# zhoubin-me/supertonic

Measured on AMD Instinct MI355X. Metric: audio-sec/sec (RTF^-1), 66M model, batch=128 per GPU, higher is better.
Workload: dtype bf16

## Files before the change

### include/stn.h

```cpp
#ifndef STN_H
#define STN_H
#include <stddef.h>
#include <stdint.h>

#include "stn_arch.h"

#ifdef __cplusplus
extern "C" {
#endif

#define STN_OK 0
#define STN_ERR_INVALID (-1)
#define STN_ERR_DEVICE (-2)
#define STN_ERR_STATE (-3)
#define STN_ERR_UNSUPPORTED (-4)
#define STN_ERR_IO (-5)

#define STN_DTYPE_F32 0
#define STN_DTYPE_BF16 1
#define STN_DTYPE_F16 2

typedef struct stn_handle stn_handle;

typedef struct stn_config {
// ... 240 lines not shown
int stn_op_expander(stn_handle* h, int hz, int rows, int W, const float* x, const stn_expander* c, float* y);
int stn_op_expander_ex(stn_handle* h, int hz, int rows, int W, const float* x, const stn_expander* c, int x_misalign, int in_place, float* y,
                       float* open_db, float* s1_end, float* s1_start, float* s2_end, float* s2_start, int* guard_ok, char* form,
                       size_t form_cap);
int stn_expander_coefs(const stn_expander* c, int rate_hz, double k[3], float k32[3], int64_t* hold_samples);
int stn_expander_curve(const stn_expander* c, int n, const double* in_db, double* out_db);
const char* stn_expander_error(const stn_expander* c, int rate_hz);

int stn_profile_enable(stn_handle* h, int on);
int stn_profile_reset(stn_handle* h);
int stn_profile_filter(stn_handle* h, const char* family_or_null);
int stn_profile_sample(stn_handle* h, int every);
int stn_launch_log_enable(stn_handle* h, int on);
int64_t stn_launch_log(stn_handle* h, char* out, size_t cap);
int stn_profile_count(stn_handle* h);
int stn_profile_get(stn_handle* h, int idx, char* name, size_t name_cap, double* total_ms, int64_t* launches,
                    double* flops, double* bytes);

int stn_dbg_xattn_hs_enable(stn_handle* h, int on);
int64_t stn_dbg_xattn_hs_stamps(stn_handle* h, unsigned long long* out, size_t cap);
int stn_dbg_fold_run_frames(const int32_t* latent_lengths, int B, int n_cu);

int stn_op_gemm(stn_handle* h, int dtype, int M, int N, int K, const float* A , const float* W ,
                const float* bias_or_null, int act , float* out );
int stn_op_gemm_ex(stn_handle* h, int dtype, int M, int N, int K, const float* A , const float* W , int mode, int act,
                   int out_dtype, int ldo, const float* bias_or_null, const float* gamma_or_null, const int32_t* len_or_null, int L,
                   const int32_t* row_b_or_null, const float* rowvec_or_null, int nseq, int nt, int tr, float* out, int64_t out_elems,
                   char* form, size_t form_cap);
int stn_dbg_gemm_form(int dtype, int M, int N, int K, int mode, int out_dtype, int ldo, int masked, int tr, char* out, size_t cap);
int stn_dbg_ffn_form(int dtype, int stage, int C, int I, int64_t M, int64_t gate_rows, int packed, int k, int max_dil, int mask,
                     int64_t min_rows, int64_t split_min_rows, int nt_hints, char* out, size_t cap);
int stn_op_gemm_bench(stn_handle* h, int dtype, int M, int N, int K, int mode, int iters, double* avg_ms);
int stn_op_gemm_phases(stn_handle* h, int dtype, int M, int N, int K, int mode, double* out6);
int stn_op_dwconv_ln(stn_handle* h, int dtype, int B, int L, int C, int k, int dil, const float* x,
                     const float* w , const float* bias, const float* ln_g, const float* ln_b, float* y);
int stn_op_dwconv_ln_ragged(stn_handle* h, int dtype, int B, int L, int C, int k, int dil, const float* x,
                            const float* w , const float* bias, const float* ln_g, const float* ln_b,
                            const int32_t* seqlen , float* y);
int stn_op_gemm_rows(stn_handle* h, int dtype, int M, int N, int K, const float* A, const float* W, const float* bias_or_null, int B,
                     const int32_t* rows, const int32_t* valid, int T, float* out, int64_t out_elems, char* form, size_t form_cap);
int stn_op_dwconv_ln_ex(stn_handle* h, int dtype, int B, int L, int C, int k, int dil, const float* x, int64_t x_rows,
                        const float* w_or_null , const float* bias_or_null, const float* ln_g, const float* ln_b,
                        const int32_t* seqlen_or_null, int packed, int ln_only, float* y, int64_t y_rows, char* form, size_t form_cap);
int stn_op_dwconv_ln_tail(stn_handle* h, int dtype, int B, int L, int C, int k, int dil, const float* x, int64_t x_rows,
                          const float* w , const float* bias, const float* ln_g, const float* ln_b, const int32_t* seqlen,
                          const float* tail , int T, int rf, float* y, int64_t y_rows, char* form, size_t form_cap);
int64_t stn_dbg_len_tables(int B, const int32_t* llen, int ve_rows, int with_pairs, int vo_form, int ccf, int T, int rf, int32_t* layout,
                           int32_t* out, int64_t out_n);
int stn_dbg_dwconv_ln_form(int dtype, int B, int L, int C, int k, int packed, char* out, size_t cap);
int stn_op_fold_ln(stn_handle* h, int dtype, int M, int C, int S, const float* part, const float* b2, const float* gamma,
                   const float* rowvec_or_null, const int32_t* row_b_or_null, int nseq, const float* ln_g, const float* ln_b, float* x,
                   float* y);
int stn_op_layout(stn_handle* h, int which, int dtype, const int32_t* p, int n_p, const float* a, int64_t a_n, const float* b, int64_t b_n,
                  const float* c, int64_t c_n, const int64_t* ids, int64_t ids_n, const int32_t* len, int packed, float* out, int64_t out_n,
                  float* out2, int64_t out2_n, int32_t* iout, int64_t iout_n);
int stn_op_attention(stn_handle* h, int dtype, int B, int Lq, int Lk, int H, int dh, const float* q, const float* k,
                     const float* v, const int32_t* qlen_or_null, const int32_t* klen_or_null, int rope_mode, float* o);
int stn_op_attention_ex(stn_handle* h, int dtype, int B, int Lq, int Lk, int H, int dh, const float* q, int64_t q_elems, int ldq,
                        int q_col, float* kv, int64_t kv_elems, int ldk, int k_col, int v_col, float* o, int64_t o_elems, int ldo,
                        const int32_t* qlen_or_null, const int32_t* klen_or_null, const int32_t* q_off_or_null,
                        const int32_t* k_off_or_null, int rope_mode, int k_rotated, int rot_groups, int rot_stride, int rot_col,
                        char* form, size_t form_cap);
int stn_op_xattn_hs(stn_handle* h, int dtype, int M, const float* xn, const float* Wq, const float* bq_or_null, const float* Wo,
                    const float* kv, int64_t kv_elems, int ldk, int k_col, int B, int L, int Lk, const int32_t* qlen,
                    const int32_t* klen_or_null, const int32_t* k_off_or_null, int rope_mode, int pairs_mode, int64_t part_stride,
                    float* part, int64_t part_elems, int32_t* pairs_out_or_null, char* form, size_t form_cap);
int stn_dbg_attn_form(int kind, int dtype, int B, int Lq, int Lk, int H, int dh, int ldq, int ldk, int misaligned, char* out, size_t cap);
int stn_op_ffn(stn_handle* h, int M, int C, int I, const float* xn , const float* W1, const float* b1, const float* W2,
               const float* b2_or_null, const float* gamma_or_null, const float* rowvec_or_null ,
               const int32_t* row_b_or_null , int nseq, float* x, int fused);
int stn_op_ffn_ex(stn_handle* h, int dtype, int M, int C, int I, const float* xn, int ldx, int64_t xn_elems, const float* W1, const float* b1,
                  const float* W2, const float* b2_or_null, const float* gamma_or_null, const int32_t* len_or_null, int L,
                  const int32_t* row_b_or_null, const float* rowvec_or_null, int rv_ld, int nseq, int mode, int split, float* x, int ldo,
                  int64_t x_elems, float* part_or_null, int64_t part_stride, int64_t part_elems, char* form, size_t form_cap);
int stn_op_ffn_bench(stn_handle* h, int M, int C, int I, int fused, int iters, double* out5);
int stn_op_fold_dwconv_ln(stn_handle* h, int B, int C, int k, int dil, int S, const int32_t* seqlen, const float* x, const float* part,
                          const float* b2_or_null, const float* gamma_or_null, const float* rowvec_or_null , const float* w ,
                          const float* bias, const float* ln_g, const float* ln_b, float* x_out, float* y);
int stn_op_fold_dwconv_ln_ex(stn_handle* h, int dtype, int B, int L, int C, int k, int dil, int S, int run_frames, const int32_t* seqlen,
                             const float* x_in, int64_t x_rows, const float* part, int64_t part_stride, int64_t part_elems,
                             const float* b2_or_null, const float* gamma_or_null, const float* rowvec_or_null, int rv_ld,
                             const float* w , const float* bias, const float* ln_g, const float* ln_b, float* x_out, int64_t x_out_rows,
                             float* y, int64_t y_rows, char* form, size_t form_cap);
int stn_dbg_fold_dwconv_ln_form(int dtype, int B, int L, int C, int k, int dil, int S, int has_rowvec, int run_frames, char* out, size_t cap);
int stn_op_block_bench(stn_handle* h, int B, int L, int C, int I, int k, int dil, int mode, int iters, double* out6);
int stn_op_randn(stn_handle* h, uint64_t seed, int B, int D, int L, const int64_t* utt_ids_or_null,
                 const int32_t* len_or_null, float* out);

const char* stn_version(void);
int stn_hip_versions(int* built, int* runtime);
int stn_device_count(void);
int stn_device_sync(int device);
int stn_ffn_fused_forms(int dtype, int C, int I);

#ifdef __cplusplus
}
#endif
#endif
```

### supertonic_amd/binding.py

```python
import ctypes
import os

import numpy as np

from .arch import StnArch

_HERE = os.path.dirname(os.path.abspath(__file__))
LIB_PATH = os.environ.get("STN_LIB") or os.path.join(_HERE, "libstn.so")
_LIB = None

F32, BF16, F16 = 0, 1, 2
_DTYPES = {"f32": F32, "fp32": F32, "float32": F32, "bf16": BF16, "f16": F16, "fp16": F16, "float16": F16, "half": F16,
           F32: F32, BF16: BF16, F16: F16}
ACT_NONE, ACT_GELU, ACT_SILU, ACT_GELU_TANH = 0, 1, 2, 3
EPI_STORE, EPI_RESID, EPI_STORE_T = 0, 1, 2
FFN_VOCODER, FFN_ESTIMATOR, FFN_TEXT = 1, 2, 4
LAYOUT_ROW_MAP, LAYOUT_NCL_TO_ROWS, LAYOUT_EULER_NCL, LAYOUT_UNPACK_ROWS, LAYOUT_EMBED, LAYOUT_MASKED_MEAN, LAYOUT_IM2COL, LAYOUT_VOCODER_IN = range(8)
LAYOUT_FILL_ROWS, LAYOUT_HS_PAIRS, LAYOUT_TRIM_LEN = 8, 9, 10
ENC_F32, ENC_PCM16, ENC_PCM24, ENC_MULAW, ENC_ALAW = 0, 1, 2, 3, 4
ENCODINGS = {"f32": ENC_F32, "pcm16": ENC_PCM16, "pcm24": ENC_PCM24, "mulaw": ENC_MULAW, "alaw": ENC_ALAW}
ENCODING_NAMES = {v: k for k, v in ENCODINGS.items()}
ENCODING_BYTES = {ENC_F32: 4, ENC_PCM16: 2, ENC_PCM24: 3, ENC_MULAW: 1, ENC_ALAW: 1}
ZERO_CODEWORD = {ENC_F32: 0, ENC_PCM16: 0, ENC_PCM24: 0, ENC_MULAW: 0xFF, ENC_ALAW: 0xD5}

# ... 462 lines not shown
    L.stn_batch_ve_rows.argtypes = [vp]
    L.stn_batch_ve_rows.restype = ctypes.c_int64
    L.stn_batch_vo_rows.argtypes = [vp]
    L.stn_batch_vo_rows.restype = ctypes.c_int64
    L.stn_graph_replays.restype = ctypes.c_int64
    L.stn_graph_replays.argtypes = [vp]
    L.stn_graphs_cached.restype = ctypes.c_int64
    L.stn_graphs_cached.argtypes = [vp]
    L.stn_batch_dims.argtypes = [vp, ctypes.POINTER(ci), ctypes.POINTER(ci), ctypes.POINTER(ctypes.c_int64)]
    L.stn_batch_fetch.argtypes = [vp, vp, ctypes.c_size_t, vp]
    L.stn_batch_fetch_latent.argtypes = [vp, _f32p]
    L.stn_batch_fetch_pcm16.argtypes = [vp, vp, ctypes.c_size_t, vp]
    L.stn_batch_fetch_pcm16_begin.argtypes = [vp, ci]
    L.stn_batch_fetch_slot_dims.argtypes = [vp, ci, ctypes.POINTER(ci), ctypes.POINTER(ctypes.c_int64)]
    L.stn_batch_fetch_pcm16_end.argtypes = [vp, ci, ctypes.POINTER(vp), ctypes.POINTER(ctypes.c_size_t), vp]
    L.stn_host_alloc_pinned.restype = vp
    L.stn_host_alloc_pinned.argtypes = [ctypes.c_size_t]
    L.stn_host_free_pinned.argtypes = [vp]
    L.stn_batch_wav_device_ptr.argtypes = [vp, ctypes.POINTER(vp)]
    L.stn_sync.argtypes = [vp]
    L.stn_set_stream.argtypes = [vp, vp]
    L.stn_batch_copy_wav_device.argtypes = [vp, vp, ctypes.c_int64]
    L.stn_batch_copy_pcm16_device.argtypes = [vp, vp, ctypes.c_int64]
    L.stn_profile_filter.argtypes = [vp, ctypes.c_char_p]
    L.stn_profile_sample.argtypes = [vp, ci]
    L.stn_launch_log_enable.argtypes = [vp, ci]
    L.stn_dbg_xattn_hs_enable.argtypes = [vp, ci]
    L.stn_dbg_xattn_hs_stamps.argtypes = [vp, vp, ctypes.c_size_t]
    L.stn_dbg_xattn_hs_stamps.restype = ctypes.c_int64
    L.stn_dbg_fold_run_frames.argtypes = [vp, ctypes.c_int, ctypes.c_int]
    L.stn_dbg_fold_run_frames.restype = ctypes.c_int
    L.stn_dbg_gemm_form.argtypes = [ci, ci, ci, ci, ci, ci, ci, ci, ci, ctypes.c_char_p, ctypes.c_size_t]
    L.stn_dbg_gemm_form.restype = ctypes.c_int
    L.stn_dbg_attn_form.argtypes = [ci, ci, ci, ci, ci, ci, ci, ci, ci, ci, ctypes.c_char_p, ctypes.c_size_t]
    L.stn_dbg_attn_form.restype = ctypes.c_int
    L.stn_dbg_ffn_form.argtypes = [ci, ci, ci, ci, ctypes.c_int64, ctypes.c_int64, ci, ci, ci, ci, ctypes.c_int64, ctypes.c_int64, ci,
                                   ctypes.c_char_p, ctypes.c_size_t]
    L.stn_dbg_ffn_form.restype = ctypes.c_int
    L.stn_launch_log.argtypes = [vp, ctypes.c_char_p, ctypes.c_size_t]
    L.stn_launch_log.restype = ctypes.c_int64
    L.stn_profile_enable.argtypes = [vp, ci]
    L.stn_profile_reset.argtypes = [vp]
    L.stn_profile_count.argtypes = [vp]
    L.stn_profile_get.argtypes = [vp, ci, ctypes.c_char_p, ctypes.c_size_t, ctypes.POINTER(ctypes.c_double),
                                  ctypes.POINTER(ctypes.c_int64), ctypes.POINTER(ctypes.c_double),
                                  ctypes.POINTER(ctypes.c_double)]
    L.stn_op_gemm.argtypes = [vp, ci, ci, ci, ci, _f32p, _f32p, vp, ci, _f32p]
    L.stn_op_gemm_ex.argtypes = [vp, ci, ci, ci, ci, _f32p, _f32p, ci, ci, ci, ci, vp, vp, vp, ci, vp, vp, ci, ci, ci, _f32p,
                                 ctypes.c_int64, ctypes.c_char_p, ctypes.c_size_t]
    L.stn_op_gemm_bench.argtypes = [vp, ci, ci, ci, ci, ci, ci, ctypes.POINTER(ctypes.c_double)]
    L.stn_op_gemm_phases.argtypes = [vp, ci, ci, ci, ci, ci, ctypes.POINTER(ctypes.c_double)]
    L.stn_op_dwconv_ln.argtypes = [vp, ci, ci, ci, ci, ci, ci, _f32p, _f32p, _f32p, _f32p, _f32p, _f32p]
    L.stn_op_dwconv_ln_ragged.argtypes = [vp, ci, ci, ci, ci, ci, ci, _f32p, _f32p, _f32p, _f32p, _f32p, _i32p, _f32p]
    L.stn_op_attention.argtypes = [vp, ci, ci, ci, ci, ci, ci, _f32p, _f32p, _f32p, vp, vp, ci, _f32p]
    L.stn_op_gemm_rows.argtypes = [vp, ci, ci, ci, ci, _f32p, _f32p, vp, ci, _i32p, _i32p, ci, _f32p, ctypes.c_int64, ctypes.c_char_p, ctypes.c_size_t]
    L.stn_op_dwconv_ln_ex.argtypes = [vp, ci, ci, ci, ci, ci, ci, _f32p, ctypes.c_int64, vp, vp, _f32p, _f32p, vp, ci, ci, _f32p, ctypes.c_int64,
                                      ctypes.c_char_p, ctypes.c_size_t]
    L.stn_op_dwconv_ln_tail.argtypes = [vp, ci, ci, ci, ci, ci, ci, _f32p, ctypes.c_int64, _f32p, _f32p, _f32p, _f32p, _i32p, _f32p, ci, ci, _f32p,
                                        ctypes.c_int64, ctypes.c_char_p, ctypes.c_size_t]
    L.stn_dbg_resample_form.argtypes = [ci, ci, ctypes.c_int64, ctypes.c_char_p, ctypes.c_size_t]
    L.stn_dbg_resample_form.restype = ctypes.c_int
    L.stn_dbg_dwconv_ln_form.argtypes = [ci, ci, ci, ci, ci, ci, ctypes.c_char_p, ctypes.c_size_t]
    L.stn_dbg_dwconv_ln_form.restype = ctypes.c_int
    L.stn_dbg_len_tables.argtypes = [ci, _i32p, ci, ci, ci, ci, ci, ci, _i32p, ctypes.c_void_p, ctypes.c_int64]
    L.stn_dbg_len_tables.restype = ctypes.c_int64
    L.stn_op_fold_ln.argtypes = [vp, ci, ci, ci, ci, _f32p, _f32p, _f32p, vp, vp, ci, _f32p, _f32p, _f32p, _f32p]
    L.stn_op_layout.argtypes = [vp, ci, ci, _i32p, ci, vp, ctypes.c_int64, vp, ctypes.c_int64, vp, ctypes.c_int64, vp, ctypes.c_int64, vp, ci,
                                vp, ctypes.c_int64, vp, ctypes.c_int64, vp, ctypes.c_int64]
    L.stn_op_attention_ex.argtypes = [vp, ci, ci, ci, ci, ci, ci, _f32p, ctypes.c_int64, ci, ci, _f32p, ctypes.c_int64, ci, ci, ci,
                                      _f32p, ctypes.c_int64, ci, vp, vp, vp, vp, ci, ci, ci, ci, ci, ctypes.c_char_p, ctypes.c_size_t]
    L.stn_op_xattn_hs.argtypes = [vp, ci, ci, _f32p, _f32p, vp, _f32p, _f32p, ctypes.c_int64, ci, ci, ci, ci, ci, _i32p, vp, vp, ci, ci,
                                  ctypes.c_int64, _f32p, ctypes.c_int64, vp, ctypes.c_char_p, ctypes.c_size_t]
    L.stn_op_randn.argtypes = [vp, cu64, ci, ci, ci, vp, vp, _f32p]
    L.stn_op_ffn.argtypes = [vp, ci, ci, ci, _f32p, _f32p, _f32p, _f32p, vp, vp, vp, vp, ci, _f32p, ci]
    L.stn_op_ffn_ex.argtypes = [vp, ci, ci, ci, ci, _f32p, ci, ctypes.c_int64, _f32p, _f32p, _f32p, vp, vp, vp, ci, vp, vp, ci, ci, ci, ci, _f32p, ci,
                                ctypes.c_int64, vp, ctypes.c_int64, ctypes.c_int64, ctypes.c_char_p, ctypes.c_size_t]
    L.stn_op_ffn_bench.argtypes = [vp, ci, ci, ci, ci, ci, ctypes.POINTER(ctypes.c_double)]
    L.stn_set_fused_ffn.argtypes = [vp, ci]
    L.stn_set_fused_ffn_min_rows.argtypes = [vp, ctypes.c_int64, ctypes.c_int64]
    L.stn_op_fold_dwconv_ln.argtypes = [vp, ci, ci, ci, ci, ci, _i32p, _f32p, _f32p, vp, vp, vp, _f32p, _f32p, _f32p, _f32p, _f32p, _f32p]
    L.stn_op_fold_dwconv_ln_ex.argtypes = [vp, ci, ci, ci, ci, ci, ci, ci, ci, _i32p, _f32p, ctypes.c_int64, _f32p, ctypes.c_int64, ctypes.c_int64, vp, vp,
                                           vp, ci, _f32p, _f32p, _f32p, _f32p, _f32p, ctypes.c_int64, _f32p, ctypes.c_int64, ctypes.c_char_p,
                                           ctypes.c_size_t]
    L.stn_dbg_fold_dwconv_ln_form.argtypes = [ci, ci, ci, ci, ci, ci, ci, ci, ci, ctypes.c_char_p, ctypes.c_size_t]
    L.stn_dbg_fold_dwconv_ln_form.restype = ctypes.c_int
    L.stn_op_block_bench.argtypes = [vp, ci, ci, ci, ci, ci, ci, ci, ci, ctypes.POINTER(ctypes.c_double)]
    L.stn_group_create.argtypes = [ci, vp, ci, ctypes.POINTER(vp)]
    L.stn_group_destroy.argtypes = [vp]
    L.stn_group_last_error.restype = ctypes.c_char_p
    L.stn_group_last_error.argtypes = [vp]
    L.stn_group_size.argtypes = [vp]
    L.stn_group_uses_rccl.argtypes = [vp]
    L.stn_group_handle.restype = vp
    L.stn_group_handle.argtypes = [vp, ci]
    L.stn_group_load_synthetic.argtypes = [vp, ctypes.POINTER(StnArch), cu64]
    L.stn_group_load_dir.argtypes = [vp, ctypes.c_char_p]
    L.stn_group_deal.argtypes = [ci, _i32p, ci, _i32p, _i32p]
    L.stn_group_synthesize.argtypes = [vp, ci, ci, _i64p, _f32p, _f32p, _f32p, ci, cf, vp, cu64, ctypes.POINTER(ctypes.c_int64)]
    L.stn_group_fetch_pcm16.argtypes = [vp, vp, ctypes.c_size_t, vp]
    L.stn_set_output_rate.argtypes = [vp, ci]
    L.stn_get_output_rate.argtypes = [vp]
    L.stn_resample_filter.argtypes = [ci, ci, vp, ctypes.c_size_t, ctypes.POINTER(ci), ctypes.POINTER(ci)]
    L.stn_resample_error.argtypes = [ci, ci]
    L.stn_resample_error.restype = ctypes.c_char_p
    L.stn_op_resample.argtypes = [vp, ci, ci, ci, ci, _f32p, vp, vp]
    L.stn_group_set_output_rate.argtypes = [vp, ci]
    _f64p = np.ctypeslib.ndpointer(np.float64, flags="C_CONTIGUOUS")
    L.stn_set_loudness.argtypes = [vp, ci, cf, cf]
    L.stn_get_loudness.argtypes = [vp, ctypes.POINTER(ci), ctypes.POINTER(cf), ctypes.POINTER(cf)]
    L.stn_batch_loudness.argtypes = [vp, vp, vp, vp]
    L.stn_op_loudness.argtypes = [vp, ci, ci, ci, _f32p, vp, vp, vp]
    L.stn_kweighting_filter.argtypes = [ci, _f64p, _f64p, _f64p, _f64p]
    L.stn_op_loudness_ex.argtypes = [vp, ci, ci, ci, _f32p, vp, ci, cf, cf, ci, vp, vp, vp, vp, vp, vp, vp, vp, ctypes.c_char_p, ctypes.c_size_t]
    L.stn_loudness_table.argtypes = [ci, vp, vp, ctypes.c_size_t, ctypes.POINTER(ci)]
    L.stn_group_set_loudness.argtypes = [vp, ci, cf, cf]
    L.stn_batch_loudness_range.argtypes = [vp, vp, vp, vp, vp]
    L.stn_op_loudness_range.argtypes = [vp, ci, ci, ci, _f32p, vp, vp, vp, vp, vp]
    L.stn_set_silence_trim.argtypes = [vp, ci, cf, cf, cf]
    L.stn_get_silence_trim.argtypes = [vp, ctypes.POINTER(ci), ctypes.POINTER(cf), ctypes.POINTER(cf), ctypes.POINTER(cf)]
    L.stn_batch_silence_edges.argtypes = [vp, vp, vp]
    L.stn_op_silence_edges.argtypes = [vp, ci, ci, ci, _f32p, vp, cf, cf, vp, vp]
    L.stn_op_silence_trim.argtypes = [vp, ci, ci, ci, _f32p, vp, cf, cf, cf, vp, ci, vp, vp, vp]
    L.stn_silence_fade_window.argtypes = [ci, cf, vp, ctypes.c_int64, ctypes.POINTER(ctypes.c_int64)]
    L.stn_set_pause_limit.argtypes = [vp, ci, cf]
    L.stn_get_pause_limit.argtypes = [vp, ctypes.POINTER(ci), ctypes.POINTER(cf)]
    L.stn_batch_pauses.argtypes = [vp, vp, vp, vp, ci]
    L.stn_op_pause_trim.argtypes = [vp, ci, ci, ci, _f32p, vp, cf, cf, cf, cf, vp, ci, vp, vp, vp, vp, vp, vp, ci]
    L.stn_op_silence_edges_ex.argtypes = [vp, ci, ci, ci, _f32p, vp, cf, cf, cf, cf, ci, vp, vp, vp, vp, vp, vp, vp, vp, ci, ctypes.c_char_p,
                                          ctypes.c_size_t]
    L.stn_group_set_pause_limit.argtypes = [vp, ci, cf]
    L.stn_set_limiter.argtypes = [vp, ci, cf]
    L.stn_get_limiter.argtypes = [vp, ctypes.POINTER(ci), ctypes.POINTER(cf)]
    L.stn_batch_limiter.argtypes = [vp, vp, vp]
    L.stn_op_limiter.argtypes = [vp, ci, ci, ci, _f32p, vp, vp, cf, cf, vp, vp, vp, vp]
    L.stn_limiter_window.argtypes = [ci, cf, vp, ctypes.c_int64, ctypes.POINTER(ctypes.c_int64)]
    L.stn_group_set_limiter.argtypes = [vp, ci, cf]
    L.stn_set_peak_mode.argtypes = [vp, ci]
    L.stn_get_peak_mode.argtypes = [vp]
    L.stn_group_set_peak_mode.argtypes = [vp, ci]
    L.stn_true_peak_filter.argtypes = [vp, ctypes.c_size_t, ctypes.POINTER(ci), ctypes.POINTER(ci)]
    L.stn_batch_true_peak.argtypes = [vp, vp, vp, vp]
    L.stn_op_true_peak.argtypes = [vp, ci, ci, ci, _f32p, vp, vp, ci, vp, vp, vp, ctypes.c_char_p, ctypes.c_size_t]
    L.stn_op_limiter_ex.argtypes = [vp, ci, ci, ci, _f32p, vp, vp, cf, cf, vp, vp, vp, vp, ci, vp, vp]
    fp = ctypes.POINTER(StnFilter)
    L.stn_set_filters.argtypes = [vp, ci, fp]
    L.stn_get_filters.argtypes = [vp, ctypes.POINTER(ci), fp]
    L.stn_group_set_filters.argtypes = [vp, ci, fp]
    L.stn_op_filter.argtypes = [vp, ci, ci, ci, _f32p, ci, fp, _f32p]
    L.stn_op_filter_ex.argtypes = [vp, ci, ci, ci, _f32p, ci, fp, ci, _f32p, vp, vp, ctypes.POINTER(ci), ctypes.c_char_p, ctypes.c_size_t]
    L.stn_filter_error.argtypes = [ci, fp, ci]
    L.stn_filter_error.restype = ctypes.c_char_p
    L.stn_filter_coefs.argtypes = [fp, ci, _f64p, _f32p]
    L.stn_filter_response.argtypes = [ci, fp, ci, ci, _f64p, _f64p]
    L.stn_dbg_filter_geometry.argtypes = [ctypes.POINTER(ci)] * 4
    cpp = ctypes.POINTER(StnCompressor)
    L.stn_set_compressor.argtypes = [vp, ci, cpp]
    L.stn_get_compressor.argtypes = [vp, ctypes.POINTER(ci), cpp]
    L.stn_group_set_compressor.argtypes = [vp, ci, cpp]
    L.stn_batch_compressor.argtypes = [vp, vp]
    L.stn_op_compressor.argtypes = [vp, ci, ci, ci, _f32p, cpp, _f32p]
    L.stn_op_compressor_ex.argtypes = [vp, ci, ci, ci, _f32p, cpp, ci, ci, _f32p, vp, vp, vp, vp, vp, ctypes.POINTER(ci), ctypes.c_char_p, ctypes.c_size_t]
    L.stn_compressor_error.argtypes = [cpp, ci]
    L.stn_compressor_error.restype = ctypes.c_char_p
    L.stn_compressor_coefs.argtypes = [cpp, ci, _f64p, _f32p]
    L.stn_compressor_curve.argtypes = [cpp, ci, _f64p, _f64p]
    xpp = ctypes.POINTER(StnExpander)
# ... 483 lines not shown
        raise StnError(-1, f"stn_limiter_window: {lookahead_ms} ms at {hz} Hz refused (lookahead_ms in [0.5, 10], hz in [8000, 192000])")
    w = np.empty(n.value, np.float32)
    if L.stn_limiter_window(int(hz), float(lookahead_ms), w.ctypes.data, w.size, ctypes.byref(n)) < 0:
        raise StnError(-1, "stn_limiter_window failed")
    return w


def _loudness_args(target_lufs):
    return (0, -23.0) if target_lufs is None else (1, float(target_lufs))


def resample_error(in_hz, out_hz):
    return load().stn_resample_error(int(in_hz), int(out_hz)).decode()


def resample_form(in_hz, out_hz, W):
    buf = ctypes.create_string_buffer(64)
    r = load().stn_dbg_resample_form(int(in_hz), int(out_hz), int(W), buf, len(buf))
    if r < 0:
        why = resample_error(in_hz, out_hz)
        raise StnError(r, f"stn_dbg_resample_form: {why}" if why else f"stn_dbg_resample_form: W = {W}, W >= 1 is required")
    return buf.value.decode()


def fold_run_frames(latent_lengths, n_cu=256):
    a = np.ascontiguousarray(latent_lengths, dtype=np.int32)
    r = load().stn_dbg_fold_run_frames(a.ctypes.data, len(a), int(n_cu))
    if r < 0:
        raise StnError(r, "stn_dbg_fold_run_frames: bad arguments")
    return int(r)


def gemm_form(dtype, M, N, K, mode=EPI_STORE, out_dtype="f32", ldo=None, masked=False, tr=-1):
    buf = ctypes.create_string_buffer(128)
    r = load().stn_dbg_gemm_form(_DTYPES[dtype], int(M), int(N), int(K), int(mode), _DTYPES[out_dtype], int(N if ldo is None else ldo),
                                 int(bool(masked)), int(tr), buf, len(buf))
    if r < 0:
        raise StnError(r, "stn_dbg_gemm_form: the launcher refuses this call")
    return buf.value.decode()


def attn_form(dtype, B, Lq, Lk, H, dh, ldq=None, ldk=None, misaligned=0, kind=0):
    buf = ctypes.create_string_buffer(64)
    C = H * dh
    r = load().stn_dbg_attn_form(int(kind), _DTYPES[dtype], int(B), int(Lq), int(Lk), int(H), int(dh), int(C if ldq is None else ldq),
                                 int(C if ldk is None else ldk), int(misaligned), buf, len(buf))
    if r < 0:
        raise StnError(r, "stn_dbg_attn_form: the launcher refuses this call")
    return buf.value.decode()


def dwconv_ln_form(dtype, B, L, C, k, packed=False):
    buf = ctypes.create_string_buffer(32)
    r = load().stn_dbg_dwconv_ln_form(_DTYPES[dtype], int(B), int(L), int(C), int(k), int(bool(packed)), buf, len(buf))
    if r < 0:
        raise StnError(r, "stn_dbg_dwconv_ln_form: the launcher refuses this call")
    return buf.value.decode()


LEN_VO_NONE, LEN_VO_2RF, LEN_VO_TAIL, LEN_VO_SCALED = range(4)


def len_tables(llen, ve_rows=0, with_pairs=False, vo_form=LEN_VO_NONE, ccf=6, T=0, rf=0):
    llen = _c(llen, np.int32)
    B = len(llen)
    lay = np.zeros(9, np.int32)
    args = (B, llen, int(ve_rows), int(bool(with_pairs)), int(vo_form), int(ccf), int(T), int(rf))
    tot = load().stn_dbg_len_tables(*args, lay, None, 0)
    if tot < 0:
        raise StnError(int(tot), "stn_dbg_len_tables: bad argument")
    out = np.full(tot, -12345, np.int32)
    out[:2] = 7
    assert load().stn_dbg_len_tables(*args, lay, out.ctypes.data, out.size) == tot
    assert out[0] == 7 and out[1] == 7
    names = ("seed", "llen", "ve_off", "ve_row_b", "pairs", "vo_n", "vo_valid", "vo_off")
    sizes = {"llen": B, "ve_off": B + 1, "ve_row_b": int(ve_rows), "pairs": B + 2, "vo_n": B, "vo_valid": B, "vo_off": B + 1}
    res = {"total": int(tot)}
    for i, n in enumerate(names):
        if n != "seed" and lay[i] >= 0:
            res[n] = out[lay[i]:lay[i] + sizes[n]].copy()
    return res


def fold_dwconv_ln_form(dtype, B, L, C, k, dil, S, rowvec=True, run_frames=0):
    buf = ctypes.create_string_buffer(96)
    r = load().stn_dbg_fold_dwconv_ln_form(_DTYPES[dtype], int(B), int(L), int(C), int(k), int(dil), int(S), int(bool(rowvec)), int(run_frames),
                                           buf, len(buf))
    if r < 0:
        raise StnError(r, "stn_dbg_fold_dwconv_ln_form: the launcher refuses this call")
    return buf.value.decode()


def ffn_form(dtype, stage, C, I, M, gate_rows=0, packed=True, k=5, max_dil=1, mask=9, min_rows=18432, split_min_rows=1, nt_hints=True):
    buf = ctypes.create_string_buffer(32)
    r = load().stn_dbg_ffn_form(_DTYPES[dtype], int(stage), int(C), int(I), int(M), int(gate_rows), int(bool(packed)), int(k), int(max_dil),
                                int(mask), int(min_rows), int(split_min_rows), int(bool(nt_hints)), buf, len(buf))
    if r < 0:
        raise StnError(r, "stn_dbg_ffn_form: invalid arguments")
    return buf.value.decode()


def _c(a, dt):
    return np.ascontiguousarray(a, dtype=dt)


def _opt(a, dt):
    if a is None:
        return None, None
    arr = _c(a, dt)
    return arr, arr.ctypes.data


class Engine:

    def __init__(self, device=0, dtype="bf16"):
        self._lib = load()
        self._h = ctypes.c_void_p()
        cfg = StnConfig(device, _DTYPES[dtype])
        rc = self._lib.stn_create(ctypes.byref(cfg), ctypes.byref(self._h))
        if rc != 0:
            msg = self._lib.stn_last_error(None).decode()
            self._h = None
            raise StnError(rc, msg)
        self.dtype = _DTYPES[dtype]
        self.device = device
        self.arch = None
        self._slot_enc = {}

    def close(self):
        if getattr(self, "_h", None):
            self._lib.stn_destroy(self._h)
            self._h = None

    def __del__(self):
        try:
            self.close()
        except Exception:
            pass

    def _need_model(self):
        if self.arch is None:
            raise StnError(-3, "no model loaded: call load_synthetic or load_dir first")

    def _ck(self, rc):
        if rc < 0:
            raise StnError(rc, self._lib.stn_last_error(self._h).decode())
        return rc

    def load_synthetic(self, arch: StnArch, seed: int = 7):
        self._ck(self._lib.stn_load_synthetic(self._h, ctypes.byref(arch), seed))
        self.arch = arch

    def last_error(self) -> str:
        return (self._lib.stn_last_error(self._h) or b"").decode()

    def load_dir(self, onnx_dir: str):
        self._ck(self._lib.stn_load_dir(self._h, onnx_dir.encode()))
        a = StnArch()
        self._ck(self._lib.stn_get_arch(self._h, ctypes.byref(a)))
        self.arch = a

    def tensor_names(self, arch: StnArch):
        n = self._ck(self._lib.stn_tensor_names(self._h, ctypes.byref(arch), None, 0))
        buf = ctypes.create_string_buffer(n + 1)
        self._ck(self._lib.stn_tensor_names(self._h, ctypes.byref(arch), buf, n + 1))
        return buf.value.decode().split("\n")[:-1]
# ... 781 lines not shown

    def op_gemm_bench(self, M, N, K, mode=0, iters=20, dtype=None):
        ms = ctypes.c_double()
        self._ck(self._lib.stn_op_gemm_bench(self._h, self.dtype if dtype is None else _DTYPES[dtype], M, N, K, mode,
                                             iters, ctypes.byref(ms)))
        return ms.value

    def op_ffn(self, xn, W1, b1, W2, b2, gamma, x, rowvec=None, row_b=None, fused=True):
        M, C = xn.shape
        I = W1.shape[0]
        out = np.array(x, dtype=np.float32, order="C", copy=True)
        _, b2p = _opt(b2, np.float32)
        b2a = _opt(b2, np.float32)[0]
        ga, gp = _opt(gamma, np.float32)
        rva, rvp = _opt(rowvec, np.float32)
        rba, rbp = _opt(row_b, np.int32)
        b2p = b2a.ctypes.data if b2a is not None else None
        self._ck(self._lib.stn_op_ffn(self._h, M, C, I, _c(xn, np.float32), _c(W1, np.float32), _c(b1, np.float32), _c(W2, np.float32),
                                      b2p, gp, rvp, rbp, 0 if rva is None else rva.shape[0], out, int(fused)))
        return out

    def op_ffn_ex(self, xn, W1, b1, W2, x, mode=1, b2=None, gamma=None, len=None, L=None, row_b=None, rowvec=None, split=0, part=None,
                  part_stride=0, M=None, dtype=None):
        xn = _c(xn, np.float32)
        I, C = W1.shape
        M = xn.shape[0] if M is None else int(M)
        x_r = np.array(x, dtype=np.float32, order="C", copy=True)
        p_r = None if part is None else np.array(part, dtype=np.float32, order="C", copy=True)
        nseq = 0
        for v in (len, rowvec):
            if v is not None:
                nseq = max(nseq, np.asarray(v).shape[0])
        if row_b is not None and rowvec is None:
            nseq = max(nseq, int(np.max(row_b)) + 1)
        _b, bp = _opt(b2, np.float32)
        _g, gp = _opt(gamma, np.float32)
        _l, lp = _opt(len, np.int32)
        _r, rp = _opt(row_b, np.int32)
        _v, vp_ = _opt(rowvec, np.float32)
        form = ctypes.create_string_buffer(32)
        self._ck(self._lib.stn_op_ffn_ex(self._h, self.dtype if dtype is None else _DTYPES[dtype], M, C, I, xn.reshape(-1), xn.shape[1], xn.size,
                                         _c(W1, np.float32), _c(b1, np.float32), _c(W2, np.float32), bp, gp, lp, int(M if L is None else L), rp, vp_,
                                         C if _v is None else _v.shape[1], nseq, int(mode), int(split), x_r.reshape(-1), x_r.shape[1], x_r.size,
                                         None if p_r is None else p_r.ctypes.data, int(part_stride), 0 if p_r is None else p_r.size, form,
                                         ctypes.sizeof(form)))
        return x_r, p_r, form.value.decode()

    def op_ffn_bench(self, M, C, I, fused=True, iters=20):
        out = (ctypes.c_double * 5)()
        self._ck(self._lib.stn_op_ffn_bench(self._h, M, C, I, int(fused), iters, out))
        return dict(ms=out[0], first_stage=out[1], tile_loop=out[2], epilogue=out[3], workgroups=int(out[4]))

    def op_fold_dwconv_ln(self, seqlen, x, part, b2, gamma, rowvec, w, bias, g, b, k, dil):
        seqlen = np.ascontiguousarray(seqlen, np.int32)
        S, M, C = part.shape
        xo = np.empty((M, C), np.float32)
        y = np.empty((M, C), np.float32)
        b2a, _ = _opt(b2, np.float32)
        ga, _ = _opt(gamma, np.float32)
        rva, _ = _opt(rowvec, np.float32)
        p = lambda a: None if a is None else a.ctypes.data
        self._ck(self._lib.stn_op_fold_dwconv_ln(self._h, len(seqlen), C, k, dil, S, seqlen, _c(x, np.float32), _c(part, np.float32), p(b2a), p(ga), p(rva),
                                                 _c(w, np.float32), _c(bias, np.float32), _c(g, np.float32), _c(b, np.float32), xo, y))
        return xo, y

    def op_fold_dwconv_ln_ex(self, seqlen, L, x_in, part, part_stride, S, b2, gamma, rowvec, w, bias, g, b, dil, x_out, y, run_frames=0, dtype=None):
        seqlen = _c(seqlen, np.int32)
        x_in = _c(x_in, np.float32)
        part = _c(part, np.float32).reshape(-1)
        xo = np.array(x_out, dtype=np.float32, order="C", copy=True)
        yo = np.array(y, dtype=np.float32, order="C", copy=True)
        C = x_in.shape[1]
        w = _c(w, np.float32)
        _b2, b2p = _opt(b2, np.float32)
        _g, gp = _opt(gamma, np.float32)
        _v, vp_ = _opt(rowvec, np.float32)
        form = ctypes.create_string_buffer(96)
        self._ck(self._lib.stn_op_fold_dwconv_ln_ex(self._h, self.dtype if dtype is None else _DTYPES[dtype], len(seqlen), int(L), C, w.shape[1], int(dil),
                                                    int(S), int(run_frames), seqlen, x_in.reshape(-1), x_in.shape[0], part, int(part_stride), part.size,
                                                    b2p, gp, vp_, C if _v is None else _v.shape[1], w, _c(bias, np.float32), _c(g, np.float32),
                                                    _c(b, np.float32), xo.reshape(-1), xo.shape[0], yo.reshape(-1), yo.shape[0], form, ctypes.sizeof(form)))
        return xo, yo, form.value.decode()

    def op_block_bench(self, B, L, C, I, k, dil, mode, iters=20):
        out = (ctypes.c_double * 6)()
        self._ck(self._lib.stn_op_block_bench(self._h, B, L, C, I, k, dil, mode, iters, out))
        return dict(ms=out[0], conv_ms=out[1], fold_phase1=out[2], fold_barrier=out[3], fold_phase2=out[4], fold_span=out[5])

    def set_fused_ffn_min_rows(self, k4_rows=-1, split_rows=-1):
        self._ck(self._lib.stn_set_fused_ffn_min_rows(self._h, int(k4_rows), int(split_rows)))

    def op_gemm_phases(self, M, N, K, mode=0, dtype=None):
        out = (ctypes.c_double * 6)()
        self._ck(self._lib.stn_op_gemm_phases(self._h, self.dtype if dtype is None else _DTYPES[dtype], M, N, K, mode, out))
        return dict(first_stage=out[0], k_loop=out[1], epilogue=out[2], grid_span=out[3], entry_spread=out[4], workgroups=int(out[5]))

    def op_dwconv_ln(self, x, w, bias, g, b, dil, dtype=None, seqlen=None):
        B, L, C = x.shape
        k = w.shape[1]
        y = np.empty((B, L, C), np.float32)
        if seqlen is not None:
            self._ck(self._lib.stn_op_dwconv_ln_ragged(self._h, self.dtype if dtype is None else _DTYPES[dtype], B, L, C, k,
                                                       dil, _c(x, np.float32), _c(w, np.float32), _c(bias, np.float32),
                                                       _c(g, np.float32), _c(b, np.float32), _c(seqlen, np.int32), y))
            return y
        self._ck(self._lib.stn_op_dwconv_ln(self._h, self.dtype if dtype is None else _DTYPES[dtype], B, L, C, k, dil,
                                            _c(x, np.float32), _c(w, np.float32), _c(bias, np.float32),
                                            _c(g, np.float32), _c(b, np.float32), y))
        return y

    def op_gemm_rows(self, A, W, out, rows, valid, T, bias=None, dtype=None):
        A = _c(A, np.float32)
        W = _c(W, np.float32)
        rows = _c(rows, np.int32)
        valid = _c(valid, np.int32)
        o_r = np.array(out, dtype=np.float32, order="C", copy=True)
        _b, bp = _opt(bias, np.float32)
        form = ctypes.create_string_buffer(96)
        self._ck(self._lib.stn_op_gemm_rows(self._h, self.dtype if dtype is None else _DTYPES[dtype], A.shape[0], W.shape[0], A.shape[1],
                                            A.reshape(-1), W.reshape(-1), bp, len(rows), rows, valid, int(T), o_r.reshape(-1), o_r.size, form,
                                            ctypes.sizeof(form)))
        return o_r, form.value.decode()

    def op_dwconv_ln_ex(self, x, w, bias, g, b, dil, out, B, L, seqlen=None, packed=False, ln_only=False, dtype=None):
        x = _c(x, np.float32)
        o_r = np.array(out, dtype=np.float32, order="C", copy=True)
        C = x.shape[1]
        _w, wp = _opt(w, np.float32)
        _b, bp = _opt(bias, np.float32)
        _l, lp = _opt(seqlen, np.int32)
        form = ctypes.create_string_buffer(32)
        self._ck(self._lib.stn_op_dwconv_ln_ex(self._h, self.dtype if dtype is None else _DTYPES[dtype], int(B), int(L), C,
                                               1 if _w is None else _w.shape[1], int(dil), x.reshape(-1), x.shape[0], wp, bp, _c(g, np.float32),
                                               _c(b, np.float32), lp, int(bool(packed)), int(bool(ln_only)), o_r.reshape(-1), o_r.shape[0], form,
                                               ctypes.sizeof(form)))
        return o_r, form.value.decode()

    def op_dwconv_ln_tail(self, x, w, bias, g, b, dil, out, L, seqlen, tail, T, dtype=None):
        x = _c(x, np.float32)
        tail = _c(tail, np.float32)
        o_r = np.array(out, dtype=np.float32, order="C", copy=True)
        C = x.shape[1]
        w = _c(w, np.float32)
        seqlen = _c(seqlen, np.int32)
        assert tail.ndim == 2 and tail.shape[1] == C and tail.shape[0] >= 1
        form = ctypes.create_string_buffer(32)
        self._ck(self._lib.stn_op_dwconv_ln_tail(self._h, self.dtype if dtype is None else _DTYPES[dtype], len(seqlen), int(L), C, w.shape[1],
                                                 int(dil), x.reshape(-1), x.shape[0], w, _c(bias, np.float32), _c(g, np.float32),
                                                 _c(b, np.float32), seqlen, tail.reshape(-1), int(T), tail.shape[0] - 1, o_r.reshape(-1),
                                                 o_r.shape[0], form, ctypes.sizeof(form)))
        return o_r, form.value.decode()

    def op_fold_ln(self, x, part, b2, gamma, g, b, rowvec=None, row_b=None, dtype=None):
        x_r = np.array(x, dtype=np.float32, order="C", copy=True)
        M, C = x_r.shape
        part = _c(part, np.float32)
        y = np.empty((M, C), np.float32)
        _v, vp_ = _opt(rowvec, np.float32)
        _r, rp = _opt(row_b, np.int32)
        self._ck(self._lib.stn_op_fold_ln(self._h, self.dtype if dtype is None else _DTYPES[dtype], M, C, part.shape[0], part.reshape(-1),
                                          _c(b2, np.float32), _c(gamma, np.float32), vp_, rp, 0 if _v is None else _v.shape[0],
                                          _c(g, np.float32), _c(b, np.float32), x_r, y))
        return x_r, y

    def op_layout(self, which, p, a=None, b=None, c=None, ids=None, length=None, packed=False, out=None, out2=None, iout=None, dtype="f32"):
        def f32(v):
# ... 81 lines not shown
```

### supertonic_amd/csrc/api.cpp

```cpp
#include "../../include/stn.h"

#include <algorithm>
#include <complex>
#include <cstdio>
#include <cstring>
#include <fstream>
#include <string>

#include "engine.hpp"
#include "host/json_min.hpp"
#include "host/graph_bind.hpp"
#include "host/onnx_reader.hpp"

#include <map>
#include <sstream>

struct stn_handle {
    stn::Engine* eng = nullptr;
    std::string err;
    std::vector<std::pair<std::string, stn::KernelStat>> prof;
};

static thread_local std::string g_create_err;

#define STN_TRY(h, body)                                             \
    if (!(h)) return STN_ERR_INVALID;                                \
    try {                                                            \
        body;                                                        \
        return STN_OK;                                               \
    } catch (const std::invalid_argument& e) {                       \
        (h)->err = e.what();                                         \
        return STN_ERR_INVALID;                                      \
    } catch (const std::exception& e) {                              \
        (h)->err = e.what();                                         \
        return (h)->err.rfind("HIP error", 0) == 0 ? STN_ERR_DEVICE : STN_ERR_STATE; \
    } catch (...) {                                                  \
        (h)->err = "unknown failure";                                \
        return STN_ERR_DEVICE;                                       \
    }

static void need(bool ok, const char* what) {
    if (!ok) throw std::invalid_argument(what);
}
static void need_model(stn_handle* h) {
    if (!h->eng->loaded()) throw std::runtime_error("no model loaded: call stn_load_synthetic or stn_load_dir first");
}

extern "C" {

const char* stn_version(void) { return "supertonic_amd 0.1 (gfx950)"; }

int stn_hip_versions(int* built, int* runtime) {
    int rt = 0;
    const hipError_t e = hipRuntimeGetVersion(&rt);
    if (built) *built = HIP_VERSION;
    if (runtime) *runtime = e == hipSuccess ? rt : -1;
    return e == hipSuccess ? STN_OK : STN_ERR_DEVICE;
}
int stn_device_count(void) {
    int n = 0;
    if (hipGetDeviceCount(&n) != hipSuccess) { (void)hipGetLastError(); return STN_ERR_DEVICE; }
    return n;
}
int stn_device_sync(int device) {
    if (hipSetDevice(device) != hipSuccess || hipDeviceSynchronize() != hipSuccess) { (void)hipGetLastError(); return STN_ERR_DEVICE; }
    return STN_OK;
}
int stn_ffn_fused_forms(int dtype, int C, int I) {
    if (C <= 0 || I <= 0 || !stn::ffn_fused_supported(dtype, C, I)) return 0;
    return stn::ffn_split_factor(dtype, C, I) > 1 ? 2 : 1;
}

int stn_create(const stn_config* cfg, stn_handle** out) {
    if (!cfg || !out) { g_create_err = "stn_create: null argument"; return STN_ERR_INVALID; }
    *out = nullptr;
    try {
        stn_handle* h = new stn_handle;
        h->eng = new stn::Engine(cfg->device, cfg->dtype);
        *out = h;
        return STN_OK;
    } catch (const std::exception& e) {
        g_create_err = e.what();
        return STN_ERR_DEVICE;
    }
}
int stn_destroy(stn_handle* h) {
    if (!h) return STN_OK;
    try { delete h->eng; } catch (...) {}
    delete h;
    return STN_OK;
}
const char* stn_last_error(const stn_handle* h) { return h ? h->err.c_str() : g_create_err.c_str(); }
// ... 1039 lines not shown
    if (form && form_cap) std::snprintf(form, form_cap, "%s", f.c_str());
}
int stn_op_xattn_hs(stn_handle* h, int dtype, int M, const float* xn, const float* Wq, const float* bq, const float* Wo, const float* kv,
                    int64_t kv_elems, int ldk, int k_col, int B, int L, int Lk, const int32_t* qlen, const int32_t* klen, const int32_t* k_off,
                    int rope_mode, int pairs_mode, int64_t part_stride, float* part, int64_t part_elems, int32_t* pairs_out, char* form,
                    size_t form_cap) {
    STN_TRY(h, xattn_hs_checked(h, dtype, M, xn, Wq, bq, Wo, kv, kv_elems, ldk, k_col, B, L, Lk, qlen, klen, k_off, rope_mode, pairs_mode,
                                part_stride, part, part_elems, pairs_out, form, form_cap))
}
int stn_dbg_attn_form(int kind, int dtype, int B, int Lq, int Lk, int H, int dh, int ldq, int ldk, int misaligned, char* out, size_t cap) {
    if (B < 1 || Lq < 1 || Lk < 1 || H < 1 || (dtype != STN_DTYPE_F32 && dtype != STN_DTYPE_BF16 && dtype != STN_DTYPE_F16) || (kind != 0 && kind != 1))
        return STN_ERR_INVALID;
    std::string f;
    try {
        if (kind == 0) {
            auto ptr = [&](int bit) { return reinterpret_cast<const void*>((uintptr_t)(misaligned & bit ? 4 : 0)); };
            f = stn::attn_form(dtype, B, Lq, Lk, H, dh, ldq, ldk, ptr(1), ptr(2), ptr(4)).str();
        } else {
            f = stn::xattn_hs_form(dtype, H * dh, H, B, Lq, Lk, ldk).str();
        }
    } catch (const std::exception&) { return STN_ERR_INVALID; }
    if (out && cap > f.size()) std::memcpy(out, f.c_str(), f.size() + 1);
    return (int)f.size();
}
int stn_op_ffn(stn_handle* h, int M, int C, int I, const float* xn, const float* W1, const float* b1, const float* W2, const float* b2,
               const float* gamma, const float* rowvec, const int32_t* row_b, int nseq, float* x, int fused) {
    STN_TRY(h, { need(M > 0 && C > 0 && I > 0 && C % 8 == 0 && I % 8 == 0 && xn && W1 && b1 && W2 && x, "stn_op_ffn: bad argument");
                 need(!rowvec || nseq > 0, "stn_op_ffn: rowvec needs nseq > 0");
                 if (rowvec && row_b) for (int m = 0; m < M; ++m) need(row_b[m] >= 0 && row_b[m] < nseq, "stn_op_ffn: row_b out of range");
                 need(fused >= 0 && fused <= 2, "stn_op_ffn: mode must be 0 (two launches), 1 (K4) or 2 (K4-split + fold)");
                 h->eng->op_ffn(M, C, I, xn, W1, b1, W2, b2, gamma, rowvec, row_b, nseq, x, fused); })
}
static void ffn_ex_checked(stn_handle* h, int dtype, int M, int C, int I, const float* xn, int ldx, int64_t xn_elems, const float* W1, const float* b1,
                           const float* W2, const float* b2, const float* gamma, const int32_t* len, int L, const int32_t* row_b, const float* rowvec,
                           int rv_ld, int nseq, int mode, int split, float* x, int ldo, int64_t x_elems, float* part, int64_t part_stride,
                           int64_t part_elems, char* form, size_t form_cap) {
    need(M > 0 && C > 0 && I > 0 && C % 8 == 0 && I % 8 == 0 && xn && W1 && b1 && W2 && x && L >= 1, "stn_op_ffn_ex: bad argument");
    need((dtype == STN_DTYPE_BF16 || dtype == STN_DTYPE_F16) && dtype == h->eng->dtype(), "stn_op_ffn_ex: dtype must be the 16-bit format of the engine");
    need(mode >= stn::FFN_GEMMS && mode <= stn::FFN_K4_SPLIT, "stn_op_ffn_ex: mode must be 0 (two launches), 1 (K4) or 2 (K4-split)");
    need(mode == stn::FFN_GEMMS || stn::ffn_fused_supported(dtype, C, I), "stn_op_ffn_ex: shape not supported by the fused kernel");
    need(ldx >= C && ldx % 8 == 0 && xn_elems >= (int64_t)M * ldx, "stn_op_ffn_ex: needs ldx >= C, ldx % 8 == 0 and xn_elems >= M*ldx");
    need(ldo >= C && ldo % 4 == 0 && x_elems >= (int64_t)M * ldo, "stn_op_ffn_ex: needs ldo >= C, ldo % 4 == 0 and x_elems >= M*ldo");
    need(!(len && row_b), "stn_op_ffn_ex: len and row_b exclude each other");
    const int64_t seqs = ((int64_t)M + L - 1) / L;
    if (len || (rowvec && !row_b)) need(nseq >= seqs, "stn_op_ffn_ex: len / rowvec by m / L need nseq >= ceil(M/L)");
    if (rowvec || len || row_b) need(nseq > 0, "stn_op_ffn_ex: nseq must be > 0");
    if (rowvec) need(rv_ld >= C && rv_ld % 4 == 0, "stn_op_ffn_ex: needs rv_ld >= C and rv_ld % 4 == 0");
    if (len) for (int b = 0; b < nseq; ++b) need(len[b] >= 0 && len[b] <= L, "stn_op_ffn_ex: len out of [0, L]");
    if (row_b) for (int m = 0; m < M; ++m) need(row_b[m] >= 0 && row_b[m] < nseq, "stn_op_ffn_ex: row_b out of [0, nseq)");
    if (mode == stn::FFN_K4_SPLIT) {
        const int S = split ? split : stn::ffn_split_choose(dtype, C, I, M);
        need(stn::ffn_split_valid(dtype, C, I, S), "stn_op_ffn_ex: not a split this shape runs with");
        need(part && part_stride >= stn::ffn_split_rows(M) * C && part_stride % 8 == 0 && part_elems >= (int64_t)S * part_stride,
             "stn_op_ffn_ex: mode 2 needs part, part_stride >= rows padded to 128 * C (a multiple of 8) and part_elems >= S * part_stride");
    } else {
        need(split == 0 && !part, "stn_op_ffn_ex: split and part belong to mode 2");
    }
    const std::string f = h->eng->op_ffn_ex(M, C, I, xn, ldx, xn_elems, W1, b1, W2, b2, gamma, len, L, row_b, rowvec, rv_ld, nseq, mode, split, x, ldo,
                                            x_elems, part, part_stride, part_elems);
    if (form && form_cap) std::snprintf(form, form_cap, "%s", f.c_str());
}
int stn_op_ffn_ex(stn_handle* h, int dtype, int M, int C, int I, const float* xn, int ldx, int64_t xn_elems, const float* W1, const float* b1,
                  const float* W2, const float* b2, const float* gamma, const int32_t* len, int L, const int32_t* row_b, const float* rowvec, int rv_ld,
                  int nseq, int mode, int split, float* x, int ldo, int64_t x_elems, float* part, int64_t part_stride, int64_t part_elems, char* form,
                  size_t form_cap) {
    STN_TRY(h, ffn_ex_checked(h, dtype, M, C, I, xn, ldx, xn_elems, W1, b1, W2, b2, gamma, len, L, row_b, rowvec, rv_ld, nseq, mode, split, x, ldo,
                              x_elems, part, part_stride, part_elems, form, form_cap))
}
int stn_op_ffn_bench(stn_handle* h, int M, int C, int I, int fused, int iters, double* out5) {
    STN_TRY(h, { need(M > 0 && C > 0 && I > 0 && C % 8 == 0 && I % 8 == 0 && iters > 0 && out5, "stn_op_ffn_bench: bad argument");
                 need(fused >= 0 && fused <= 2, "stn_op_ffn_bench: mode must be 0, 1 or 2");
                 h->eng->op_ffn_bench(M, C, I, fused, iters, out5); })
}
int stn_op_fold_dwconv_ln(stn_handle* h, int B, int C, int k, int dil, int S, const int32_t* seqlen, const float* x, const float* part,
                          const float* b2, const float* gamma, const float* rowvec, const float* w, const float* bias, const float* g,
                          const float* b, float* x_out, float* y) {
    STN_TRY(h, { need(B > 0 && C > 0 && C % 8 == 0 && (k == 5 || k == 7) && dil > 0 && (S == 4 || S == 8 || S == 12 || S == 24) && seqlen && x && part && w && bias && g && b && x_out && y,
                      "stn_op_fold_dwconv_ln: bad argument");
                 int64_t tot = 0;
                 for (int i = 0; i < B; ++i) { need(seqlen[i] >= 0 && seqlen[i] < (1 << 20), "stn_op_fold_dwconv_ln: seqlen out of range"); tot += seqlen[i]; }
                 need(tot > 0, "stn_op_fold_dwconv_ln: no rows");
                 h->eng->op_fold_dwconv_ln(B, C, k, dil, S, seqlen, x, part, b2, gamma, rowvec, w, bias, g, b, x_out, y); })
}
static void fold_dwconv_ln_ex_checked(stn_handle* h, int dtype, int B, int L, int C, int k, int dil, int S, int run_frames, const int32_t* seqlen,
                                      const float* x_in, int64_t x_rows, const float* part, int64_t part_stride, int64_t part_elems, const float* b2,
                                      const float* gamma, const float* rowvec, int rv_ld, const float* w, const float* bias, const float* g,
                                      const float* b, float* x_out, int64_t x_out_rows, float* y, int64_t y_rows, char* form, size_t form_cap) {
    const char* who = "stn_op_fold_dwconv_ln_ex";
    auto req = [&](bool ok, const char* what) { need(ok, (std::string(who) + ": " + what).c_str()); };
    req(B > 0 && L > 0 && C > 0 && seqlen && x_in && part && w && bias && g && b && x_out && y, "bad argument");
    req(dtype == STN_DTYPE_BF16 || dtype == STN_DTYPE_F16, "a 16-bit format needed");
    req(B <= 1024, "B <= 1024 needed");
    try { (void)stn::fold_dwconv_ln_form(dtype, B, L, C, k, dil, S, rowvec != nullptr, run_frames); }
    catch (const std::invalid_argument& e) { req(false, e.what()); }
    int64_t tot = 0;
    for (int i = 0; i < B; ++i) { req(seqlen[i] >= 0 && seqlen[i] <= L, "seqlen out of [0, L]"); tot += seqlen[i]; }
    req(tot > 0, "no rows");
    req(tot * C * 2 < 0x7FFFFFFFll, "too many rows");
    req(x_rows >= tot && x_out_rows >= tot && y_rows >= tot, "x_in / x_out / y hold fewer rows than the launch addresses");
    req(part_stride >= tot * C && part_stride % 8 == 0 && part_elems >= (int64_t)(S - 1) * part_stride + tot * C, "part smaller than the launch addresses, or a stride that is no multiple of 8");
    req(!rowvec || (rv_ld >= C && rv_ld % 4 == 0), "rv_ld >= C, a multiple of 4, needed");
    const std::string f = h->eng->op_fold_dwconv_ln_ex(dtype, B, L, C, k, dil, S, run_frames, seqlen, x_in, x_rows, part, part_stride, part_elems, b2, gamma,
                                                       rowvec, rv_ld, w, bias, g, b, x_out, x_out_rows, y, y_rows);
    if (form && form_cap) std::snprintf(form, form_cap, "%s", f.c_str());
}
int stn_op_fold_dwconv_ln_ex(stn_handle* h, int dtype, int B, int L, int C, int k, int dil, int S, int run_frames, const int32_t* seqlen,
                             const float* x_in, int64_t x_rows, const float* part, int64_t part_stride, int64_t part_elems, const float* b2,
                             const float* gamma, const float* rowvec, int rv_ld, const float* w, const float* bias, const float* g, const float* b,
                             float* x_out, int64_t x_out_rows, float* y, int64_t y_rows, char* form, size_t form_cap) {
    STN_TRY(h, fold_dwconv_ln_ex_checked(h, dtype, B, L, C, k, dil, S, run_frames, seqlen, x_in, x_rows, part, part_stride, part_elems, b2, gamma, rowvec,
                                         rv_ld, w, bias, g, b, x_out, x_out_rows, y, y_rows, form, form_cap))
}
int stn_dbg_fold_dwconv_ln_form(int dtype, int B, int L, int C, int k, int dil, int S, int has_rowvec, int run_frames, char* out, size_t cap) {
    std::string f;
    try { f = stn::fold_dwconv_ln_form(dtype, B, L, C, k, dil, S, has_rowvec != 0, run_frames).str(); } catch (const std::exception&) { return STN_ERR_INVALID; }
    if (out && cap > f.size()) std::memcpy(out, f.c_str(), f.size() + 1);
    return (int)f.size();
}
int stn_op_block_bench(stn_handle* h, int B, int L, int C, int I, int k, int dil, int mode, int iters, double* out2) {
    STN_TRY(h, { need(B > 0 && L > 0 && C > 0 && I > 0 && C % 8 == 0 && I % 8 == 0 && (k == 5 || k == 7) && dil > 0 && iters > 0 && out2 && (mode == 0 || mode == 2),
                      "stn_op_block_bench: bad argument");
                 h->eng->op_block_bench(B, L, C, I, k, dil, mode, iters, out2); })
}
int stn_op_randn(stn_handle* h, uint64_t seed, int B, int D, int L, const int64_t* utt_ids, const int32_t* len, float* out) {
    STN_TRY(h, { need(B > 0 && D > 0 && L > 0 && out, "stn_op_randn: bad argument"); h->eng->op_randn(seed, B, D, L, utt_ids, len, out); })
}

}
```

### supertonic_amd/csrc/engine.cpp

```cpp
#include "engine.hpp"
#include "dev_env.hpp"
#include "engine_internal.hpp"

#include <algorithm>
#include <cmath>
#include <cstdio>
#include <cstring>

namespace stn {
using detail::up;

Arena::~Arena() {
    for (auto& c : chunks_) (void)hipFree(c.p);
}
size_t Arena::capacity() const {
    size_t t = 0;
    for (auto& c : chunks_) t += c.cap;
    return t;
}
void* Arena::alloc(size_t bytes) {
    bytes = (bytes + 255) & ~size_t(255);
    if (bytes == 0) bytes = 256;
    for (;;) {
        if (cur_ < chunks_.size()) {
// ... 416 lines not shown
    if (g_launch_ev.start) {
        g_launch_ev = LaunchEvents{};
        ev_pool_.push_back(spans_.back().a);
        ev_pool_.push_back(spans_.back().b);
        spans_.pop_back();
    }
    prof_active_ = false;
}
void Engine::profile_reset() {
    sync();
    for (auto& sp : spans_) { ev_pool_.push_back(sp.a); ev_pool_.push_back(sp.b); }
    spans_.clear();
    g_launch_log.entries.clear();
}
void Engine::launch_log_enable(bool on) { g_launch_log.on = on; g_launch_log.family = "-"; g_launch_log.entries.clear(); }
std::string Engine::launch_log() const {
    std::string out;
    for (const auto& e : g_launch_log.entries) {
        std::string k = e.second;
        size_t b = 0;
        while (b < k.size() && (k[b] == '(' || k[b] == ' ' || k[b] == '&')) ++b;
        size_t en = b;
        while (en < k.size() && (isalnum((unsigned char)k[en]) || k[en] == '_' || k[en] == ':')) ++en;
        out += e.first + "\t" + k.substr(b, en - b) + "\n";
    }
    return out;
}
std::vector<std::pair<std::string, KernelStat>> Engine::profile_collect() {
    sync();
    std::unordered_map<std::string, KernelStat> acc;
    std::vector<std::string> order;
    for (auto& sp : spans_) {
        float ms = 0.f;
        if (hipEventElapsedTime(&ms, sp.a, sp.b) != hipSuccess) { (void)hipGetLastError(); continue; }
        auto it = acc.find(sp.tag);
        if (it == acc.end()) { order.push_back(sp.tag); it = acc.emplace(sp.tag, KernelStat{}).first; }
        it->second.ms += ms;
        it->second.launches += 1;
        it->second.flops += sp.flops;
        it->second.bytes += sp.bytes;
    }
    std::vector<std::pair<std::string, KernelStat>> out;
    for (auto& t : order) out.emplace_back(t, acc[t]);
    return out;
}

void Engine::gemm(const char* tag, int dt, const void* A, int lda, const Linear& w, int M, Epilogue e) {
    if (!e.bias) e.bias = w.b;
    const double esz = is_half(dt) ? 2.0 : 4.0;
    if (prof_on_) {
        double out_b = (double)M * w.N * (e.mode == EPI_STORE ? (is_half(e.out_dtype) ? 2.0 : 4.0) : (e.mode == EPI_RESID ? 8.0 : 4.0));
        prof_begin(tag, 2.0 * M * (double)w.N * w.K, ((double)M * w.K + (double)w.N * w.K) * esz + out_b);
    }
    const GemmForm f = gemm_form(dt, M, w.N, w.K, lda, w.K, e, A, w.w.as(dt));
    if (f.split > 1) {
        const Arena::Mark mk = ar_.mark();
        float* ws = f32_alloc((int64_t)f.split * M * w.N);
        launch_gemm_form(s_, f, A, lda, w.w.as(dt), w.K, M, w.N, w.K, e, ws);
        ar_.release(mk);
    } else {
        launch_gemm_form(s_, f, A, lda, w.w.as(dt), w.K, M, w.N, w.K, e, nullptr);
    }
    if (prof_on_) prof_end();
}

void* Engine::to_act(const float* src, int64_t n) {
    if (dt_ == F32) return const_cast<float*>(src);
    void* d = act_alloc(n);
    launch_cast(s_, dt_, src, n, d);
    return d;
}

void Engine::convnext(const ConvNeXt& p, const FfnForm& f, float* x, int B, int L, int C, int hid, int k, int dil, const int* len,
                      const int* conv_len, const float* rowvec, int rv_ld, const Ragged* rg, FoldState* fs, const DwconvTail& tl) {
    const int64_t M = rg ? (int64_t)rg->rows : (int64_t)B * L;
    if (f.kind == FFN_K4_SPLIT && !(fs && rg)) throw std::logic_error("convnext: K4-split needs the stage's fold state and packed rows");
    const Arena::Mark mk = ar_.mark();
    void* xn = act_alloc(M * C);
    if (fs) x = fs->x;
    if (tl.tail && (fs || !rg)) throw std::logic_error("convnext: a tail table needs packed rows and no fold state");
    if (fs && fs->pending) {
        if (prof_on_) prof_begin("fold_dwconv_ln", (double)M * C * (2.0 * k + 8 + 2.0 * fs->fold.S), (double)M * C * (8.0 + 2.0 + 2.0 * fs->fold.S));
        fs->fold.run_frames = rg->fold_run;
        launch_fold_dwconv_ln(s_, dt_, fs->x, fs->x_alt, B, L, C, fs->fold, p.dw_t, p.dw_b, k, dil, p.ln.g, p.ln.b, a_.ln_eps, xn, len, rg->off);
        if (prof_on_) prof_end();
        std::swap(fs->x, fs->x_alt);
        fs->pending = false;
        x = fs->x;
    } else {
        if (prof_on_) prof_begin("dwconv_ln", (double)M * C * (2.0 * k + 8), (double)M * C * (4.0 + (is_half(dt_) ? 2.0 : 4.0)));
        launch_dwconv_ln(s_, dt_, x, B, L, C, p.dw_t, p.dw_b, k, dil, p.ln.g, p.ln.b, a_.ln_eps, xn, rg ? len : conv_len, rg ? rg->off : nullptr, tl);
        if (prof_on_) prof_end();
    }
    FfnArgs fa;
    fa.xn = xn; fa.ldx = C; fa.b1 = p.pw1.b; fa.b2 = p.pw2.b; fa.gamma = p.gamma; fa.x = x; fa.ldo = C; fa.M = (int)M; fa.I = hid;
    fa.rowvec = rowvec; fa.rv_ld = rv_ld; fa.row_b = (rg && rowvec) ? rg->row_b : nullptr;
    fa.len = rg ? nullptr : len; fa.L = L;
    if (f.kind != FFN_GEMMS) {
        const auto fw = ffn_w_.find(p.pw1.w.as(dt_));
        const int* s = std::find(std::begin(FFN_SPLITS), std::end(FFN_SPLITS), f.split);
        fa.wseq = fw == ffn_w_.end() ? nullptr : f.kind == FFN_K4 ? fw->second.wseq : s != std::end(FFN_SPLITS) ? fw->second.wsplit[s - FFN_SPLITS] : nullptr;
        if (!fa.wseq) throw std::logic_error("convnext: no packed weight stream for " + f.str());
    }
    if (f.kind == FFN_K4_SPLIT) { fa.part = fs->part; fa.part_stride = fs->part_stride; }
    const FoldArgs pending = ffn_launch(f, C, fa, p.pw1, p.pw2);
    if (f.kind == FFN_K4_SPLIT) { fs->fold = pending; fs->pending = true; }
    ar_.release(mk);
}

FoldArgs Engine::ffn_launch(const FfnForm& f, int C, const FfnArgs& a, const Linear& w1, const Linear& w2) {
    const int64_t M = a.M;
    const int hid = a.I;
    FoldArgs pending;
    if (f.kind == FFN_K4_SPLIT) {
        FfnArgs sa;
        sa.xn = a.xn; sa.ldx = a.ldx; sa.wseq = a.wseq; sa.b1 = a.b1; sa.M = a.M; sa.I = hid; sa.ts = a.ts;
        sa.split = f.split; sa.part = a.part; sa.part_stride = a.part_stride;
        if (prof_on_) prof_begin("ffn_split", 4.0 * M * (double)C * hid, (double)M * C * (2.0 + 2.0 * sa.split) + 4.0 * C * hid);
        launch_ffn_fused(s_, dt_, C, sa);
        if (prof_on_) prof_end();
        pending = ffn_pending(f, a);
    } else if (f.kind == FFN_K4) {
        if (prof_on_) prof_begin("ffn_fused", 4.0 * M * (double)C * hid, (double)M * C * (2.0 + 8.0) + 4.0 * C * hid);
        launch_ffn_fused(s_, dt_, C, a);
        if (prof_on_) prof_end();
    } else {
        const Arena::Mark mk = ar_.mark();
        void* u = act_alloc(M * hid);
        Epilogue e1;
        e1.mode = EPI_STORE; e1.act = gelu_act_; e1.out_dtype = dt_; e1.out = u; e1.ldo = hid; e1.bias = a.b1; e1.nt = f.nt ? 1 : 0;
        gemm("gemm_pw1_gelu", dt_, a.xn, a.ldx, w1, (int)M, e1);
        Epilogue e2;
        e2.mode = EPI_RESID; e2.resid = a.x; e2.ldo = a.ldo; e2.bias = a.b2; e2.gamma = a.gamma; e2.len = a.len; e2.L = a.L;
        e2.rowvec = a.rowvec; e2.rv_ld = a.rv_ld; e2.row_b = a.row_b;
        gemm("gemm_pw2_resid", dt_, u, hid, w2, (int)M, e2);
        ar_.release(mk);
    }
    return pending;
}

void Engine::fold_layernorm(FoldState& fs, int64_t M, int C, const LNorm& ln, void* xn, const char* tag) {
    const size_t esz = is_half(dt_) ? 2 : 4;
    if (fs.pending) {
        if (prof_on_) prof_begin("fold_ln", (double)M * C * (8 + 2.0 * fs.fold.S), (double)M * C * (8.0 + esz + 2.0 * fs.fold.S));
        launch_fold_ln(s_, dt_, fs.x, M, C, fs.fold, ln.g, ln.b, a_.ln_eps, xn);
        if (prof_on_) prof_end();
        fs.pending = false;
        return;
    }
    if (tag && prof_on_) prof_begin(tag, (double)M * C * 8, (double)M * C * (4.0 + esz));
    launch_layernorm(s_, dt_, fs.x, M, C, ln.g, ln.b, a_.ln_eps, xn);
    if (tag && prof_on_) prof_end();
}

void Engine::attn_block(const Attn& p, float* x, int B, int Lq, int C, int H, const void* ctx, int Lk, const int* qlen,
                        const int* klen, int rope_mode, bool self, const Ragged* qrg) {
    const int64_t Mq = qrg ? (int64_t)qrg->rows : (int64_t)B * Lq, Mk = (int64_t)B * Lk;
    const Arena::Mark mk = ar_.mark();
    const size_t esz = is_half(dt_) ? 2 : 4;
    void* xn = act_alloc(Mq * C);
    if (prof_on_) prof_begin("layernorm", (double)Mq * C * 8, (double)Mq * C * (4.0 + esz));
    launch_layernorm(s_, dt_, x, Mq, C, p.ln.g, p.ln.b, a_.ln_eps, xn);
    if (prof_on_) prof_end();
    const char *q = nullptr, *k = nullptr, *v = nullptr;
    int ldq = C, ldk = 2 * C;
    if (self) {
// ... 597 lines not shown
```

### supertonic_amd/csrc/engine.hpp

```cpp
#pragma once
#include <cmath>
#include <hip/hip_runtime.h>

#include <algorithm>
#include <cstdint>
#include <functional>
#include <initializer_list>
#include <iterator>
#include <stdexcept>
#include <string>
#include <unordered_map>
#include <vector>

#include "../../include/stn_arch.h"
#include "host/len_tables.hpp"
#include "host/join_plan.hpp"
#include "host/pause_plan.hpp"
#include "host/formant.hpp"
#include "host/pitch.hpp"
#include "kernels.hpp"

namespace stn {

#define STN_HIP(expr)                                                                                          \
// ... 77 lines not shown

   private:
    char* p_ = nullptr;
    size_t cap_ = 0;
};

class DeviceTable {
   public:
    DeviceTable() = default;
    DeviceTable(const DeviceTable&) = delete;
    DeviceTable& operator=(const DeviceTable&) = delete;
    ~DeviceTable() { if (p_) (void)hipFree(p_); }
    void* put(Engine& e, const void* host, size_t bytes);
    template <typename T> T* put(Engine& e, const std::vector<T>& host) { return static_cast<T*>(put(e, host.data(), host.size() * sizeof(T))); }
    explicit operator bool() const { return p_ != nullptr; }

   private:
    void* p_ = nullptr;
};
template <typename Table, size_t N = 1>
struct OnDevice { Table t; DeviceTable dev[N]; };

struct RowSpans { const int64_t* n = nullptr; const int64_t* full = nullptr; };

struct Carve {
    char* base = nullptr;
    size_t off = 0;
    template <typename T> T* take(size_t count) {
        const size_t o = off;
        off += (count * sizeof(T) + 255) / 256 * 256;
        return base ? reinterpret_cast<T*>(base + o) : nullptr;
    }
};

enum Stage : int { ST_PITCH, ST_RATE, ST_FILTER, ST_EXPANDER, ST_DEESSER, ST_COMPRESSOR, N_STAGES };
struct RowsId {
    uint64_t seq = 0; int hz = 0; int64_t Wo = 0; uint64_t gen[N_STAGES] = {};
    bool operator==(const RowsId& o) const { return seq == o.seq && hz == o.hz && Wo == o.Wo && std::equal(gen, gen + N_STAGES, o.gen); }
};
template <typename Set, typename Table>
struct DynStage {
    bool on = false;
    Set set;
    uint64_t gen = 0;
    struct Made { Table t; Set from{}; DeviceTable dev[2]; };
    Made tab, op_tab;
    DevBuf buf;
    RowsId key; const void* key_buf = nullptr; bool valid = false;
};

struct KernelStat { double ms = 0; long launches = 0; double flops = 0; double bytes = 0; };

class Engine {
   public:
    Engine(int device, int dtype);
    ~Engine();
    Engine(const Engine&) = delete;

    void load_synthetic(const stn_arch& a, uint64_t seed);
    using TensorSource = std::function<std::vector<float>(const std::string& name, int rows, int cols)>;
    void load_tensors(const stn_arch& a, const TensorSource& src);
    std::vector<std::string> tensor_names(const stn_arch& a);
    bool loaded() const { return loaded_; }
    const stn_arch& arch() const { return a_; }
    int64_t param_count() const { return params_; }
    int dtype() const { return dt_; }
    hipStream_t stream() const { return s_; }
    void sync() { STN_HIP(hipStreamSynchronize(s_)); if (dp_s_) STN_HIP(hipStreamSynchronize(dp_s_)); if (te_s_) STN_HIP(hipStreamSynchronize(te_s_)); ++drains_; }
    void set_stream(hipStream_t s);

    struct Ragged;
    void duration_dev(int B, int Lt, const int64_t* ids, const float* style_dp, const int* tlen, float* dur, const Ragged* trg = nullptr);
    void text_enc_dev(int B, int Lt, const int64_t* ids, const float* style_ttl, const int* tlen, float* ncl, void* rows,
                      const Ragged* trg = nullptr);
    struct VeCtx { void* text_kv = nullptr; void* style_kv = nullptr; int Lt = 0; const int* text_off = nullptr; };
    VeCtx ve_prepare_dev(int B, int Lt, const void* text_rows, const float* style_ttl, const int* tlen, const Ragged* trg = nullptr, bool defer_text = false);
    void ve_text_kv_dev(const VeCtx& c, int B, int Lt, const void* text_rows, const int* tlen, const Ragged* trg);
    float* ve_time_cond_dev(int rows, const float* total_step, const float* current_step, float* tb_out = nullptr );
    struct TimeCond { int steps = 0, B = 0; uint64_t wgen = ~0ull; float* buf = nullptr; size_t cap = 0; float *tot = nullptr, *cur = nullptr, *dt = nullptr, *tb = nullptr; };
    TimeCond tcond_;
    void ensure_time_cond(int total_step, int B);
    struct Ragged { const int* off = nullptr; const int* row_b = nullptr; int rows = 0;
                    const int* hs_pairs = nullptr;
                    int fold_run = 0; };
    void ve_step_dev(int B, int L, const VeCtx& c, const float* noisy, const int* tlen, const int* llen,
                     const float* total_step, const float* current_step, float* denoised, const float* tb = nullptr,
                     const Ragged* rg = nullptr, const float* dt = nullptr ,
                     void* z_rows = nullptr ,
                     bool z_ready = false ,
                     bool z_next = false );
    void vocoder_dev(int B, int L, const float* latent, float* wav, const int* vlen = nullptr, int vrows = 0,
                     const int* valid = nullptr, bool tails = false, const int* voff = nullptr);
    int vocoder_receptive_field() const;
    void prepare_xattn_weights();
    std::unordered_map<const void*, const void*> frag_w_;
    void hs_stamps_enable(bool on);
    int64_t hs_stamps_fetch(unsigned long long* out, size_t cap);
    unsigned long long* hs_ts_ = nullptr;
    int hs_ts_wgs_ = 0;
    static constexpr int HS_TS_WG = 8192;
    const float* unit_vec_ = nullptr;
    std::unordered_map<const void*, const void*> frag_acc_w_;
    void prepare_vocoder_constants();
    void prepare_ffn_weights();
    struct FfnW { const void *wseq = nullptr, *wsplit[std::size(FFN_SPLITS)] = {}; };
    std::unordered_map<const void*, FfnW> ffn_w_;

    void duration(int B, int Lt, const int64_t* ids, const float* style_dp, const float* text_mask, float* dur);
    void text_enc(int B, int Lt, const int64_t* ids, const float* style_ttl, const float* text_mask, float* text_emb);
    void vector_est(int B, int L, int Lt, const float* noisy, const float* text_emb, const float* style_ttl,
                    const float* text_mask, const float* latent_mask, const float* total_step,
                    const float* current_step, float* denoised);
    void vocoder(int B, int L, const float* latent, float* wav);

    struct Batch {
        int B = 0, Lt = 0, L = 0, noise_L = 0, total_step = 0;
        float speed = 1.f;
        bool have_override = false, have_noise = false;
        uint64_t noise_seed = 0;
        int64_t* ids = nullptr; size_t ids_cap = 0;
        int* tlen = nullptr; size_t tlen_cap = 0;
        float* style_ttl = nullptr; size_t ttl_cap = 0;
        float* style_dp = nullptr; size_t dp_cap = 0;
        float* dur = nullptr; size_t dur_cap = 0;
        int* llen = nullptr;
        int* tab = nullptr; size_t tab_cap = 0;
        LenTables tl;
        int64_t* utt_ids = nullptr; size_t utt_cap = 0;
        float* noise = nullptr; size_t noise_cap = 0;
        float* xt[2] = {nullptr, nullptr}; size_t xt_cap[2] = {0, 0};
        float* wav = nullptr; size_t wav_cap = 0;
        unsigned char* text_side = nullptr; size_t text_side_cap = 0;
        unsigned char* text_rows = nullptr; size_t text_cap = 0;
        int* toff = nullptr; size_t toff_cap = 0;
        int trows = 0;
        uint64_t gen = 0;
        std::vector<float> h_dur; std::vector<int> h_llen;
    };
    void batch_upload(int B, int Lt, const int64_t* ids, const float* text_mask, const float* style_ttl,
                      const float* style_dp, const float* duration_override, const int64_t* utt_ids);
    void batch_set_noise(const float* noise, int L);
    void batch_run(int total_step, float speed, uint64_t noise_seed);
    void set_graph_mode(bool on) { graph_on_ = on; }
    void set_vocoder_mode(bool length_aware) { vo_ragged_ = length_aware; }
    void set_packed_rows(bool on) { packed_ve_ = on; }
    void set_gelu_form(int tanh_form) { if ((tanh_form != 0) != (gelu_act_ == ACT_GELU_TANH)) { sync(); drop_graphs(); } gelu_act_ = tanh_form ? ACT_GELU_TANH : ACT_GELU; }
    int gelu_form() const { return gelu_act_ == ACT_GELU_TANH ? 1 : 0; }
    void set_shape_buckets(bool on) { shape_buckets_ = on; }
    static int64_t bucket_up(int64_t x, int64_t min_gran) {
        if (x <= 0) return x;
        int64_t g = min_gran;
        while (g * 8 <= x) g *= 2;
        return (x + g - 1) / g * g;
    }
    void set_duration_read(bool always) { dur_read_always_ = always; }
    void set_fused_xattn(int mode) { fused_xattn_ = mode ? 1 : 0; }
    void set_fused_ffn(int mask) { fused_ffn_ = mask; }
    void set_fused_ffn_min_rows(int64_t k4_rows, int64_t split_rows) {
        sync(); drop_graphs();
        if (k4_rows >= 0) ffn_min_rows_ = k4_rows;
        if (split_rows >= 0) ffn_split_min_rows_ = split_rows;
    }
    int fused_ffn() const { return fused_ffn_; }
    int64_t last_ve_rows() const { return last_ve_rows_; }
    int64_t last_vo_rows() const { return last_vo_rows_; }
    bool packed_text_ok(int B) const {
        return packed_ve_ && B <= 1024 && dwconv_ln_supports_packed(a_.te_dim, a_.te_kernel) && dwconv_ln_supports_packed(a_.dp_dim, a_.dp_kernel);
    }
    bool packed_rows_ok(int B) const { return packed_ve_ && B <= 1024 && a_.ve_dilated > 0 && dwconv_ln_supports_packed(a_.ve_dim, a_.ve_kernel); }
    long graph_replays() const { return graph_replays_; }
    size_t graphs_cached() const { return graphs_.size(); }
    const Batch& batch() const { return bt_; }
    void batch_fetch(float* wav, size_t wav_capacity, float* duration);
    void batch_fetch_pcm16(int16_t* pcm, size_t capacity, float* duration);
    bool fetch_slot_dims(int slot, int* B, int64_t* W) const {
        const FetchSlot& f = fetch_[slot];
        if (!f.busy || f.dur.empty()) return false;
        *B = (int)f.dur.size(); *W = (int64_t)(f.n / f.dur.size());
        return true;
    }
    void batch_fetch_pcm16_begin(int slot);
    void batch_fetch_pcm16_end(int slot, const int16_t** pcm, size_t* n, float* duration);
    void batch_fetch_latent(float* latent);
    void batch_copy_wav_device(float* dst, int64_t dst_stride);
    void batch_copy_pcm16_device(int16_t* dst, int64_t dst_stride);
    void batch_fetch_encoded(int enc, void* dst, size_t capacity_bytes, float* duration);
    void batch_fetch_encoded_begin(int slot, int enc);
    void batch_fetch_encoded_end(int slot, const void** data, size_t* n_bytes, float* duration);
    void batch_copy_encoded_device(int enc, void* dst, int64_t dst_stride);
    void op_encode(int enc, int rows, int W, const float* x, void* y);
    void set_dither(int mode, uint64_t seed);
    int dither_mode() const { return dither_.mode; }
    uint64_t dither_seed() const { return dither_.seed; }
    void set_pitch(float semitones);
    float pitch() const { return ps_semi_; }
    int pitch_a() const { return ps_a_; }
    int pitch_b() const { return ps_b_; }
    bool pitch_on() const { return ps_a_ != ps_b_; }
    void op_time_stretch(int hz, int rows, int W, const float* x, const int64_t* n, int a, int b, float* y, int* delta, float* score);
    void op_pitch(int hz, int rows, int W, const float* x, const int64_t* n, float semitones, float* y);
    void set_pitch_mode(int mode);
    int pitch_mode() const { return ps_mode_; }
    struct FormantProbe {
        float *ax = nullptr, *cy = nullptr;
        double *g = nullptr, *ex = nullptr, *ey = nullptr;
        bool guard_ok = false;
    };
    void op_formant(int hz, int rows, int W, const float* x, const float* y, const int64_t* n, float* out, FormantProbe* probe = nullptr);
// ... 81 lines not shown
    void op_filter(int hz, int rows, int W, const float* x, int n, const stn_filter* f, float* y, FlProbe* probe);

    void set_compressor(bool on, const stn_compressor* c);
    bool compressor_on() const { return cp_.on; }
    const stn_compressor& compressor() const { return cp_.set; }
    void batch_compressor(float* max_reduction_db);
    struct CpProbe {
        int x_misalign = 0, in_place = 0;
        float *gr = nullptr, *s1_end = nullptr, *s1_start = nullptr, *s2_end = nullptr, *s2_start = nullptr;
        bool guard_ok = false;
        const char* form = "";
    };
    void op_compressor(int hz, int rows, int W, const float* x, const stn_compressor& c, float* y, CpProbe* probe);

    void set_deesser(bool on, const stn_deesser* c);
    bool deesser_on() const { return ds_.on; }
    const stn_deesser& deesser() const { return ds_.set; }
    void batch_deesser(float* max_reduction_db);
    struct DsProbe {
        int x_misalign = 0, in_place = 0;
        float *band = nullptr, *gr = nullptr, *st_end = nullptr, *st_start = nullptr;
        float *s1_end = nullptr, *s1_start = nullptr, *s2_end = nullptr, *s2_start = nullptr;
        bool guard_ok = false;
        const char* form = "";
    };
    void op_deesser(int hz, int rows, int W, const float* x, const stn_deesser& c, float* y, DsProbe* probe);

    void set_expander(bool on, const stn_expander* c);
    bool expander_on() const { return xp_.on; }
    const stn_expander& expander() const { return xp_.set; }
    void batch_expander(float* min_attenuation_db, int64_t* closed_samples);
    struct XpProbe {
        int x_misalign = 0, in_place = 0;
        float *open = nullptr, *s1_end = nullptr, *s1_start = nullptr, *s2_end = nullptr, *s2_start = nullptr;
        bool guard_ok = false;
        const char* form = "";
    };
    void op_expander(int hz, int rows, int W, const float* x, const stn_expander& c, float* y, XpProbe* probe);

    void profile_enable(bool on) { if (on != prof_on_) profile_reset(); prof_on_ = on; }
    void launch_log_enable(bool on);
    std::string launch_log() const;
    void profile_sample(int every) { prof_every_ = every < 1 ? 1 : every; prof_seen_ = 0; }
    void profile_filter(const std::string& family) { if (family != prof_filter_) profile_reset(); prof_filter_ = family; }
    void profile_reset();
    std::vector<std::pair<std::string, KernelStat>> profile_collect();

    void op_gemm(int dtype, int M, int N, int K, const float* A, const float* W, const float* bias, int act, float* out);
    std::string op_gemm_ex(int dtype, int M, int N, int K, const float* A, const float* W, int mode, int act, int out_dtype, int ldo,
                           const float* bias, const float* gamma, const int* len, int L, const int* row_b, const float* rowvec, int nseq,
                           int nt, int tr, float* out, int64_t out_elems);
    std::string op_attention_ex(int dtype, int B, int Lq, int Lk, int H, int dh, const float* q, int64_t q_elems, int ldq, int q_col,
                                float* kv, int64_t kv_elems, int ldk, int k_col, int v_col, float* o, int64_t o_elems, int ldo,
                                const int* qlen, const int* klen, const int* q_off, const int* k_off, int rope_mode, int k_rotated,
                                int rot_groups, int rot_stride, int rot_col);
    std::string op_xattn_hs(int dtype, int M, const float* xn, const float* Wq, const float* bq, const float* Wo, const float* kv,
                            int64_t kv_elems, int ldk, int k_col, int B, int L, int Lk, const int* qlen, const int* klen, const int* k_off,
                            int rope_mode, int pairs_mode, int64_t part_stride, float* part, int64_t part_elems, int* pairs_out);
    void op_attention(int dtype, int B, int Lq, int Lk, int H, int dh, const float* q, const float* k, const float* v,
                      const int* qlen, const int* klen, int rope_mode, float* o);
    std::string op_gemm_rows(int dtype, int M, int N, int K, const float* A, const float* W, const float* bias, int B, const int* rows,
                             const int* valid, int T, float* out, int64_t out_elems);
    void op_dwconv_ln(int dtype, int B, int L, int C, int k, int dil, const float* x, const float* w, const float* bias,
                      const float* g, const float* b, float* y, const int* seqlen = nullptr );
    std::string op_dwconv_ln_ex(int dtype, int B, int L, int C, int k, int dil, const float* x, int64_t x_rows, const float* w, const float* bias,
                                const float* g, const float* b, const int* seqlen, int packed, int ln_only, float* y, int64_t y_rows,
                                const float* tail = nullptr, int T = 0, int rf = 0);
    void op_fold_ln(int dtype, int M, int C, int S, const float* part, const float* b2, const float* gamma, const float* rowvec, const int* row_b,
                    int nseq, const float* g, const float* b, float* x, float* y);
    void op_layout(int which, int dtype, const int* p, const float* a, int64_t a_n, const float* b, int64_t b_n, const float* c, int64_t c_n,
                   const int64_t* ids, int64_t ids_n, const int* len, int packed, float* out, int64_t out_n, float* out2, int64_t out2_n, int* iout,
                   int64_t iout_n);
    double op_gemm_bench(int dtype, int M, int N, int K, int mode, int iters);
    void op_gemm_phases(int dtype, int M, int N, int K, int mode, double* out6);
    void op_randn(uint64_t seed, int B, int D, int L, const int64_t* utt_ids, const int* len, float* out);
    void op_ffn(int M, int C, int I, const float* xn, const float* W1, const float* b1, const float* W2, const float* b2, const float* gamma,
                const float* rowvec , const int* row_b , int nseq, float* x, int mode);
    std::string op_ffn_ex(int M, int C, int I, const float* xn, int ldx, int64_t xn_elems, const float* W1, const float* b1, const float* W2,
                          const float* b2, const float* gamma, const int* len, int L, const int* row_b, const float* rowvec, int rv_ld, int nseq,
                          int mode, int split, float* x, int ldo, int64_t x_elems, float* part, int64_t part_stride, int64_t part_elems);
    void op_fold_dwconv_ln(int B, int C, int k, int dil, int S, const int* seqlen, const float* x, const float* part, const float* b2,
                           const float* gamma, const float* rowvec , const float* w , const float* bias,
                           const float* g, const float* b, float* x_out, float* y);
    std::string op_fold_dwconv_ln_ex(int dtype, int B, int L, int C, int k, int dil, int S, int run_frames, const int* seqlen, const float* x_in,
                                     int64_t x_rows, const float* part, int64_t part_stride, int64_t part_elems, const float* b2, const float* gamma,
                                     const float* rowvec, int rv_ld, const float* w, const float* bias, const float* g, const float* b, float* x_out,
                                     int64_t x_out_rows, float* y, int64_t y_rows);
    void op_ffn_bench(int M, int C, int I, int mode, int iters, double* out5);
    void op_block_bench(int B, int L, int C, int I, int k, int dil, int mode, int iters, double* out6);

    Arena& arena() { return ar_; }

   private:
    DevTensor& tensor(const std::string& name);
    const float* vecf(const std::string& name) { return tensor(name).f32; }
    Linear linear(const std::string& prefix);
    LNorm lnorm(const std::string& prefix);
    ConvNeXt convnext_w(const std::string& prefix);
    Attn attn_w(const std::string& prefix, bool self);
    void free_weights();
    using RawSource = std::function<std::vector<float>(const std::string& name, int kind, int rows, int cols, float gain)>;
    void load_weights(const stn_arch& a, const RawSource& src, std::vector<std::string>* names_only);

    size_t act_bytes(int64_t n) const { return (size_t)n * (is_half(dt_) ? 2 : 4); }
    void* act_alloc(int64_t n) { return ar_.alloc(act_bytes(n)); }
    float* f32_alloc(int64_t n) { return static_cast<float*>(ar_.alloc((size_t)n * 4)); }
    void gemm(const char* tag, int dt, const void* A, int lda, const Linear& w, int M, Epilogue e);
    struct FoldState {
        float* x = nullptr;
        float* x_alt = nullptr;
        void* part = nullptr;
        int64_t part_stride = 0;
        bool pending = false;
        FoldArgs fold;
    };
    FfnForm ffn_plan(int stage, int C, int I, int64_t M, int64_t gate_rows, bool packed, int k, int max_dil) const {
        return ffn_form(dt_, stage, C, I, M, gate_rows, packed, k, max_dil, fused_ffn_, ffn_min_rows_, ffn_split_min_rows_, nt_hints_);
    }
    FoldArgs ffn_launch(const FfnForm& f, int C, const FfnArgs& a, const Linear& w1, const Linear& w2);
    static FoldArgs ffn_pending(const FfnForm& f, const FfnArgs& a) {
        return FoldArgs{a.part, f.split, a.part_stride, a.b2, a.gamma, a.rowvec, a.rv_ld, a.row_b};
    }
    struct FfnOp { FfnForm f; Linear w1, w2; FfnArgs a; };
    FfnOp op_ffn_setup(const char* op, int mode, int M, int C, int I, const float* W1, const float* W2, int split = 0);
    void convnext(const ConvNeXt& p, const FfnForm& f, float* x, int B, int L, int C, int hid, int k, int dil, const int* len,
                  const int* conv_len = nullptr, const float* rowvec = nullptr, int rv_ld = 0, const Ragged* rg = nullptr, FoldState* fs = nullptr,
                  const DwconvTail& tl = DwconvTail() );
    void fold_layernorm(FoldState& fs, int64_t M, int C, const LNorm& ln, void* xn, const char* tag);
    void attn_block(const Attn& p, float* x, int B, int Lq, int C, int H, const void* ctx, int Lk, const int* qlen,
                    const int* klen, int rope_mode, bool self, const Ragged* qrg = nullptr);
    void* to_act(const float* src, int64_t n);

    struct ProfSpan { std::string tag; hipEvent_t a, b; double flops, bytes; };
    void prof_begin(const char* tag, double flops, double bytes);
    void prof_end();
    class StageSpan {
       public:
        StageSpan(Engine& e, const char* stage, const char* tag, double flops, double bytes) : e_(e), prev_(e.stage_) {
            e_.stage_ = stage;
            begin(tag, flops, bytes);
        }
        ~StageSpan() { end(); e_.stage_ = prev_; }
        StageSpan(const StageSpan&) = delete;
        StageSpan& operator=(const StageSpan&) = delete;
        void next(const char* tag, double flops, double bytes) { end(); begin(tag, flops, bytes); }

       private:
        void begin(const char* tag, double flops, double bytes) { if ((begun_ = e_.prof_on_)) e_.prof_begin(tag, flops, bytes); }
        void end() { if (begun_) e_.prof_end(); begun_ = false; }
        Engine& e_;
        const char* prev_;
        bool begun_ = false;
    };

    int device_, dt_;
    int n_cu_ = 256;
    hipStream_t s_ = nullptr, own_s_ = nullptr;
    const char* stage_ = "";
    std::string prof_filter_;
    std::string log_family_;
    int prof_every_ = 1;
    uint64_t prof_seen_ = 0;
    bool prof_active_ = false;
    stn_arch a_{};
    bool loaded_ = false;
    int64_t params_ = 0;
    std::unordered_map<std::string, DevTensor> w_;
// ... 243 lines not shown
```

### supertonic_amd/csrc/engine_batch.cpp

```cpp
#include "engine.hpp"
#include "engine_internal.hpp"

#include <algorithm>
#include <cmath>
#include <cstdio>
#include <cstring>

namespace stn {
using detail::up;


template <typename T>
void Engine::ensure(T*& p, size_t& cap, size_t need) {
    if (p && need <= cap) return;
    const size_t n = std::max<size_t>(need + need / 4, 64);
    T* q = nullptr;
    STN_HIP(hipMalloc(reinterpret_cast<void**>(&q), n * sizeof(T)));
    if (p) {
        batch_owned_.erase(std::find(batch_owned_.begin(), batch_owned_.end(), static_cast<void*>(p)));
        batch_retired_.push_back(p);
    }
    batch_owned_.push_back(q);
    p = q;
    cap = n;
// ... 64 lines not shown
}

static void latent_geometry(const stn_arch& a, const std::vector<float>& dur, int& L, std::vector<int>& llen) {
    const int cs = a.base_chunk_size * a.chunk_compress_factor;
    float mx = dur[0];
    for (float d : dur) mx = std::max(mx, d);
    const float wav_len_max = mx * (float)a.sample_rate;
    L = (int)((wav_len_max + (float)cs - 1.0f) / (float)cs);
    llen.resize(dur.size());
    for (size_t i = 0; i < dur.size(); ++i) {
        const int64_t wl = (int64_t)(dur[i] * (float)a.sample_rate);
        llen[i] = (int)((wl + cs - 1) / cs);
    }
}

void Engine::batch_run(int total_step, float speed, uint64_t noise_seed) {
    STN_HIP(hipSetDevice(device_));
    Batch& b = bt_;
    if (b.B == 0) throw std::runtime_error("batch_run: no batch uploaded");
    if (total_step < 1) throw std::runtime_error("total_step must be >= 1");
    if (!(speed > 0.f)) throw std::runtime_error("speed must be > 0");
    const stn_arch& a = a_;
    const int B = b.B, Lt = b.Lt, D = a.latent_dim * a.chunk_compress_factor;
    b.total_step = total_step; b.speed = speed; b.noise_seed = noise_seed;
    ar_.reset();
    Ragged trg;
    const bool tpk = packed_text_ok(B) && b.trows > 0;
    if (tpk) { trg.off = b.toff; trg.rows = b.trows; }
    std::vector<float> dur(B);
    const size_t text_bytes = (size_t)(tpk ? (int64_t)b.trows : (int64_t)B * Lt) * a.te_out_dim * (is_half(dt_) ? 2 : 4);
    ensure(b.text_side, b.text_side_cap, text_bytes);
    ensure(b.text_rows, b.text_cap, text_bytes);
    {
        struct Side {
            Engine& e; hipStream_t& s; Arena& ar; bool on;
            Side(Engine& e_, hipStream_t& s_, Arena& ar_) : e(e_), s(s_), ar(ar_), on(s_ != nullptr) { if (on) { std::swap(e.s_, s); e.ar_.swap(ar); e.ar_.reset(); } }
            ~Side() { if (on) { std::swap(e.s_, s); e.ar_.swap(ar); } }
        };
        {
            Side side(*this, te_s_, te_ar_);
            if (side.on && copied_valid_) STN_HIP(hipStreamWaitEvent(s_, ev_copied_, 0));
            text_enc_dev(B, Lt, b.ids, b.style_ttl, b.tlen, nullptr, b.text_side, tpk ? &trg : nullptr);
            STN_HIP(hipEventRecord(ev_te_, s_));
        }
        {
            Side side(*this, dp_s_, dp_ar_);
            duration_dev(B, Lt, b.ids, b.style_dp, b.tlen, b.dur, tpk ? &trg : nullptr);
            if (!b.have_override || dur_read_always_) {
                STN_HIP(hipMemcpyAsync(dur.data(), b.dur, sizeof(float) * B, hipMemcpyDeviceToHost, s_));
                STN_HIP(hipEventRecord(ev_dp_, s_));
            }
        }
        if (!b.have_override || dur_read_always_) STN_HIP(hipEventSynchronize(ev_dp_));
        if (b.have_override) dur = b.h_dur;
    }
    auto take_text_rows = [this, &b, text_bytes]() {
        if (te_s_) STN_HIP(hipStreamWaitEvent(s_, ev_te_, 0));
        STN_HIP(hipMemcpyAsync(b.text_rows, b.text_side, text_bytes, hipMemcpyDeviceToDevice, s_));
        STN_HIP(hipEventRecord(ev_copied_, s_));
        copied_valid_ = true;
    };
    for (float& d : dur) d /= speed;
    int L = 0;
    latent_geometry(a, dur, L, b.h_llen);
    if (L < 1) throw std::runtime_error("predicted duration too short: zero latent frames");
    if (shape_buckets_ && !b.have_noise) L = (int)bucket_up(L, 16);
    if (b.have_noise && b.noise_L != L)
        throw std::runtime_error("injected noise has L=" + std::to_string(b.noise_L) + " but the durations imply L=" + std::to_string(L));
    b.L = L;
    reported_dur_ = dur;
    ++ed_seq_;
    const size_t nx = (size_t)B * D * L, nw = (size_t)B * L * a.base_chunk_size * a.chunk_compress_factor;
    ensure(b.xt[0], b.xt_cap[0], nx);
    ensure(b.xt[1], b.xt_cap[1], nx);
    ensure(b.wav, b.wav_cap, nw);
    int ve_rows = 0;
    if (packed_rows_ok(B)) for (int v : b.h_llen) ve_rows += v;
    if (shape_buckets_) ve_rows = (int)bucket_up(ve_rows, 64);
    int vform = VO_DENSE;
    const int tr_rows = vocoder_rows(B, L, &vform);
    const int tab_vo = vo_ragged_ ? LEN_VO_SCALED : !tr_rows ? LEN_VO_NONE : vform == VO_TRIM_TAIL ? LEN_VO_TAIL : LEN_VO_2RF;
    const bool tab_pairs = ve_rows > 0 && fused_xattn_ && is_half(dt_) && B >= 2;
    b.tl = len_tables_layout(B, ve_rows, tab_pairs, tab_vo);
    h_tab_.assign((size_t)b.tl.total, 0);
    len_tables_build(b.tl, b.h_llen.data(), B, ve_rows, tab_pairs, tab_vo, a.chunk_compress_factor, L * a.chunk_compress_factor, vo_rf_, h_tab_.data());
    const unsigned long long seed64 = (unsigned long long)noise_seed;
    std::memcpy(h_tab_.data() + b.tl.seed, &seed64, sizeof seed64);
    ensure(b.tab, b.tab_cap, (size_t)b.tl.total);
    b.llen = b.tab + b.tl.llen;
    seed_dev_ = reinterpret_cast<unsigned long long*>(b.tab + b.tl.seed);
    if ((size_t)b.tl.total > pin_tab_cap_) {
        if (pin_tab_) { sync(); drop_graphs(); (void)hipHostFree(pin_tab_); pin_tab_ = nullptr; }
        const size_t cap = std::max<size_t>((size_t)b.tl.total + (size_t)b.tl.total / 4, (size_t)1024 * (64 + 8));
        STN_HIP(hipHostMalloc(reinterpret_cast<void**>(&pin_tab_), sizeof(int) * cap, hipHostMallocDefault));
        pin_tab_cap_ = cap;
        pin_valid_ = false;
    }
    if (!pin_valid_ || pin_tab_n_ != h_tab_.size() || !std::equal(h_tab_.begin(), h_tab_.end(), pin_tab_)) {
        sync();
        std::copy(h_tab_.begin(), h_tab_.end(), pin_tab_);
        pin_tab_n_ = h_tab_.size();
        pin_valid_ = true;
    }

    ensure_time_cond(total_step, B);
    GraphKey key;
    key.B = B; key.Lt = Lt; key.L = L; key.steps = total_step; key.noise = b.have_noise; key.ragged = vo_ragged_; key.xattn = fused_xattn_;
    key.ffn = fused_ffn_; key.gen = b.gen; key.wgen = wgen_; key.pin = pin_tab_;
    key.rows = ve_rows;
    last_ve_rows_ = key.rows ? key.rows : (int64_t)B * L;
    key.vrows = tr_rows; key.vform = vform;
    if (shape_buckets_) key.vrows = (int)bucket_up(key.vrows, 64 * a.chunk_compress_factor);
    key.trows = tpk ? b.trows : 0;
    last_vo_rows_ = (int64_t)B * L * a.chunk_compress_factor;
    if (vo_ragged_ && packed_ve_ && is_half(dt_)) {
        last_vo_rows_ = 0;
        for (int v : b.h_llen) last_vo_rows_ += (int64_t)v * a.chunk_compress_factor;
        if (shape_buckets_) last_vo_rows_ = bucket_up(last_vo_rows_, 64 * a.chunk_compress_factor);
        key.vrows = (int)last_vo_rows_;
    }
    else if (key.vrows) last_vo_rows_ = key.vrows;
    key.p0 = b.xt[0]; key.p1 = b.wav; key.s = s_;
    const bool graphable = graph_on_ && !prof_on_;
    if (graphable) {
        for (auto& g : graphs_)
            if (g.key == key) {
                g.last_use = ++graph_clock_;
                STN_HIP(hipGraphLaunch(g.exec, s_));
                take_text_rows();
                STN_HIP(hipGraphLaunch(g.exec2, s_));
                ++graph_replays_;
                return;
            }
    }
    const auto warm = std::find(warm_keys_.begin(), warm_keys_.end(), key);
    if (graphable && warm != warm_keys_.end()) {
        const Arena::Mark cap0 = ar_.mark();
        const size_t cap_before = ar_.capacity();
        STN_HIP(hipStreamBeginCapture(s_, hipStreamCaptureModeThreadLocal));
        bool ok = true;
        std::string why;
        hipGraph_t g = nullptr, g2 = nullptr;
        hipError_t ec1 = hipErrorUnknown;
        bool split = false;
        auto split_capture = [&]() {
            ec1 = hipStreamEndCapture(s_, &g);
            split = true;
            STN_HIP(hipStreamBeginCapture(s_, hipStreamCaptureModeThreadLocal));
        };
        try { enqueue_after_duration(total_step, split_capture); } catch (const std::exception& e) { ok = false; why = e.what(); }
        const hipError_t ec = hipStreamEndCapture(s_, &g2);
        text_gate_ = nullptr;
        ar_.release(cap0);
        hipGraphExec_t ex = nullptr, ex2 = nullptr;
        if (ok && split && ec1 == hipSuccess && ec == hipSuccess && g && g2 && ar_.capacity() == cap_before &&
            hipGraphInstantiate(&ex, g, nullptr, nullptr, 0) == hipSuccess && hipGraphInstantiate(&ex2, g2, nullptr, nullptr, 0) == hipSuccess) {
            if (graphs_.size() >= kGraphCache) {
                auto lru = std::min_element(graphs_.begin(), graphs_.end(), [](const GraphEntry& x, const GraphEntry& y) { return x.last_use < y.last_use; });
                sync();
                (void)hipGraphExecDestroy(lru->exec);
                (void)hipGraphDestroy(lru->graph);
                if (lru->exec2) (void)hipGraphExecDestroy(lru->exec2);
                if (lru->graph2) (void)hipGraphDestroy(lru->graph2);
                graphs_.erase(lru);
            }
            GraphEntry e;
            e.key = key; e.graph = g; e.exec = ex; e.graph2 = g2; e.exec2 = ex2; e.last_use = ++graph_clock_;
            graphs_.push_back(e);
            warm_keys_.erase(warm);
            STN_HIP(hipGraphLaunch(ex, s_));
            take_text_rows();
            STN_HIP(hipGraphLaunch(ex2, s_));
            ++graph_replays_;
            return;
        }
        if (ex) (void)hipGraphExecDestroy(ex);
        if (ex2) (void)hipGraphExecDestroy(ex2);
        if (g2) (void)hipGraphDestroy(g2);
        if (g) (void)hipGraphDestroy(g);
        (void)hipGetLastError();
        if (!ok) throw std::runtime_error("graph capture failed: " + why);
    }
    if (warm == warm_keys_.end()) {
        if (warm_keys_.size() >= kWarmKeys) warm_keys_.erase(warm_keys_.begin());
        warm_keys_.push_back(key);
    }
    enqueue_after_duration(total_step, take_text_rows);
}

void Engine::ensure_time_cond(int total_step, int B) {
    TimeCond& t = tcond_;
    if (t.steps == total_step && t.B == B && t.wgen == wgen_ && t.buf) return;
    const stn_arch& a = a_;
    const size_t n_cnt = (size_t)2 * total_step * B + (size_t)B, n_tb = (size_t)total_step * B * a.ve_main_blocks * a.ve_dim;
    const size_t need = (n_cnt + 3) / 4 * 4 + n_tb;
    if (need > t.cap) {
        sync();
        drop_graphs();
        if (t.buf) (void)hipFree(t.buf);
        t.buf = nullptr; t.cap = 0;
        STN_HIP(hipMalloc(reinterpret_cast<void**>(&t.buf), need * sizeof(float)));
        t.cap = need;
    }
    t.tot = t.buf; t.cur = t.tot + (size_t)total_step * B; t.dt = t.cur + (size_t)total_step * B; t.tb = t.buf + (n_cnt + 3) / 4 * 4;
    t.steps = 0;
    const Arena::Mark mk = ar_.mark();
    launch_step_counters(s_, t.tot, t.cur, t.dt, B, total_step);
    (void)ve_time_cond_dev(total_step * B, t.tot, t.cur, t.tb);
    ar_.release(mk);
    t.steps = total_step; t.B = B; t.wgen = wgen_;
}

void Engine::enqueue_after_duration(int total_step, const std::function<void()>& take_text_rows) {
    Batch& b = bt_;
    const stn_arch& a = a_;
    const int B = b.B, Lt = b.Lt, L = b.L, D = a.latent_dim * a.chunk_compress_factor;
    const size_t nx = (size_t)B * D * L;
    STN_HIP(hipMemcpyAsync(b.tab, pin_tab_, sizeof(int) * (size_t)b.tl.total, hipMemcpyHostToDevice, s_));
    Ragged trg;
    const bool tpk = packed_text_ok(B) && b.trows > 0;
    if (tpk) { trg.off = b.toff; trg.rows = b.trows; }
    const Ragged* trgp = tpk ? &trg : nullptr;
    void* text_rows = b.text_rows;
    if (b.have_noise) {
        STN_HIP(hipMemcpyAsync(b.xt[0], b.noise, nx * 4, hipMemcpyDeviceToDevice, s_));
        launch_mask_ncl(s_, b.xt[0], B, D, L, b.llen);
    } else {
        stage_ = "ve";
        if (prof_on_) prof_begin("noise", 0.0, (double)nx * 4.0);
        launch_randn_masked(s_, 0, b.utt_ids, B, D, L, b.llen, b.xt[0], seed_dev_);
        if (prof_on_) prof_end();
    }
    VeCtx c = ve_prepare_dev(B, Lt, text_rows, b.style_ttl, b.tlen, trgp, true);
    text_gate_ = [this, &c, &b, &take_text_rows, B, Lt, text_rows, trgp]() {
        take_text_rows();
        ve_text_kv_dev(c, B, Lt, text_rows, b.tlen, trgp);
    };
    struct Disarm { std::function<void()>& g; ~Disarm() { g = nullptr; } } disarm{text_gate_};
    if (a.ve_main_blocks == 0) { auto fire = std::move(text_gate_); text_gate_ = nullptr; fire(); }
    if (tcond_.steps != total_step || tcond_.B != B || tcond_.wgen != wgen_) throw std::runtime_error("time conditioning not prepared for this run");
    const float* tot_all = tcond_.tot;
    const float* cur_all = tcond_.cur;
    const float* dt_all = tcond_.dt;
    const float* tb_all = tcond_.tb;
    const size_t tb_stride = (size_t)B * a.ve_main_blocks * a.ve_dim;
    Ragged rg;
    const Ragged* rgp = nullptr;
    if (packed_rows_ok(B)) {
        rg.rows = 0;
        for (int v : b.h_llen) rg.rows += v;
        if (shape_buckets_) rg.rows = (int)bucket_up(rg.rows, 64);
        if (b.tl.ve_off < 0 || b.tl.ve_row_b + rg.rows > b.tl.total) throw std::logic_error("batch_run: no row map in the length tables");
        const int* off = b.tab + b.tl.ve_off;
        const int* row_b = b.tab + b.tl.ve_row_b;
        rg.off = off; rg.row_b = row_b;
        rg.fold_run = fold_run_frames(b.h_llen.data(), B, n_cu_);
        if (fused_xattn_ && is_half(dt_) && B >= 2) {
            if (b.tl.pairs < 0) throw std::logic_error("batch_run: no pairing in the length tables");
            const int* pairs = b.tab + b.tl.pairs;
            rg.hs_pairs = pairs;
        }
        rgp = &rg;
    }
    int cur = 0;
    const int Dz = (a.latent_dim * a.chunk_compress_factor + 63) / 64 * 64;
    const int64_t Mz = rgp ? (int64_t)rg.rows : (int64_t)B * L;
    void* z_rows = act_alloc(Mz * Dz);
    for (int st = 0; st < total_step; ++st) {
        ve_step_dev(B, L, c, b.xt[cur], b.tlen, b.llen, tot_all + (size_t)st * B, cur_all + (size_t)st * B, b.xt[cur ^ 1],
                    tb_all + (size_t)st * tb_stride, rgp, dt_all, z_rows, st > 0, st + 1 < total_step);
        cur ^= 1;
    }
    final_xt_ = cur;
    const int* vlen = nullptr;
    if (vo_ragged_) vlen = b.tab + b.tl.vo_n;
    int vrows = 0;
    const int* valid = nullptr;
    bool tails = false;
    if (vo_ragged_ && packed_ve_) {
        for (int v : b.h_llen) vrows += v * a.chunk_compress_factor;
        if (shape_buckets_) vrows = (int)bucket_up(vrows, 64 * a.chunk_compress_factor);
    } else if (int vform = VO_DENSE; int tr = vocoder_rows(B, L, &vform)) {
        if (shape_buckets_) tr = (int)bucket_up(tr, 64 * a.chunk_compress_factor);
        vlen = b.tab + b.tl.vo_n; valid = b.tab + b.tl.vo_valid; vrows = tr; tails = vform == VO_TRIM_TAIL;
    }
    if (vlen && b.tl.vo_n < 0) throw std::logic_error("batch_run: no vocoder extents in the length tables");
    vocoder_dev(B, L, b.xt[cur], b.wav, vlen, vrows, valid, tails, vlen ? b.tab + b.tl.vo_off : nullptr);
    STN_HIP(hipGetLastError());
}


char* DevBuf::reserve(Engine& e, size_t bytes, bool* moved) {
    const bool grow = !p_ || bytes > cap_;
    if (moved) *moved = grow;
    if (!grow) return p_;
    e.sync();
    if (p_) (void)hipFree(p_);
    p_ = nullptr; cap_ = 0;
    STN_HIP(hipMalloc(reinterpret_cast<void**>(&p_), bytes + bytes / 4));
    cap_ = bytes + bytes / 4;
    return p_;
}

void* DeviceTable::put(Engine& e, const void* host, size_t bytes) {
    void* p = nullptr;
    STN_HIP(hipMalloc(&p, bytes));
    STN_HIP(hipMemcpyAsync(p, host, bytes, hipMemcpyHostToDevice, e.stream()));
    e.sync();
    if (p_) (void)hipFree(p_);
    return p_ = p;
}

int64_t Engine::out_row_len() {
    STN_HIP(hipSetDevice(device_));
    const Batch& b = bt_;
    if (!b.wav || b.L == 0) throw std::runtime_error("no finished batch");
    return out_len(native_row_len());
}

bool Engine::out_native() const { return !pitch_on() && !loudness_on() && !out_in_scratch(); }

const float* Engine::out_source(int64_t Wo) {
    const Batch& b = bt_;
    const float* wav = wav_rows();
    if (!out_in_scratch()) return wav;
    float* d = out_f32_buf((size_t)b.B * Wo);
    const float* cur = wav;
    if (resample_on()) { resample_enqueue(rs_table(), cur, b.B, native_row_len(), ENC_F32, d, Wo); cur = d; }
    if (filter_on()) { fl_batch(cur, Wo, d); cur = d; }
    if (expander_on()) { xp_batch(cur, Wo, d); cur = d; }
    if (deesser_on()) { ds_batch(cur, Wo, d); cur = d; }
    if (compressor_on()) { cp_batch(cur, Wo, d); cur = d; }
    return d;
}

RowsId Engine::rows_id(Stage stage, int64_t Wo) const {
    const uint64_t gen[] = {ps_gen_, 0, fl_gen_, xp_.gen, ds_.gen, cp_.gen};
    static_assert(sizeof(gen) / sizeof(gen[0]) == N_STAGES, "one generation per stage of the chain");
    RowsId id{ed_seq_, output_rate(), Wo, {}};
// ... 450 lines not shown
```

### supertonic_amd/csrc/engine_ops.cpp

```cpp
#include "engine.hpp"
#include "engine_internal.hpp"

#include <algorithm>
#include <cmath>
#include <cstdio>
#include <cstring>

namespace stn {
using detail::up;

void Engine::op_gemm(int dtype, int M, int N, int K, const float* A, const float* W, const float* bias, int act, float* out) {
    STN_HIP(hipSetDevice(device_));
    ar_.reset();
    float* dA = up(ar_, s_, A, (size_t)M * K);
    float* dW = up(ar_, s_, W, (size_t)N * K);
    float* dB = bias ? up(ar_, s_, bias, (size_t)N) : nullptr;
    float* dO = f32_alloc((size_t)M * N);
    const void* pa = dA;
    const void* pw = dW;
    if (is_half(dtype)) {
        void* a16 = ar_.alloc((size_t)M * K * 2);
        void* w16 = ar_.alloc((size_t)N * K * 2);
        launch_cast(s_, dtype, dA, (int64_t)M * K, a16);
        launch_cast(s_, dtype, dW, (int64_t)N * K, w16);
// ... 336 lines not shown
    float* d_x = up(ar_, s_, x, (size_t)M * C);
    fa.xn = xn16; fa.x = d_x; fa.b1 = up(ar_, s_, b1, (size_t)I); fa.b2 = b2 ? up(ar_, s_, b2, (size_t)C) : nullptr;
    fa.gamma = gamma ? up(ar_, s_, gamma, (size_t)C) : nullptr;
    fa.rowvec = rowvec ? up(ar_, s_, rowvec, (size_t)nseq * C) : nullptr; fa.rv_ld = C;
    fa.row_b = (rowvec && row_b) ? up(ar_, s_, row_b, (size_t)M) : nullptr;
    FoldArgs fo = ffn_launch(op.f, C, fa, op.w1, op.w2);
    if (op.f.kind == FFN_K4_SPLIT) {
        float *ones = f32_alloc(C), *zeros = f32_alloc(C);
        launch_fill(s_, ones, C, 1.f); launch_fill(s_, zeros, C, 0.f);
        if (!fo.b2) fo.b2 = zeros;
        if (!fo.gamma) fo.gamma = ones;
        void* y = act_alloc((int64_t)M * C);
        launch_fold_ln(s_, dt_, d_x, M, C, fo, ones, ones, a_.ln_eps, y);
    }
    STN_HIP(hipGetLastError());
    STN_HIP(hipMemcpyAsync(x, d_x, sizeof(float) * (size_t)M * C, hipMemcpyDeviceToHost, s_));
    sync();
}

void Engine::op_ffn_bench(int M, int C, int I, int mode, int iters, double* out5) {
    STN_HIP(hipSetDevice(device_));
    ar_.reset();
    for (int i = 0; i < 5; ++i) out5[i] = 0.0;
    float* rnd = f32_alloc((int64_t)M * C);
    launch_randn_masked(s_, 11, nullptr, 1, M, C, nullptr, rnd);
    float* wr = f32_alloc((int64_t)I * C);
    launch_randn_masked(s_, 12, nullptr, 1, I, C, nullptr, wr);
    launch_scale(s_, wr, I * C, 0.05f);
    FfnOp op = op_ffn_setup("op_ffn_bench", mode, M, C, I, wr, wr);
    void* xn16 = act_alloc((int64_t)M * C);
    launch_cast(s_, dt_, rnd, (int64_t)M * C, xn16);
    float* d_b1 = f32_alloc(I);
    float* d_b2 = f32_alloc(C);
    float* d_g = f32_alloc(C);
    launch_fill(s_, d_b1, I, 0.01f); launch_fill(s_, d_b2, C, 0.01f); launch_fill(s_, d_g, C, 0.1f);
    float* d_x = f32_alloc((int64_t)M * C);
    STN_HIP(hipMemsetAsync(d_x, 0, sizeof(float) * (size_t)M * C, s_));
    op.a.xn = xn16; op.a.b1 = d_b1; op.a.b2 = d_b2; op.a.gamma = d_g; op.a.x = d_x;
    const int S = op.f.split;
    const int nslab = (M + 127) / 128;
    const int nwg = S > 1 ? (nslab + 7) / 8 * 8 * S : nslab;
    unsigned long long* ts = static_cast<unsigned long long*>(ar_.alloc(sizeof(unsigned long long) * 4 * (size_t)nwg));
    auto run = [&](unsigned long long* stamps) { op.a.ts = stamps; ffn_launch(op.f, C, op.a, op.w1, op.w2); };
    for (int i = 0; i < 3; ++i) run(nullptr);
    hipEvent_t a, b;
    STN_HIP(hipEventCreate(&a)); STN_HIP(hipEventCreate(&b));
    STN_HIP(hipEventRecord(a, s_));
    for (int i = 0; i < iters; ++i) run(nullptr);
    STN_HIP(hipEventRecord(b, s_));
    STN_HIP(hipEventSynchronize(b));
    float ms = 0.f;
    STN_HIP(hipEventElapsedTime(&ms, a, b));
    (void)hipEventDestroy(a); (void)hipEventDestroy(b);
    out5[0] = ms / iters;
    if (op.f.kind != FFN_GEMMS) {
        STN_HIP(hipMemsetAsync(ts, 0, sizeof(unsigned long long) * 4 * (size_t)nwg, s_));
        run(ts);
        std::vector<unsigned long long> h((size_t)4 * nwg);
        STN_HIP(hipMemcpyAsync(h.data(), ts, sizeof(unsigned long long) * h.size(), hipMemcpyDeviceToHost, s_));
        sync();
        double s1 = 0, s2 = 0, s3 = 0;
        int live = 0;
        for (int w = 0; w < nwg; ++w) {
            if (!h[4 * w + 3]) continue;
            ++live;
            s1 += (double)(h[4 * w + 1] - h[4 * w]); s2 += (double)(h[4 * w + 2] - h[4 * w + 1]); s3 += (double)(h[4 * w + 3] - h[4 * w + 2]);
        }
        if (live) { out5[1] = s1 / live; out5[2] = s2 / live; out5[3] = s3 / live; }
        out5[4] = live;
    }
    STN_HIP(hipGetLastError());
    sync();
}

void Engine::op_fold_dwconv_ln(int B, int C, int k, int dil, int S, const int* seqlen, const float* x, const float* part, const float* b2,
                               const float* gamma, const float* rowvec, const float* w, const float* bias, const float* g, const float* b,
                               float* x_out, float* y) {
    if (!is_half(dt_)) throw std::invalid_argument("op_fold_dwconv_ln: 16-bit engines only");
    int L = 0;
    int64_t M = 0;
    for (int i = 0; i < B; ++i) { M += seqlen[i]; L = std::max(L, seqlen[i]); }
    std::fill(x_out, x_out + M * C, 0.f);
    std::fill(y, y + M * C, 0.f);
    op_fold_dwconv_ln_ex(dt_, B, L, C, k, dil, S, 0, seqlen, x, M, part, M * C, M * C * S, b2, gamma, rowvec, C, w, bias, g, b, x_out, M, y, M);
}

void Engine::op_block_bench(int B, int L, int C, int I, int k, int dil, int mode, int iters, double* out2) {
    STN_HIP(hipSetDevice(device_));
    ar_.reset();
    for (int i = 0; i < 6; ++i) out2[i] = 0.0;
    const int64_t M = (int64_t)B * L;
    float* wr = f32_alloc((int64_t)I * C);
    launch_randn_masked(s_, 12, nullptr, 1, I, C, nullptr, wr);
    launch_scale(s_, wr, I * C, 0.05f);
    FfnOp op = op_ffn_setup("op_block_bench", mode, (int)M, C, I, wr, wr);
    std::vector<int> len(B, L), off(B + 1);
    for (int i = 0; i <= B; ++i) off[i] = i * L;
    const int* dlen = up(ar_, s_, len.data(), (size_t)B);
    const int* doff = up(ar_, s_, off.data(), (size_t)B + 1);
    float* xa = f32_alloc(M * C);
    float* xb = f32_alloc(M * C);
    launch_randn_masked(s_, 11, nullptr, 1, (int)M, C, nullptr, xa);
    float* d_b1 = f32_alloc(I);
    float* d_b2 = f32_alloc(C);
    float* d_g = f32_alloc(C);
    float* d_one = f32_alloc(C);
    float* dwt = f32_alloc((int64_t)k * C);
    launch_fill(s_, d_b1, I, 0.01f); launch_fill(s_, d_b2, C, 0.01f); launch_fill(s_, d_g, C, 0.01f); launch_fill(s_, d_one, C, 1.f);
    launch_fill(s_, dwt, k * C, 1.f / k);
    void* xn = act_alloc(M * C);
    op.a.xn = xn; op.a.b1 = d_b1; op.a.b2 = d_b2; op.a.gamma = d_g;
    const bool split = op.f.kind == FFN_K4_SPLIT;
    if (split) STN_HIP(hipMemsetAsync(op.a.part, 0, (size_t)op.a.part_stride * op.f.split * 2, s_));
    FoldArgs fo = ffn_pending(op.f, op.a);
    auto conv = [&]() {
        if (split) { launch_fold_dwconv_ln(s_, dt_, xa, xb, B, L, C, fo, dwt, d_b2, k, dil, d_one, d_b2, 1e-6f, xn, dlen, doff); std::swap(xa, xb); }
        else launch_dwconv_ln(s_, dt_, xa, B, L, C, dwt, d_b2, k, dil, d_one, d_b2, 1e-6f, xn, dlen, doff);
    };
    auto block = [&]() { conv(); op.a.x = xa; ffn_launch(op.f, C, op.a, op.w1, op.w2); };
    hipEvent_t a, b;
    STN_HIP(hipEventCreate(&a)); STN_HIP(hipEventCreate(&b));
    for (int which = 0; which < 2; ++which) {
        for (int i = 0; i < 3; ++i) { if (which) conv(); else block(); }
        STN_HIP(hipEventRecord(a, s_));
        for (int i = 0; i < iters; ++i) { if (which) conv(); else block(); }
        STN_HIP(hipEventRecord(b, s_));
        STN_HIP(hipEventSynchronize(b));
        float ms = 0.f;
        STN_HIP(hipEventElapsedTime(&ms, a, b));
        out2[which] = ms / iters;
    }
    (void)hipEventDestroy(a); (void)hipEventDestroy(b);
    if (split) {
        const int nwg = B * ((L + 7) / 8);
        unsigned long long* ts = static_cast<unsigned long long*>(ar_.alloc(sizeof(unsigned long long) * 4 * (size_t)nwg));
        STN_HIP(hipMemsetAsync(ts, 0, sizeof(unsigned long long) * 4 * (size_t)nwg, s_));
        fo.ts = ts;
        conv();
        fo.ts = nullptr;
        std::vector<unsigned long long> h((size_t)4 * nwg);
        STN_HIP(hipMemcpyAsync(h.data(), ts, sizeof(unsigned long long) * h.size(), hipMemcpyDeviceToHost, s_));
        sync();
        double p1 = 0, p2 = 0, p3 = 0; int live = 0;
        unsigned long long tmin = ~0ull, tmax = 0;
        for (int w = 0; w < nwg; ++w) {
            if (!h[4 * w + 3]) continue;
            ++live;
            p1 += (double)(h[4 * w + 1] - h[4 * w]); p2 += (double)(h[4 * w + 2] - h[4 * w + 1]); p3 += (double)(h[4 * w + 3] - h[4 * w + 2]);
            tmin = std::min(tmin, h[4 * w]); tmax = std::max(tmax, h[4 * w + 3]);
        }
        if (live) { out2[2] = p1 / live; out2[3] = p2 / live; out2[4] = p3 / live; out2[5] = (double)(tmax - tmin); }
    }
    STN_HIP(hipGetLastError());
    sync();
}

static void down_as(Arena& ar, hipStream_t s, int dtype, const void* d, float* h, size_t n) {
    const float* src = static_cast<const float*>(d);
    if (is_half(dtype)) {
        float* w = static_cast<float*>(ar.alloc(n * 4));
        launch_half_to_f32(s, dtype, d, (int64_t)n, w);
        src = w;
    }
    STN_HIP(hipMemcpyAsync(h, src, n * 4, hipMemcpyDeviceToHost, s));
}

std::string Engine::op_ffn_ex(int M, int C, int I, const float* xn, int ldx, int64_t xn_elems, const float* W1, const float* b1, const float* W2,
// ... 2 lines not shown
    STN_HIP(hipSetDevice(device_));
    ar_.reset();
    float* d_w1 = up(ar_, s_, W1, (size_t)I * C);
    float* d_w2 = up(ar_, s_, W2, (size_t)C * I);
    FfnOp op = op_ffn_setup("op_ffn_ex", mode, M, C, I, d_w1, d_w2, split);
    FfnArgs& fa = op.a;
    fa.xn = up_as(ar_, s_, dt_, xn, (size_t)xn_elems); fa.ldx = ldx;
    float* d_x = up(ar_, s_, x, (size_t)x_elems);
    fa.x = d_x; fa.ldo = ldo;
    fa.b1 = up(ar_, s_, b1, (size_t)I);
    fa.b2 = b2 ? up(ar_, s_, b2, (size_t)C) : nullptr;
    fa.gamma = gamma ? up(ar_, s_, gamma, (size_t)C) : nullptr;
    fa.rowvec = rowvec ? up(ar_, s_, rowvec, (size_t)nseq * rv_ld) : nullptr; fa.rv_ld = rv_ld;
    fa.row_b = row_b ? up(ar_, s_, row_b, (size_t)M) : nullptr;
    fa.len = len ? up(ar_, s_, len, (size_t)nseq) : nullptr; fa.L = L;
    void* d_part = nullptr;
    if (op.f.kind == FFN_K4_SPLIT) {
        d_part = up_as(ar_, s_, dt_, part, (size_t)part_elems);
        fa.part = d_part; fa.part_stride = part_stride;
    }
    ffn_launch(op.f, C, fa, op.w1, op.w2);
    STN_HIP(hipGetLastError());
    STN_HIP(hipMemcpyAsync(x, d_x, sizeof(float) * (size_t)x_elems, hipMemcpyDeviceToHost, s_));
    if (d_part) down_as(ar_, s_, dt_, d_part, part, (size_t)part_elems);
    sync();
    return op.f.str();
}

std::string Engine::op_dwconv_ln_ex(int dtype, int B, int L, int C, int k, int dil, const float* x, int64_t x_rows, const float* w,
                                    const float* bias, const float* g, const float* b, const int* seqlen, int packed, int ln_only, float* y,
                                    int64_t y_rows, const float* tail, int T, int rf) {
    STN_HIP(hipSetDevice(device_));
    ar_.reset();
    const int* dlen = seqlen ? up(ar_, s_, seqlen, (size_t)B) : nullptr;
    float* dx = up(ar_, s_, x, (size_t)x_rows * C);
    float* dg = up(ar_, s_, g, (size_t)C);
    float* dbt = up(ar_, s_, b, (size_t)C);
    void* dy = up_as(ar_, s_, dtype, y, (size_t)y_rows * C);
    std::string form = "layernorm";
    if (ln_only) {
        launch_layernorm(s_, dtype, dx, (int64_t)B * L, C, dg, dbt, 1e-6f, dy);
    } else {
        std::vector<float> wt((size_t)C * k);
        for (int c = 0; c < C; ++c) for (int j = 0; j < k; ++j) wt[(size_t)j * C + c] = w[(size_t)c * k + j];
        float* dw = up(ar_, s_, wt.data(), wt.size());
        float* db = up(ar_, s_, bias, (size_t)C);
        int* off = nullptr;
        if (packed) {
            off = static_cast<int*>(ar_.alloc(sizeof(int) * (size_t)(B + 1)));
            launch_row_map(s_, dlen, B, off, nullptr);
        }
        DwconvTail tl;
        if (tail) { tl.tail = up(ar_, s_, tail, (size_t)(rf + 1) * C); tl.T = T; tl.rf = rf; }
        form = dwconv_ln_form(dtype, B, L, C, k, packed != 0).str();
        launch_dwconv_ln(s_, dtype, dx, B, L, C, dw, db, k, dil, dg, dbt, 1e-6f, dy, dlen, off, tl);
    }
    STN_HIP(hipGetLastError());
    down_as(ar_, s_, dtype, dy, y, (size_t)y_rows * C);
    sync();
    return form;
}

void Engine::op_fold_ln(int dtype, int M, int C, int S, const float* part, const float* b2, const float* gamma, const float* rowvec,
                        const int* row_b, int nseq, const float* g, const float* b, float* x, float* y) {
    STN_HIP(hipSetDevice(device_));
    ar_.reset();
    const size_t n = (size_t)M * C;
    FoldArgs fo;
    fo.part = up_as(ar_, s_, dtype, part, n * S); fo.S = S; fo.part_stride = (int64_t)n;
    fo.b2 = up(ar_, s_, b2, (size_t)C); fo.gamma = up(ar_, s_, gamma, (size_t)C);
    fo.rowvec = rowvec ? up(ar_, s_, rowvec, (size_t)nseq * C) : nullptr; fo.rv_ld = C;
    fo.row_b = (rowvec && row_b) ? up(ar_, s_, row_b, (size_t)M) : nullptr;
    float* dx = up(ar_, s_, x, n);
    float* dg = up(ar_, s_, g, (size_t)C);
    float* dbt = up(ar_, s_, b, (size_t)C);
    void* dy = ar_.alloc(n * 2);
    launch_fold_ln(s_, dtype, dx, M, C, fo, dg, dbt, 1e-6f, dy);
    STN_HIP(hipGetLastError());
    STN_HIP(hipMemcpyAsync(x, dx, n * 4, hipMemcpyDeviceToHost, s_));
    down_as(ar_, s_, dtype, dy, y, n);
    sync();
}

std::string Engine::op_fold_dwconv_ln_ex(int dtype, int B, int L, int C, int k, int dil, int S, int run_frames, const int* seqlen, const float* x_in,
                                         int64_t x_rows, const float* part, int64_t part_stride, int64_t part_elems, const float* b2, const float* gamma,
                                         const float* rowvec, int rv_ld, const float* w, const float* bias, const float* g, const float* b, float* x_out,
                                         int64_t x_out_rows, float* y, int64_t y_rows) {
    STN_HIP(hipSetDevice(device_));
    ar_.reset();
    std::vector<float> wt((size_t)C * k);
    for (int c = 0; c < C; ++c) for (int j = 0; j < k; ++j) wt[(size_t)j * C + c] = w[(size_t)c * k + j];
    const int* dlen = up(ar_, s_, seqlen, (size_t)B);
    int* doff = static_cast<int*>(ar_.alloc(sizeof(int) * (size_t)(B + 1)));
    launch_row_map(s_, dlen, B, doff, nullptr);
    float* dx = up(ar_, s_, x_in, (size_t)x_rows * C);
    float* dxo = up(ar_, s_, x_out, (size_t)x_out_rows * C);
    void* dy = up_as(ar_, s_, dtype, y, (size_t)y_rows * C);
    float* dw = up(ar_, s_, wt.data(), wt.size());
    float* db = up(ar_, s_, bias, (size_t)C);
    float* dg = up(ar_, s_, g, (size_t)C);
    float* dbt = up(ar_, s_, b, (size_t)C);
    FoldArgs fo;
    fo.part = up_as(ar_, s_, dtype, part, (size_t)part_elems); fo.S = S; fo.part_stride = part_stride;
    if (b2) fo.b2 = up(ar_, s_, b2, (size_t)C);
    else { float* z = f32_alloc(C); launch_fill(s_, z, C, 0.f); fo.b2 = z; }
    if (gamma) fo.gamma = up(ar_, s_, gamma, (size_t)C);
    else { float* o = f32_alloc(C); launch_fill(s_, o, C, 1.f); fo.gamma = o; }
    fo.rowvec = rowvec ? up(ar_, s_, rowvec, (size_t)B * rv_ld) : nullptr; fo.rv_ld = rowvec ? rv_ld : C;
    fo.run_frames = run_frames;
    const std::string form = fold_dwconv_ln_form(dtype, B, L, C, k, dil, S, rowvec != nullptr, run_frames).str();
    launch_fold_dwconv_ln(s_, dtype, dx, dxo, B, L, C, fo, dw, db, k, dil, dg, dbt, 1e-6f, dy, dlen, doff);
    STN_HIP(hipGetLastError());
    STN_HIP(hipMemcpyAsync(x_out, dxo, sizeof(float) * (size_t)x_out_rows * C, hipMemcpyDeviceToHost, s_));
    down_as(ar_, s_, dtype, dy, y, (size_t)y_rows * C);
    sync();
    return form;
}

void Engine::op_layout(int which, int dtype, const int* p, const float* a, int64_t a_n, const float* b, int64_t b_n, const float* c, int64_t c_n,
                       const int64_t* ids, int64_t ids_n, const int* len, int packed, float* out, int64_t out_n, float* out2, int64_t out2_n,
                       int* iout, int64_t iout_n) {
    STN_HIP(hipSetDevice(device_));
    ar_.reset();
    auto need = [](bool ok, const char* what) { if (!ok) throw std::invalid_argument(std::string("stn_op_layout: ") + what); };
    auto rows_needed = [&](int B, int rows_per_seq) -> int64_t {
        if (!packed) return (int64_t)B * rows_per_seq;
        int64_t t = 0;
        for (int i = 0; i < B; ++i) t += len[i];
        return t;
    };
    auto check_len = [&](int B, int hi, bool required) {
        need(B > 0 && B <= 1024, "1 <= B <= 1024");
        need(len || !(required || packed), "lengths needed");
        if (len) for (int i = 0; i < B; ++i) need(len[i] >= 0 && len[i] <= hi, "a length outside [0, rows per sequence]");
    };
    auto row_off = [&](const int* dlen, int B) -> int* {
        if (!packed) return nullptr;
        int* off = static_cast<int*>(ar_.alloc(sizeof(int) * (size_t)(B + 1)));
        launch_row_map(s_, dlen, B, off, nullptr);
        return off;
    };
    switch (which) {
    case 0: {
        const int B = p[0], rows_padded = p[1], with_b = p[2];
        need(B > 0 && len && iout && rows_padded >= 0, "row_map: B > 0, lengths and iout needed");
        if (B > 1024) { launch_row_map(s_, nullptr, B, nullptr, nullptr); return; }
        int64_t tot = 0;
        for (int i = 0; i < B; ++i) { need(len[i] >= 0 && len[i] < (1 << 20), "row_map: length out of range"); tot += len[i]; }
        need(iout_n >= B + 1 + (with_b ? std::max<int64_t>(tot, rows_padded) : 0), "row_map: iout too small");
        const int* dlen = up(ar_, s_, len, (size_t)B);
        int* d = up(ar_, s_, iout, (size_t)iout_n);
        launch_row_map(s_, dlen, B, d, with_b ? d + B + 1 : nullptr, rows_padded);
        STN_HIP(hipMemcpyAsync(iout, d, (size_t)iout_n * 4, hipMemcpyDeviceToHost, s_));
        break;
    }
    case 1: {
        const int B = p[0], C = p[1], L = p[2], ldo = p[3];
        need(C > 0 && L > 0 && ldo >= C && a && out, "ncl_to_rows: bad shape");
        check_len(B, L, false);
        need(a_n >= (int64_t)B * C * L && out_n >= rows_needed(B, L) * ldo, "ncl_to_rows: buffer too small");
        const int* dlen = len ? up(ar_, s_, len, (size_t)B) : nullptr;
        float* da = up(ar_, s_, a, (size_t)a_n);
        void* d = up_as(ar_, s_, dtype, out, (size_t)out_n);
        launch_ncl_to_rows(s_, dtype, da, B, C, L, d, ldo, dlen, row_off(dlen, B));
        down_as(ar_, s_, dtype, d, out, (size_t)out_n);
        break;
    }
    case 2: {
        const int B = p[0], D = p[1], L = p[2], with_z = p[3], ldz = p[4];
        need(D > 0 && L > 0 && a && b && c && out && (!with_z || (out2 && ldz >= D)), "euler_ncl: bad shape");
        check_len(B, L, false);
        const int64_t vr = rows_needed(B, L);
        need(a_n >= (int64_t)B * D * L && out_n >= (int64_t)B * D * L && c_n >= B && b_n >= vr * D && (!with_z || out2_n >= vr * ldz), "euler_ncl: buffer too small");
        const int* dlen = len ? up(ar_, s_, len, (size_t)B) : nullptr;
        float* dp = up(ar_, s_, a, (size_t)a_n);
        float* dv = up(ar_, s_, b, (size_t)b_n);
        float* ddt = up(ar_, s_, c, (size_t)c_n);
        float* d = up(ar_, s_, out, (size_t)out_n);
        void* dz = with_z ? up_as(ar_, s_, dtype, out2, (size_t)out2_n) : nullptr;
        launch_euler_ncl(s_, dp, dv, ddt, dlen, B, D, L, d, row_off(dlen, B), dz, dtype, ldz);
        STN_HIP(hipMemcpyAsync(out, d, (size_t)out_n * 4, hipMemcpyDeviceToHost, s_));
        if (dz) down_as(ar_, s_, dtype, dz, out2, (size_t)out2_n);
        break;
    }
    case 3: {
        const int B = p[0], T = p[1], W = p[2];
        need(T > 0 && W > 0 && W % 4 == 0 && a && out, "unpack_rows: bad shape");
        packed = 1;
        check_len(B, T, true);
        need(a_n >= rows_needed(B, T) * W && a_n > 0 && out_n >= (int64_t)B * T * W, "unpack_rows: buffer too small");
        const int* dlen = up(ar_, s_, len, (size_t)B);
        float* da = up(ar_, s_, a, (size_t)a_n);
        float* d = up(ar_, s_, out, (size_t)out_n);
// ... 110 lines not shown
```

### supertonic_amd/csrc/kernels.hpp

```cpp
#pragma once
#include <hip/hip_runtime.h>
#include <hip/hip_ext.h>
#include <stdint.h>
#include <stdio.h>
#include <stdlib.h>

#include <stdexcept>
#include <type_traits>
#include <utility>
#include <vector>
#include <string>

#include "dither.hpp"

namespace stn {

struct LaunchEvents { hipEvent_t start = nullptr, stop = nullptr; };
inline thread_local LaunchEvents g_launch_ev;
struct LaunchLog {
    bool on = false;
    const char* family = "-";
    std::vector<std::pair<std::string, const char*>> entries;
    void add(const char* kexpr) { if (entries.size() < 200000) entries.emplace_back(family, kexpr); }
};
// ... 43 lines not shown
};

struct Epilogue {
    int mode = EPI_STORE;
    int act = ACT_NONE;
    int out_dtype = F32;
    const float* bias = nullptr;
    void* out = nullptr;
    int ldo = 0;
    const float* gamma = nullptr;
    float* resid = nullptr;
    const int* len = nullptr;
    int L = 1;
    const int* row_b = nullptr;
    const float* rowvec = nullptr;
    int rv_ld = 0;
    const int* map_off = nullptr;
    const int* map_valid = nullptr;
    int map_B = 0, map_T = 0;
    int ksplit = 1;
    int nt = 0;
    int tr_epilogue = 0;
    int tr_force = -1;
    unsigned long long* ts = nullptr;
};

enum GemmKernel : int { GK_TILED = 0, GK_RING_VEC = 1, GK_RING = 2, GK_REG = 3 };
enum GemmEpiForm : int { GE_LANE = 0, GE_SLAB = 1, GE_TR = 2 };
constexpr int GEMM_CFG_F32_64 = 19, GEMM_CFG_F32_128 = 20;
struct GemmForm {
    int dtype = F32, mode = EPI_STORE;
    int kernel = GK_REG;
    int cfg = 0;
    int bm = 128, bn = 128, wm = 2, wn = 2, nstage = 2, ks = 64, esz = 2;
    int epi = GE_LANE;
    int tr_epilogue = 0;
    int split = 1;
    std::string str() const;
};
GemmForm gemm_form(int dtype, int M, int N, int K, int lda, int ldw, const Epilogue& e, const void* A, const void* W, bool allow_split = true);
void launch_gemm_form(hipStream_t s, const GemmForm& f, const void* A, int lda, const void* W, int ldw, int M, int N, int K,
                      const Epilogue& e, float* workspace);
bool gemm_form_maps_rows(const GemmForm& f);
void launch_gemm(hipStream_t s, int dtype, const void* A, int lda, const void* W, int ldw, int M, int N, int K,
                 const Epilogue& e);
int gemm_splitk_factor(int dtype, int M, int N, int K, const Epilogue& e);
void launch_gemm_splitk(hipStream_t s, int dtype, const void* A, int lda, const void* W, int ldw, int M, int N, int K, const Epilogue& e,
                        int S, float* workspace);

struct FfnArgs {
    const void* xn = nullptr; int ldx = 0;
    const void* wseq = nullptr;
    const float* b1 = nullptr;
    const float* b2 = nullptr;
    const float* gamma = nullptr;
    float* x = nullptr; int ldo = 0;
    int M = 0, I = 0;
    const int* row_b = nullptr;
    const float* rowvec = nullptr; int rv_ld = 0;
    const int* len = nullptr; int L = 1;
    unsigned long long* ts = nullptr;
    int split = 1;
    void* part = nullptr;
    int64_t part_stride = 0;
};
bool ffn_fused_supported(int dtype, int C, int I);
int ffn_split_factor(int dtype, int C, int I);
constexpr int FFN_SPLITS[] = {4, 8, 12};
bool ffn_split_valid(int dtype, int C, int I, int S);
int ffn_split_choose(int dtype, int C, int I, int64_t M);
inline int64_t ffn_split_rows(int64_t M) { return (M + 127) / 128 * 128; }
enum FfnKind : int { FFN_GEMMS = 0, FFN_K4 = 1, FFN_K4_SPLIT = 2 };
enum FfnStage : int { FFN_VOCODER = 1, FFN_ESTIMATOR = 2, FFN_TEXT = 4 };
struct FfnForm {
    int kind = FFN_GEMMS, split = 1;
    bool nt = false;
    std::string str() const;
};
FfnForm ffn_form(int dtype, int stage, int C, int I, int64_t M, int64_t gate_rows, bool packed, int k, int max_dil, int mask, int64_t min_rows,
                 int64_t split_min_rows, bool nt_hints);
__host__ __device__ constexpr inline int ffn_lds_side_offset(int C, int I) { return (4 * C * 64 + (I + 2 * C) * 4 + 1023) & ~1023; }
__host__ __device__ constexpr inline bool ffn_lds_has_side(int C) { return C == 384; }
void launch_ffn_fused(hipStream_t s, int dtype, int C, const FfnArgs& a);
struct FoldArgs {
    const void* part = nullptr; int S = 0; int64_t part_stride = 0;
    const float* b2 = nullptr;
    const float* gamma = nullptr;
    const float* rowvec = nullptr; int rv_ld = 0;
    const int* row_b = nullptr;
    unsigned long long* ts = nullptr;
    int run_frames = 0;
};
int fold_run_frames(const int* lengths, int B, int n_cu);
void launch_fold_ln(hipStream_t s, int act_dtype, float* x, int64_t M, int C, const FoldArgs& f, const float* g, const float* b, float eps, void* y);
bool fold_dwconv_ln_supported(int C, int k, int dil);
struct FoldDwconvLnForm {
    int act_dtype = BF16, K = 5, nslot = 3, S = 4, U = 1, run = 32, cps = 1;
    bool rv = false;
    unsigned grid = 0;
    size_t lds = 0;
    std::string str() const;
};
FoldDwconvLnForm fold_dwconv_ln_form(int act_dtype, int B, int L, int C, int k, int dil, int S, bool has_rowvec, int run_frames);
void launch_fold_dwconv_ln(hipStream_t s, int act_dtype, const float* x_in, float* x_out, int B, int L, int C, const FoldArgs& f, const float* w_t,
                           const float* bias, int k, int dil, const float* ln_g, const float* ln_b, float eps, void* y, const int* seqlen,
                           const int* row_off);
void launch_repack_frag_acc(hipStream_t s, const void* W, int N, int K, void* Wf);
void launch_ffn_pack(hipStream_t s, const void* W1, const void* W2, int C, int I, void* tmp, void* wseq, int S = 1);

struct DwconvTail {
    const float* tail = nullptr;
    int T = 0, rf = 0;
};
void launch_dwconv_ln(hipStream_t s, int out_dtype, const float* x, int B, int L, int C, const float* w_t,
                      const float* bias, int k, int dil, const float* ln_g, const float* ln_b, float eps, void* y,
                      const int* seqlen = nullptr, const int* row_off = nullptr, const DwconvTail& tl = DwconvTail());
enum DwconvLnKernel : int { DW_V3 = 0, DW_V2 = 1, DW_GENERIC = 2 };
struct DwconvLnForm {
    int out_dtype = F32;
    int kernel = DW_GENERIC;
    int K = 0, R = 1;
    bool occ4 = false;
    std::string str() const;
};
DwconvLnForm dwconv_ln_form(int out_dtype, int B, int L, int C, int k, bool packed);
bool dwconv_ln_supports_packed(int C, int k);
void launch_row_map(hipStream_t s, const int* len, int B, int* row_off , int* row_b ,
                    int rows_padded = 0 );
constexpr int LN_NI = 4;
void check_ln_shape(int C);
void launch_layernorm(hipStream_t s, int out_dtype, const float* x, int64_t M, int C, const float* g, const float* b,
                      float eps, void* y);

enum AttnVec : int { ATTN_VEC_Q = 1, ATTN_VEC_K = 2, ATTN_VEC_V = 4 };
struct AttnForm {
    int dtype = F32;
    bool mfma = false;
    int dh = 0;
    int kc = 0, nch = 0;
    int tpr = 8, vec = 0;
    size_t lds = 0;
    std::string str() const;
};
AttnForm attn_form(int dtype, int B, int Lq, int Lk, int H, int dh, int ldq, int ldk, const void* q, const void* k, const void* v);
void launch_attention(hipStream_t s, int dtype, const void* q, int ldq, const void* k, const void* v, int ldk, void* o,
                      int ldo, int B, int Lq, int Lk, int H, int dh, const int* qlen, const int* klen, int rope_mode,
                      float rope_base, float rope_gamma, bool k_rotated = false,
                      const int* q_off = nullptr ,
                      const int* k_off = nullptr );
void launch_repack_frag(hipStream_t s, const void* W, int N, int K, void* Wf);
bool xattn_hs_supported(int dtype, int C, int H, int L, int Lk, int ldk);
void launch_xattn_hs(hipStream_t s, int dtype, const void* xn, int64_t M, const void* WqF, const float* bq, const void* kp, const void* vp, int ldk,
                     const void* WoA, void* part, int64_t part_stride, int B, int L, int Lk, const int* qlen, const int* klen,
                     const int* q_off, const int* k_off, int rope_mode, float rope_base, float rope_gamma, unsigned long long* ts = nullptr,
                     const int* pairs = nullptr );
struct XattnHsForm {
    bool f16 = false;
    int U = 1, kc = 32;
    size_t lds = 0;
    std::string str() const;
};
XattnHsForm xattn_hs_form(int dtype, int C, int H, int B, int L, int Lk, int ldk);
void launch_xattn_hs_pairs(hipStream_t s, const int* qlen, int B, int* pairs);
void launch_rope_rows(hipStream_t s, int dtype, void* x, int ld, int B, int L, const int* len, int groups, int group_stride,
                      int H, int dh, int rope_mode, float rope_base, float rope_gamma, const int* row_off = nullptr );

void launch_embed(hipStream_t s, const int64_t* ids, const float* emb, int vocab, int B, int L, int C, const int* len,
                  float* x, const int* row_off = nullptr );
void launch_mask_to_len(hipStream_t s, const float* mask, int B, int L, int* len);
void launch_ncl_to_rows(hipStream_t s, int out_dtype, const float* in, int B, int C, int L, void* out, int ld_out = 0,
                        const int* len = nullptr, const int* row_off = nullptr );
void launch_euler_ncl(hipStream_t s, const float* prev, const float* v, const float* dt, const int* len, int B, int D, int L, float* out,
                      const int* row_off = nullptr , void* z_rows = nullptr, int z_dtype = 0, int ldz = 0);
void launch_cast(hipStream_t s, int out_dtype, const float* in, int64_t n, void* out);
void launch_add_rowvec(hipStream_t s, float* x, const float* v, int ldv, int B, int L, int C, const int* len);
void launch_time_embed(hipStream_t s, const float* cur, const float* tot, int B, int dim, float scale, float* te);
void launch_scale_len(hipStream_t s, const int* len, int B, int factor, int* out);
void launch_vocoder_in(hipStream_t s, const float* latent, int B, int L, int ld, int ccf, const float* w ,
                       const float* bias, int C, int k, float* x, const int* seqlen = nullptr);
void launch_vocoder_im2col(hipStream_t s, int out_dtype, const float* latent, int B, int L, int ld, int ccf, int k, int kp, void* cols,
                           const int* seqlen = nullptr ,
                           const int* row_off = nullptr );
void launch_fill_rows(hipStream_t s, const int* valid, int B, int T, int W, int rf, const float* quiet, const float* edge, float* dst);
void launch_unpack_rows(hipStream_t s, const float* src, const int* len, const int* row_off, int B, int T, int W, float* dst);
void launch_trim_len(hipStream_t s, const int* len, int B, int ccf, int T, int rf, int* n_out, int* valid_out, bool tail_form = false);
void launch_unpack_rows_quiet(hipStream_t s, const float* src, const int* valid, const int* row_off, int B, int T, int W, int rf,
                              const float* quiet, const float* edge, float* dst);
void launch_masked_mean(hipStream_t s, int in_dtype, const void* x, int B, int L, int C, const int* len, float* pooled,
                        const int* row_off = nullptr );
// ... 172 lines not shown
```

### supertonic_amd/csrc/kernels_fold.hip

```cpp
#include "kernels.hpp"
#include "kernels_dev.hpp"
#include "dev_env.hpp"
#include "kernels_fold.hpp"

#include <type_traits>
#include <stdio.h>
#include <stdlib.h>

namespace stn {

template <typename OutT, bool F16, bool RV, int S>
__global__ __launch_bounds__(256) void fold_ln_kernel(float* __restrict__ x, int64_t M, int C, const uint16_t* __restrict__ part,
                                                      int64_t pstride, const float* __restrict__ b2, const float* __restrict__ gamma,
                                                      const float* __restrict__ rowvec, int rv_ld, const int* __restrict__ row_b,
                                                      const float* __restrict__ g, const float* __restrict__ bt, float eps, OutT* __restrict__ y) {
    const int lane = threadIdx.x & 63;
    const int64_t row = (int64_t)blockIdx.x * 4 + (threadIdx.x >> 6);
    if (row >= M) return;
    const int C4 = C >> 2;
    float4* x4 = reinterpret_cast<float4*>(x) + row * C4;
    const float4* rv4 = nullptr;
    if constexpr (RV) rv4 = reinterpret_cast<const float4*>(rowvec + (size_t)(row_b ? row_b[row] : 0) * rv_ld);
    const float4* b24 = reinterpret_cast<const float4*>(b2);
    const float4* gm4 = reinterpret_cast<const float4*>(gamma);
// ... 162 lines not shown
            }
#pragma unroll
            for (int u = 0; u < U; ++u) {
                const int r = r0 + u * rpp;
                if (r < nw) {
                    float4* sp4 = reinterpret_cast<float4*>(fold_sm + (size_t)r * C + c8 * 8);
                    sp4[0] = fold_four(xa[u][0], acc[u], bb0, gm0, tv0);
                    sp4[1] = fold_four(xa[u][1], acc[u] + 4, bb1, gm1, tv1);
                }
            }
        }
    }
#pragma unroll
    for (int i = 0; i < NPV; ++i) {
        const int q = tid + i * FOLD_NT;
        if (q < (K + 3) * C4) reinterpret_cast<float4*>(wsm)[q] = pv[i];
    }
    if (tid < C4) reinterpret_cast<float4*>(zrow)[tid] = make_float4(0.f, 0.f, 0.f, 0.f);
    if (ts) st1 = __builtin_readcyclecounter();
    __syncthreads();
    if (ts) st2 = __builtin_readcyclecounter();
    const int lane = tid & 63, l32 = lane & 31;
    const float4* ws4 = reinterpret_cast<const float4*>(wsm);
    for (int tp = t0; tp < t1; tp += FOLD_TCH) {
    asm volatile("" ::: "memory");
    const int t = tp + 2 * (tid >> 6) + (lane >> 5);
    const bool live = t < t1;
    const int tl = live ? t : t0;
    float4 h[FOLD_NSLOT];
#pragma unroll
    for (int i = 0; i < FOLD_NSLOT; ++i) {
        const int c4 = l32 + 32 * i, cq = c4 < C4 ? c4 : 0;
        float4 a = ws4[K * C4 + cq];
#pragma unroll
        for (int j = 0; j < K; ++j) {
            const int tt = tl + (j - HALF) * dil;
            const bool in = tt >= 0 && tt < Lv;
            const float4 xv = *reinterpret_cast<const float4*>((in ? fold_sm + (size_t)(tt - w0) * C : zrow) + cq * 4);
            const float4 wv = ws4[j * C4 + cq];
            a.x = fmaf(wv.x, xv.x, a.x); a.y = fmaf(wv.y, xv.y, a.y);
            a.z = fmaf(wv.z, xv.z, a.z); a.w = fmaf(wv.w, xv.w, a.w);
        }
        h[i] = c4 < C4 ? a : make_float4(0.f, 0.f, 0.f, 0.f);
    }
    float s = 0.f;
#pragma unroll
    for (int i = 0; i < FOLD_NSLOT; ++i) s += (h[i].x + h[i].y) + (h[i].z + h[i].w);
    const float mean = half_wave_sum(s) * inv_c;
    float v = 0.f;
#pragma unroll
    for (int i = 0; i < FOLD_NSLOT; ++i)
        if (l32 + 32 * i < C4) {
            const float dx = h[i].x - mean, dy = h[i].y - mean, dz = h[i].z - mean, dw = h[i].w - mean;
            v += (dx * dx + dy * dy) + (dz * dz + dw * dw);
        }
    const float rstd = rsqrtf(half_wave_sum(v) * inv_c + eps);
    if (live) {
#pragma unroll
        for (int i = 0; i < FOLD_NSLOT; ++i) {
            const int c4 = l32 + 32 * i;
            if (c4 < C4) {
                const float4 gg = ws4[(K + 1) * C4 + c4], bb = ws4[(K + 2) * C4 + c4];
                store4(y + (row0 + t) * C + c4 * 4, (h[i].x - mean) * rstd * gg.x + bb.x, (h[i].y - mean) * rstd * gg.y + bb.y,
                       (h[i].z - mean) * rstd * gg.z + bb.z, (h[i].w - mean) * rstd * gg.w + bb.w);
            }
        }
    }
    }
    if (rq < rpp)
        for (int r = rq; r < nw; r += rpp) {
            const int tt = w0 + r;
            if (tt >= t0 && tt < t1) {
                const float4* sp4 = reinterpret_cast<const float4*>(fold_sm + (size_t)r * C + c8 * 8);
                float4* op = reinterpret_cast<float4*>(xout + (row0 + tt) * C + c8 * 8);
                op[0] = sp4[0]; op[1] = sp4[1];
            }
        }
    if (ts && tid == 0) {
        unsigned long long* tp = ts + (size_t)blockIdx.x * 4;
        tp[0] = st0; tp[1] = st1; tp[2] = st2; tp[3] = __builtin_readcyclecounter();
    }
}

int fold_run_frames(const int* lengths, int B, int n_cu) {
    if (!lengths || B <= 0 || n_cu <= 0) return 0;
    int Lmax = 0;
    for (int i = 0; i < B; ++i) Lmax = std::max(Lmax, lengths[i]);
    if ((long)B * ((Lmax + FOLD_TCH - 1) / FOLD_TCH) <= n_cu) return 0;
    for (int tch = FOLD_TCH + 8; tch <= FOLD_TCH_MAX; tch += 8)
        if ((long)B * ((Lmax + tch - 1) / tch) <= n_cu) return tch;
    return 0;
}

static size_t fold_dwconv_lds(int C, int k, int dil, int tch = FOLD_TCH) { return ((size_t)(tch + (k - 1) * dil) + 1 + (size_t)(k + 3)) * C * 4; }
bool fold_dwconv_ln_supported(int C, int k, int dil) {
    return C % 8 == 0 && C <= 512 && (k == 5 || k == 7) && dil >= 1 && fold_dwconv_lds(C, k, dil) <= 160 * 1024;
}

std::string FoldDwconvLnForm::str() const {
    char m_[96];
    snprintf(m_, sizeof m_, "fold_dwconv_ln<%s,K%d,%s,ns%d,S%d,U%d> run %d cps %d", act_dtype == F16 ? "f16" : "bf16", K, rv ? "rv" : "norv", nslot, S, U, run, cps);
    return m_;
}

static FoldDwconvLnForm fold_dwconv_ln_form_forced(int act_dtype, int B, int L, int C, int k, int dil, int S, bool has_rowvec, int run_frames, int force) {
    if (!is_half(act_dtype) || B < 1 || L < 1 || !fold_dwconv_ln_supported(C, k, dil) || (S != 4 && S != 8 && S != 12 && S != 24) ||
        (int64_t)B * ((L + FOLD_TCH_FEW - 1) / FOLD_TCH_FEW) > 0x7FFFFFFFll)
        throw std::invalid_argument("fold_dwconv_ln: 16-bit format, k in {5,7}, C % 8 == 0, C <= 512, 4, 8, 12 or 24 splits and an image within 160 KiB of LDS needed");
    FoldDwconvLnForm f;
    f.act_dtype = act_dtype; f.K = k; f.rv = has_rowvec; f.S = S;
    f.nslot = C <= 384 ? 3 : 4;
    f.U = fold_phase1_rows(S, k, f.nslot);
    int tch = force == FOLD_TCH || force == FOLD_TCH_FEW ? force : (int64_t)B * ((L + FOLD_TCH - 1) / FOLD_TCH) < 64 ? FOLD_TCH_FEW : FOLD_TCH;
    if ((force == 40 || force == 48) && fold_dwconv_lds(C, k, dil, force) <= 160 * 1024) tch = force;
    if (!force && tch == FOLD_TCH && run_frames > FOLD_TCH && run_frames <= FOLD_TCH_MAX && run_frames % 8 == 0 && fold_dwconv_lds(C, k, dil, run_frames) <= 160 * 1024)
        tch = run_frames;
    f.run = tch;
    f.cps = (L + tch - 1) / tch;
    f.grid = (unsigned)((int64_t)B * f.cps);
    f.lds = fold_dwconv_lds(C, k, dil, tch);
    return f;
}
FoldDwconvLnForm fold_dwconv_ln_form(int act_dtype, int B, int L, int C, int k, int dil, int S, bool has_rowvec, int run_frames) {
    return fold_dwconv_ln_form_forced(act_dtype, B, L, C, k, dil, S, has_rowvec, run_frames, 0);
}

template <typename OutT, int K, bool RV, int NSLOT, int S>
static void launch_fold_dwconv_ln_one(hipStream_t s, const FoldDwconvLnForm& fm, const float* x_in, float* x_out, int C, const FoldArgs& f, const float* w_t,
                                      const float* bias, int dil, const float* g, const float* b, float eps, OutT* y, const int* seqlen, const int* row_off) {
    constexpr bool F16 = std::is_same<OutT, f16_t>::value;
    static PerDeviceOnce attr_once;
    if (attr_once.need())
        stn_check_hip(hipFuncSetAttribute(reinterpret_cast<const void*>(&fold_dwconv_ln_kernel<OutT, F16, K, RV, NSLOT, S>), hipFuncAttributeMaxDynamicSharedMemorySize,
                                          160 * 1024), "hipFuncSetAttribute(fold_dwconv_ln)");
    if (fm.K != K || fm.rv != RV || fm.nslot != NSLOT || fm.S != S || fm.U != fold_phase1_rows(S, K, NSLOT)) throw std::logic_error("fold_dwconv_ln: no kernel for form " + fm.str());
    STN_KLAUNCH((fold_dwconv_ln_kernel<OutT, F16, K, RV, NSLOT, S>), dim3(fm.grid), dim3(FOLD_NT), fm.lds, s, x_in, x_out, fm.cps, C,
                static_cast<const uint16_t*>(f.part), f.part_stride, f.b2, f.gamma, f.rowvec, f.rv_ld, w_t, bias, dil, g, b, eps, 1.0f / (float)C, y, seqlen, row_off, f.ts, fm.run);
}

void launch_fold_dwconv_ln(hipStream_t s, int act_dtype, const float* x_in, float* x_out, int B, int L, int C, const FoldArgs& f, const float* w_t,
                           const float* bias, int k, int dil, const float* ln_g, const float* ln_b, float eps, void* y, const int* seqlen,
                           const int* row_off) {
    if (B == 0 || L == 0) return;
    if (!is_half(act_dtype) || !seqlen || !row_off || x_in == x_out || !fold_dwconv_ln_supported(C, k, dil) ||
        (int64_t)B * ((L + FOLD_TCH_FEW - 1) / FOLD_TCH_FEW) > 0x7FFFFFFFll)
        throw std::invalid_argument("launch_fold_dwconv_ln: packed 16-bit rows, separate output, k in {5,7}, C % 8 == 0, C <= 512 needed");
    check_fold_args(f, 0, C, "launch_fold_dwconv_ln");
    static const int force = [] { const char* e = stn::dev_env("STN_FOLD_TCH"); return e ? atoi(e) : 0; }();
    const FoldDwconvLnForm fm = fold_dwconv_ln_form_forced(act_dtype, B, L, C, k, dil, f.S, f.rowvec != nullptr, f.run_frames, force);
    bool found = false;
    with_half_type(act_dtype, [&](auto* tag) {
    with_const<5, 7>(fm.K, [&](auto K) {
    with_const<0, 1>(fm.rv, [&](auto rv) {
    with_const<3, 4>(fm.nslot, [&](auto ns) {
    found = with_const<4, 8, 12, 24>(fm.S, [&](auto S) {
        using T = std::remove_pointer_t<decltype(tag)>;
        launch_fold_dwconv_ln_one<T, K(), rv() != 0, ns(), S()>(s, fm, x_in, x_out, C, f, w_t, bias, dil, ln_g, ln_b, eps, static_cast<T*>(y), seqlen, row_off);
    }); }); }); }); });
    if (!found) throw std::logic_error("fold_dwconv_ln: no kernel for form " + fm.str());
}

}
```

### supertonic_amd/csrc/kernels_fold.hpp

```cpp
#pragma once
#include <hip/hip_runtime.h>
#include <stdint.h>

namespace stn {

template <bool F16>
__device__ __forceinline__ float p16_to_f(unsigned h) {
    if constexpr (F16) { const _Float16 v = __builtin_bit_cast(_Float16, (uint16_t)h); return (float)v; }
    else return __uint_as_float(h << 16);
}
template <bool F16, int N, int CH, bool FIRST>
__device__ __forceinline__ void fold_chunk(const uint16_t* __restrict__ p16, int64_t pstride, int s0, float (&acc)[N]) {
    unsigned w[CH][N / 2];
#pragma unroll
    for (int c = 0; c < CH; ++c) {
        const uint16_t* q = p16 + (size_t)(s0 + c) * pstride;
        if constexpr (N == 8) { const uint4 u = *reinterpret_cast<const uint4*>(q); w[c][0] = u.x; w[c][1] = u.y; w[c][2] = u.z; w[c][3] = u.w; }
        else { const uint2 u = *reinterpret_cast<const uint2*>(q); w[c][0] = u.x; w[c][1] = u.y; }
    }
#pragma unroll
    for (int c = 0; c < CH; ++c)
#pragma unroll
        for (int j = 0; j < N / 2; ++j) {
            const float lo = p16_to_f<F16>(w[c][j] & 0xFFFFu), hi = p16_to_f<F16>(w[c][j] >> 16);
            if (FIRST && c == 0) { acc[2 * j] = lo; acc[2 * j + 1] = hi; }
            else { acc[2 * j] += lo; acc[2 * j + 1] += hi; }
        }
}
template <bool F16, int N, int S>
__device__ __forceinline__ void fold_sum(const uint16_t* __restrict__ p16, int64_t pstride, float (&acc)[N]) {
    constexpr int CH = S <= 12 ? S : 12;
    static_assert(S % CH == 0, "split count");
    fold_chunk<F16, N, CH, true>(p16, pstride, 0, acc);
#pragma unroll
    for (int s0 = CH; s0 < S; s0 += CH) fold_chunk<F16, N, CH, false>(p16, pstride, s0, acc);
}
__device__ __forceinline__ float fold_one(float x, float y, float b2, float gm, float rv) { return x + gm * (y + b2) + rv; }
__device__ __forceinline__ float4 fold_four(float4 x, const float* acc, float4 b2, float4 gm, float4 rv) {
    return make_float4(fold_one(x.x, acc[0], b2.x, gm.x, rv.x), fold_one(x.y, acc[1], b2.y, gm.y, rv.y), fold_one(x.z, acc[2], b2.z, gm.z, rv.z),
                       fold_one(x.w, acc[3], b2.w, gm.w, rv.w));
}


__device__ __forceinline__ float dpp_add(float v, int ctrl_sel) {
    const int iv = __float_as_int(v);
    int o;
    switch (ctrl_sel) {
        case 0: o = __builtin_amdgcn_update_dpp(0, iv, 0xB1, 0xF, 0xF, true); break;
        case 1: o = __builtin_amdgcn_update_dpp(0, iv, 0x4E, 0xF, 0xF, true); break;
        case 2: o = __builtin_amdgcn_update_dpp(0, iv, 0x141, 0xF, 0xF, true); break;
        default: o = __builtin_amdgcn_update_dpp(0, iv, 0x140, 0xF, 0xF, true); break;
    }
    return v + __int_as_float(o);
}
__device__ __forceinline__ float half_wave_sum(float v) {
    v = dpp_add(v, 0); v = dpp_add(v, 1); v = dpp_add(v, 2); v = dpp_add(v, 3);
    return v + __int_as_float(__builtin_amdgcn_ds_swizzle(__float_as_int(v), 0x401F));
}


}
```

Before: 48240.

## Add packed-run fold_dwconv_ln kernel that tiles ragged rows evenly across CUs

```diff
diff --git a/include/stn.h b/include/stn.h
--- a/include/stn.h
+++ b/include/stn.h
@@ -346,6 +346,13 @@
                              const float* b2_or_null, const float* gamma_or_null, const float* rowvec_or_null, int rv_ld,
                              const float* w , const float* bias, const float* ln_g, const float* ln_b, float* x_out, int64_t x_out_rows,
                              float* y, int64_t y_rows, char* form, size_t form_cap);
+int stn_op_fold_dwconv_ln_runs(stn_handle* h, int dtype, int B, int L, int C, int k, int dil, int S, int n_cu, const int32_t* seqlen,
+                               const float* x_in, int64_t x_rows, const float* part, int64_t part_stride, int64_t part_elems,
+                               const float* b2_or_null, const float* gamma_or_null, const float* rowvec_or_null, int rv_ld,
+                               const float* w , const float* bias, const float* ln_g, const float* ln_b, float* x_out, int64_t x_out_rows,
+                               float* y, int64_t y_rows, char* form, size_t form_cap);
+int64_t stn_dbg_fold_runs(const int32_t* lengths, int B, int rows, int n_cu, int k, int dil, int32_t* shape3, int32_t* table, int32_t* windows,
+                          int32_t* taps);
 int stn_dbg_fold_dwconv_ln_form(int dtype, int B, int L, int C, int k, int dil, int S, int has_rowvec, int run_frames, char* out, size_t cap);
 int stn_op_block_bench(stn_handle* h, int B, int L, int C, int I, int k, int dil, int mode, int iters, double* out6);
 int stn_op_randn(stn_handle* h, uint64_t seed, int B, int D, int L, const int64_t* utt_ids_or_null,
diff --git a/supertonic_amd/binding.py b/supertonic_amd/binding.py
--- a/supertonic_amd/binding.py
+++ b/supertonic_amd/binding.py
@@ -568,6 +568,9 @@
     L.stn_op_fold_dwconv_ln_ex.argtypes = [vp, ci, ci, ci, ci, ci, ci, ci, ci, _i32p, _f32p, ctypes.c_int64, _f32p, ctypes.c_int64, ctypes.c_int64, vp, vp,
                                            vp, ci, _f32p, _f32p, _f32p, _f32p, _f32p, ctypes.c_int64, _f32p, ctypes.c_int64, ctypes.c_char_p,
                                            ctypes.c_size_t]
+    L.stn_op_fold_dwconv_ln_runs.argtypes = L.stn_op_fold_dwconv_ln_ex.argtypes
+    L.stn_dbg_fold_runs.argtypes = [_i32p, ci, ci, ci, ci, ci, ctypes.c_void_p, ctypes.c_void_p, ctypes.c_void_p, ctypes.c_void_p]
+    L.stn_dbg_fold_runs.restype = ctypes.c_int64
     L.stn_dbg_fold_dwconv_ln_form.argtypes = [ci, ci, ci, ci, ci, ci, ci, ci, ci, ctypes.c_char_p, ctypes.c_size_t]
     L.stn_dbg_fold_dwconv_ln_form.restype = ctypes.c_int
     L.stn_op_block_bench.argtypes = [vp, ci, ci, ci, ci, ci, ci, ci, ci, ctypes.POINTER(ctypes.c_double)]
@@ -1217,6 +1220,21 @@
     return res
 
 
+def fold_runs(lengths, rows=None, n_cu=256, k=5, dil=1):
+    lengths = _c(lengths, np.int32)
+    rows = int(lengths.sum()) if rows is None else int(rows)
+    sh = np.zeros(3, np.int32)
+    n = load().stn_dbg_fold_runs(lengths, len(lengths), rows, int(n_cu), int(k), int(dil), sh.ctypes.data, None, None, None)
+    if n < 0:
+        raise StnError(int(n), "stn_dbg_fold_runs: bad argument")
+    table = np.full(n, -12345, np.int32)
+    windows = np.full(2 * int(sh[1]), -12345, np.int32)
+    taps = np.full(int(lengths.sum()) * int(k), -12345, np.int32)
+    assert load().stn_dbg_fold_runs(lengths, len(lengths), rows, int(n_cu), int(k), int(dil), sh.ctypes.data, table.ctypes.data, windows.ctypes.data,
+                                    taps.ctypes.data) == n
+    return dict(R=int(sh[0]), grid=int(sh[1]), rounds=int(sh[2]), table=table.reshape(-1, 4), windows=windows.reshape(-1, 2), taps=taps.reshape(-1, int(k)))
+
+
 def fold_dwconv_ln_form(dtype, B, L, C, k, dil, S, rowvec=True, run_frames=0):
     buf = ctypes.create_string_buffer(96)
     r = load().stn_dbg_fold_dwconv_ln_form(_DTYPES[dtype], int(B), int(L), int(C), int(k), int(dil), int(S), int(bool(rowvec)), int(run_frames),
@@ -2164,6 +2182,24 @@
                                                     _c(b, np.float32), xo.reshape(-1), xo.shape[0], yo.reshape(-1), yo.shape[0], form, ctypes.sizeof(form)))
         return xo, yo, form.value.decode()
 
+    def op_fold_dwconv_ln_runs(self, seqlen, L, x_in, part, part_stride, S, b2, gamma, rowvec, w, bias, g, b, dil, x_out, y, n_cu=256, dtype=None):
+        seqlen = _c(seqlen, np.int32)
+        x_in = _c(x_in, np.float32)
+        part = _c(part, np.float32).reshape(-1)
+        xo = np.array(x_out, dtype=np.float32, order="C", copy=True)
+        yo = np.array(y, dtype=np.float32, order="C", copy=True)
+        C = x_in.shape[1]
+        w = _c(w, np.float32)
+        _b2, b2p = _opt(b2, np.float32)
+        _g, gp = _opt(gamma, np.float32)
+        _v, vp_ = _opt(rowvec, np.float32)
+        form = ctypes.create_string_buffer(112)
+        self._ck(self._lib.stn_op_fold_dwconv_ln_runs(self._h, self.dtype if dtype is None else _DTYPES[dtype], len(seqlen), int(L), C, w.shape[1], int(dil),
+                                                      int(S), int(n_cu), seqlen, x_in.reshape(-1), x_in.shape[0], part, int(part_stride), part.size,
+                                                      b2p, gp, vp_, C if _v is None else _v.shape[1], w, _c(bias, np.float32), _c(g, np.float32),
+                                                      _c(b, np.float32), xo.reshape(-1), xo.shape[0], yo.reshape(-1), yo.shape[0], form, ctypes.sizeof(form)))
+        return xo, yo, form.value.decode()
+
     def op_block_bench(self, B, L, C, I, k, dil, mode, iters=20):
         out = (ctypes.c_double * 6)()
         self._ck(self._lib.stn_op_block_bench(self._h, B, L, C, I, k, dil, mode, iters, out))
diff --git a/supertonic_amd/csrc/api.cpp b/supertonic_amd/csrc/api.cpp
--- a/supertonic_amd/csrc/api.cpp
+++ b/supertonic_amd/csrc/api.cpp
@@ -8,6 +8,7 @@
 #include <string>
 
 #include "engine.hpp"
+#include "kernels_fold.hpp"
 #include "host/json_min.hpp"
 #include "host/graph_bind.hpp"
 #include "host/onnx_reader.hpp"
@@ -1213,11 +1214,11 @@
                  need(tot > 0, "stn_op_fold_dwconv_ln: no rows");
                  h->eng->op_fold_dwconv_ln(B, C, k, dil, S, seqlen, x, part, b2, gamma, rowvec, w, bias, g, b, x_out, y); })
 }
-static void fold_dwconv_ln_ex_checked(stn_handle* h, int dtype, int B, int L, int C, int k, int dil, int S, int run_frames, const int32_t* seqlen,
+static void fold_dwconv_ln_ex_checked(stn_handle* h, int dtype, int B, int L, int C, int k, int dil, int S, int run_frames, int n_cu, const int32_t* seqlen,
                                       const float* x_in, int64_t x_rows, const float* part, int64_t part_stride, int64_t part_elems, const float* b2,
                                       const float* gamma, const float* rowvec, int rv_ld, const float* w, const float* bias, const float* g,
                                       const float* b, float* x_out, int64_t x_out_rows, float* y, int64_t y_rows, char* form, size_t form_cap) {
-    const char* who = "stn_op_fold_dwconv_ln_ex";
+    const char* who = n_cu ? "stn_op_fold_dwconv_ln_runs" : "stn_op_fold_dwconv_ln_ex";
     auto req = [&](bool ok, const char* what) { need(ok, (std::string(who) + ": " + what).c_str()); };
     req(B > 0 && L > 0 && C > 0 && seqlen && x_in && part && w && bias && g && b && x_out && y, "bad argument");
     req(dtype == STN_DTYPE_BF16 || dtype == STN_DTYPE_F16, "a 16-bit format needed");
@@ -1228,10 +1229,11 @@
     for (int i = 0; i < B; ++i) { req(seqlen[i] >= 0 && seqlen[i] <= L, "seqlen out of [0, L]"); tot += seqlen[i]; }
     req(tot > 0, "no rows");
     req(tot * C * 2 < 0x7FFFFFFFll, "too many rows");
+    if (n_cu) req(n_cu > 0 && S != 24 && x_rows * C * 2 < 0x7FFFFFFFll, "n_cu >= 1, 4, 8 or 12 splits and x_rows * C * 2 < 2^31 needed");
     req(x_rows >= tot && x_out_rows >= tot && y_rows >= tot, "x_in / x_out / y hold fewer rows than the launch addresses");
     req(part_stride >= tot * C && part_stride % 8 == 0 && part_elems >= (int64_t)(S - 1) * part_stride + tot * C, "part smaller than the launch addresses, or a stride that is no multiple of 8");
     req(!rowvec || (rv_ld >= C && rv_ld % 4 == 0), "rv_ld >= C, a multiple of 4, needed");
-    const std::string f = h->eng->op_fold_dwconv_ln_ex(dtype, B, L, C, k, dil, S, run_frames, seqlen, x_in, x_rows, part, part_stride, part_elems, b2, gamma,
+    const std::string f = h->eng->op_fold_dwconv_ln_ex(dtype, B, L, C, k, dil, S, run_frames, n_cu, seqlen, x_in, x_rows, part, part_stride, part_elems, b2, gamma,
                                                        rowvec, rv_ld, w, bias, g, b, x_out, x_out_rows, y, y_rows);
     if (form && form_cap) std::snprintf(form, form_cap, "%s", f.c_str());
 }
@@ -1239,8 +1241,37 @@
                              const float* x_in, int64_t x_rows, const float* part, int64_t part_stride, int64_t part_elems, const float* b2,
                              const float* gamma, const float* rowvec, int rv_ld, const float* w, const float* bias, const float* g, const float* b,
                              float* x_out, int64_t x_out_rows, float* y, int64_t y_rows, char* form, size_t form_cap) {
-    STN_TRY(h, fold_dwconv_ln_ex_checked(h, dtype, B, L, C, k, dil, S, run_frames, seqlen, x_in, x_rows, part, part_stride, part_elems, b2, gamma, rowvec,
+    STN_TRY(h, fold_dwconv_ln_ex_checked(h, dtype, B, L, C, k, dil, S, run_frames, 0, seqlen, x_in, x_rows, part, part_stride, part_elems, b2, gamma, rowvec,
                                          rv_ld, w, bias, g, b, x_out, x_out_rows, y, y_rows, form, form_cap))
+}
+int stn_op_fold_dwconv_ln_runs(stn_handle* h, int dtype, int B, int L, int C, int k, int dil, int S, int n_cu, const int32_t* seqlen,
+                               const float* x_in, int64_t x_rows, const float* part, int64_t part_stride, int64_t part_elems, const float* b2,
+                               const float* gamma, const float* rowvec, int rv_ld, const float* w, const float* bias, const float* g, const float* b,
+                               float* x_out, int64_t x_out_rows, float* y, int64_t y_rows, char* form, size_t form_cap) {
+    STN_TRY(h, { need(n_cu > 0, "stn_op_fold_dwconv_ln_runs: n_cu >= 1 needed");
+                 fold_dwconv_ln_ex_checked(h, dtype, B, L, C, k, dil, S, 0, n_cu, seqlen, x_in, x_rows, part, part_stride, part_elems, b2, gamma, rowvec,
+                                           rv_ld, w, bias, g, b, x_out, x_out_rows, y, y_rows, form, form_cap); })
+}
+int64_t stn_dbg_fold_runs(const int32_t* lengths, int B, int rows, int n_cu, int k, int dil, int32_t* shape3, int32_t* table, int32_t* windows, int32_t* taps) {
+    if (!lengths || B < 1 || rows < 1 || n_cu < 1 || (k != 5 && k != 7) || dil < 1) return STN_ERR_INVALID;
+    int64_t live = 0;
+    for (int i = 0; i < B; ++i) { if (lengths[i] < 0) return STN_ERR_INVALID; live += lengths[i]; }
+    if (live > rows) return STN_ERR_INVALID;
+    const stn::FoldRunsShape sh = stn::fold_runs_shape(rows, n_cu);
+    if (shape3) { shape3[0] = sh.R; shape3[1] = sh.grid; shape3[2] = sh.rounds; }
+    if (!table) return (int64_t)4 * sh.grid;
+    stn::fold_runs_build(lengths, B, rows, n_cu, table);
+    const int reach = (k - 1) / 2 * dil;
+    if (windows)
+        for (int i = 0; i < sh.grid; ++i) {
+            windows[2 * i] = windows[2 * i + 1] = i * sh.R;
+            if (table[4 * i] > i * sh.R) stn::fold_run_window(i * sh.R, table[4 * i], table[4 * i + 1], table[4 * i + 2], reach, windows[2 * i], windows[2 * i + 1]);
+        }
+    if (taps)
+        for (int b = 0, s = 0; b < B; s += lengths[b++])
+            for (int t = s; t < s + lengths[b]; ++t)
+                for (int j = 0; j < k; ++j) taps[(int64_t)t * k + j] = stn::fold_run_tap(t, (j - (k - 1) / 2) * dil, s, s + lengths[b]);
+    return (int64_t)4 * sh.grid;
 }
 int stn_dbg_fold_dwconv_ln_form(int dtype, int B, int L, int C, int k, int dil, int S, int has_rowvec, int run_frames, char* out, size_t cap) {
     std::string f;
diff --git a/supertonic_amd/csrc/engine.cpp b/supertonic_amd/csrc/engine.cpp
--- a/supertonic_amd/csrc/engine.cpp
+++ b/supertonic_amd/csrc/engine.cpp
@@ -522,6 +522,7 @@
     if (fs && fs->pending) {
         if (prof_on_) prof_begin("fold_dwconv_ln", (double)M * C * (2.0 * k + 8 + 2.0 * fs->fold.S), (double)M * C * (8.0 + 2.0 + 2.0 * fs->fold.S));
         fs->fold.run_frames = rg->fold_run;
+        fs->fold.runs = rg->fold_runs ? FoldRuns{rg->fold_runs, rg->row_b, rg->rows, n_cu_} : FoldRuns{};
         launch_fold_dwconv_ln(s_, dt_, fs->x, fs->x_alt, B, L, C, fs->fold, p.dw_t, p.dw_b, k, dil, p.ln.g, p.ln.b, a_.ln_eps, xn, len, rg->off);
         if (prof_on_) prof_end();
         std::swap(fs->x, fs->x_alt);
diff --git a/supertonic_amd/csrc/engine.hpp b/supertonic_amd/csrc/engine.hpp
--- a/supertonic_amd/csrc/engine.hpp
+++ b/supertonic_amd/csrc/engine.hpp
@@ -183,7 +183,8 @@
     void ensure_time_cond(int total_step, int B);
     struct Ragged { const int* off = nullptr; const int* row_b = nullptr; int rows = 0;
                     const int* hs_pairs = nullptr;
-                    int fold_run = 0; };
+                    int fold_run = 0;
+                    const int* fold_runs = nullptr; };
     void ve_step_dev(int B, int L, const VeCtx& c, const float* noisy, const int* tlen, const int* llen,
                      const float* total_step, const float* current_step, float* denoised, const float* tb = nullptr,
                      const Ragged* rg = nullptr, const float* dt = nullptr ,
@@ -225,6 +226,7 @@
         float* style_dp = nullptr; size_t dp_cap = 0;
         float* dur = nullptr; size_t dur_cap = 0;
         int* llen = nullptr;
+        int tab_runs = -1; int tab_words = 0;
         int* tab = nullptr; size_t tab_cap = 0;
         LenTables tl;
         int64_t* utt_ids = nullptr; size_t utt_cap = 0;
@@ -472,7 +474,7 @@
     void op_fold_dwconv_ln(int B, int C, int k, int dil, int S, const int* seqlen, const float* x, const float* part, const float* b2,
                            const float* gamma, const float* rowvec , const float* w , const float* bias,
                            const float* g, const float* b, float* x_out, float* y);
-    std::string op_fold_dwconv_ln_ex(int dtype, int B, int L, int C, int k, int dil, int S, int run_frames, const int* seqlen, const float* x_in,
+    std::string op_fold_dwconv_ln_ex(int dtype, int B, int L, int C, int k, int dil, int S, int run_frames, int n_cu, const int* seqlen, const float* x_in,
                                      int64_t x_rows, const float* part, int64_t part_stride, int64_t part_elems, const float* b2, const float* gamma,
                                      const float* rowvec, int rv_ld, const float* w, const float* bias, const float* g, const float* b, float* x_out,
                                      int64_t x_out_rows, float* y, int64_t y_rows);
diff --git a/supertonic_amd/csrc/engine_batch.cpp b/supertonic_amd/csrc/engine_batch.cpp
--- a/supertonic_amd/csrc/engine_batch.cpp
+++ b/supertonic_amd/csrc/engine_batch.cpp
@@ -170,16 +170,20 @@
     const int tab_vo = vo_ragged_ ? LEN_VO_SCALED : !tr_rows ? LEN_VO_NONE : vform == VO_TRIM_TAIL ? LEN_VO_TAIL : LEN_VO_2RF;
     const bool tab_pairs = ve_rows > 0 && fused_xattn_ && is_half(dt_) && B >= 2;
     b.tl = len_tables_layout(B, ve_rows, tab_pairs, tab_vo);
-    h_tab_.assign((size_t)b.tl.total, 0);
+    b.tab_runs = -1;
+    b.tab_words = b.tl.total;
+    if (fold_runs_wanted(B, L, ve_rows, n_cu_)) { b.tab_runs = b.tl.total; b.tab_words += 4 * fold_runs_shape(ve_rows, n_cu_).grid; }
+    h_tab_.assign((size_t)b.tab_words, 0);
+    if (b.tab_runs >= 0) fold_runs_build(b.h_llen.data(), B, ve_rows, n_cu_, h_tab_.data() + b.tab_runs);
     len_tables_build(b.tl, b.h_llen.data(), B, ve_rows, tab_pairs, tab_vo, a.chunk_compress_factor, L * a.chunk_compress_factor, vo_rf_, h_tab_.data());
     const unsigned long long seed64 = (unsigned long long)noise_seed;
     std::memcpy(h_tab_.data() + b.tl.seed, &seed64, sizeof seed64);
-    ensure(b.tab, b.tab_cap, (size_t)b.tl.total);
+    ensure(b.tab, b.tab_cap, (size_t)b.tab_words);
     b.llen = b.tab + b.tl.llen;
     seed_dev_ = reinterpret_cast<unsigned long long*>(b.tab + b.tl.seed);
-    if ((size_t)b.tl.total > pin_tab_cap_) {
+    if ((size_t)b.tab_words > pin_tab_cap_) {
         if (pin_tab_) { sync(); drop_graphs(); (void)hipHostFree(pin_tab_); pin_tab_ = nullptr; }
-        const size_t cap = std::max<size_t>((size_t)b.tl.total + (size_t)b.tl.total / 4, (size_t)1024 * (64 + 8));
+        const size_t cap = std::max<size_t>((size_t)b.tab_words + (size_t)b.tab_words / 4, (size_t)1024 * (64 + 8));
         STN_HIP(hipHostMalloc(reinterpret_cast<void**>(&pin_tab_), sizeof(int) * cap, hipHostMallocDefault));
         pin_tab_cap_ = cap;
         pin_valid_ = false;
@@ -304,7 +308,7 @@
     const stn_arch& a = a_;
     const int B = b.B, Lt = b.Lt, L = b.L, D = a.latent_dim * a.chunk_compress_factor;
     const size_t nx = (size_t)B * D * L;
-    STN_HIP(hipMemcpyAsync(b.tab, pin_tab_, sizeof(int) * (size_t)b.tl.total, hipMemcpyHostToDevice, s_));
+    STN_HIP(hipMemcpyAsync(b.tab, pin_tab_, sizeof(int) * (size_t)b.tab_words, hipMemcpyHostToDevice, s_));
     Ragged trg;
     const bool tpk = packed_text_ok(B) && b.trows > 0;
     if (tpk) { trg.off = b.toff; trg.rows = b.trows; }
@@ -343,6 +347,7 @@
         const int* row_b = b.tab + b.tl.ve_row_b;
         rg.off = off; rg.row_b = row_b;
         rg.fold_run = fold_run_frames(b.h_llen.data(), B, n_cu_);
+        rg.fold_runs = b.tab_runs >= 0 ? b.tab + b.tab_runs : nullptr;
         if (fused_xattn_ && is_half(dt_) && B >= 2) {
             if (b.tl.pairs < 0) throw std::logic_error("batch_run: no pairing in the length tables");
             const int* pairs = b.tab + b.tl.pairs;
diff --git a/supertonic_amd/csrc/engine_ops.cpp b/supertonic_amd/csrc/engine_ops.cpp
--- a/supertonic_amd/csrc/engine_ops.cpp
+++ b/supertonic_amd/csrc/engine_ops.cpp
@@ -442,7 +442,7 @@
     for (int i = 0; i < B; ++i) { M += seqlen[i]; L = std::max(L, seqlen[i]); }
     std::fill(x_out, x_out + M * C, 0.f);
     std::fill(y, y + M * C, 0.f);
-    op_fold_dwconv_ln_ex(dt_, B, L, C, k, dil, S, 0, seqlen, x, M, part, M * C, M * C * S, b2, gamma, rowvec, C, w, bias, g, b, x_out, M, y, M);
+    op_fold_dwconv_ln_ex(dt_, B, L, C, k, dil, S, 0, 0, seqlen, x, M, part, M * C, M * C * S, b2, gamma, rowvec, C, w, bias, g, b, x_out, M, y, M);
 }
 
 void Engine::op_block_bench(int B, int L, int C, int I, int k, int dil, int mode, int iters, double* out2) {
@@ -611,7 +611,7 @@
     sync();
 }
 
-std::string Engine::op_fold_dwconv_ln_ex(int dtype, int B, int L, int C, int k, int dil, int S, int run_frames, const int* seqlen, const float* x_in,
+std::string Engine::op_fold_dwconv_ln_ex(int dtype, int B, int L, int C, int k, int dil, int S, int run_frames, int n_cu, const int* seqlen, const float* x_in,
                                          int64_t x_rows, const float* part, int64_t part_stride, int64_t part_elems, const float* b2, const float* gamma,
                                          const float* rowvec, int rv_ld, const float* w, const float* bias, const float* g, const float* b, float* x_out,
                                          int64_t x_out_rows, float* y, int64_t y_rows) {
@@ -637,7 +637,17 @@
     else { float* o = f32_alloc(C); launch_fill(s_, o, C, 1.f); fo.gamma = o; }
     fo.rowvec = rowvec ? up(ar_, s_, rowvec, (size_t)B * rv_ld) : nullptr; fo.rv_ld = rowvec ? rv_ld : C;
     fo.run_frames = run_frames;
-    const std::string form = fold_dwconv_ln_form(dtype, B, L, C, k, dil, S, rowvec != nullptr, run_frames).str();
+    std::string form;
+    if (n_cu > 0) {
+        const int rows = (int)x_rows;
+        std::vector<int32_t> tab((size_t)4 * fold_runs_shape(rows, n_cu).grid), rb((size_t)rows, 0);
+        fold_runs_build(seqlen, B, rows, n_cu, tab.data());
+        for (int b = 0, at = 0; b < B; at += seqlen[b++]) std::fill(rb.begin() + at, rb.begin() + at + seqlen[b], b);
+        fo.runs = FoldRuns{up(ar_, s_, tab.data(), tab.size()), up(ar_, s_, rb.data(), rb.size()), rows, n_cu};
+        form = fold_dwconv_ln_runs_form(dtype, rows, n_cu, C, k, dil, S, rowvec != nullptr);
+    } else {
+        form = fold_dwconv_ln_form(dtype, B, L, C, k, dil, S, rowvec != nullptr, run_frames).str();
+    }
     launch_fold_dwconv_ln(s_, dtype, dx, dxo, B, L, C, fo, dw, db, k, dil, dg, dbt, 1e-6f, dy, dlen, doff);
     STN_HIP(hipGetLastError());
     STN_HIP(hipMemcpyAsync(x_out, dxo, sizeof(float) * (size_t)x_out_rows * C, hipMemcpyDeviceToHost, s_));
diff --git a/supertonic_amd/csrc/kernels.hpp b/supertonic_amd/csrc/kernels.hpp
--- a/supertonic_amd/csrc/kernels.hpp
+++ b/supertonic_amd/csrc/kernels.hpp
@@ -149,6 +149,7 @@
 __host__ __device__ constexpr inline int ffn_lds_side_offset(int C, int I) { return (4 * C * 64 + (I + 2 * C) * 4 + 1023) & ~1023; }
 __host__ __device__ constexpr inline bool ffn_lds_has_side(int C) { return C == 384; }
 void launch_ffn_fused(hipStream_t s, int dtype, int C, const FfnArgs& a);
+struct FoldRuns { const int* table = nullptr; const int* row_b = nullptr; int rows = 0, n_cu = 0; };
 struct FoldArgs {
     const void* part = nullptr; int S = 0; int64_t part_stride = 0;
     const float* b2 = nullptr;
@@ -157,6 +158,7 @@
     const int* row_b = nullptr;
     unsigned long long* ts = nullptr;
     int run_frames = 0;
+    FoldRuns runs;
 };
 int fold_run_frames(const int* lengths, int B, int n_cu);
 void launch_fold_ln(hipStream_t s, int act_dtype, float* x, int64_t M, int C, const FoldArgs& f, const float* g, const float* b, float eps, void* y);
@@ -172,6 +174,11 @@
 void launch_fold_dwconv_ln(hipStream_t s, int act_dtype, const float* x_in, float* x_out, int B, int L, int C, const FoldArgs& f, const float* w_t,
                            const float* bias, int k, int dil, const float* ln_g, const float* ln_b, float eps, void* y, const int* seqlen,
                            const int* row_off);
+struct FoldRunsShape { int R = 0, grid = 0, rounds = 0; };
+FoldRunsShape fold_runs_shape(int rows, int n_cu);
+bool fold_runs_wanted(int B, int L, int rows, int n_cu);
+void fold_runs_build(const int* lengths, int B, int rows, int n_cu, int32_t* out);
+std::string fold_dwconv_ln_runs_form(int act_dtype, int rows, int n_cu, int C, int k, int dil, int S, bool has_rowvec);
 void launch_repack_frag_acc(hipStream_t s, const void* W, int N, int K, void* Wf);
 void launch_ffn_pack(hipStream_t s, const void* W1, const void* W2, int C, int I, void* tmp, void* wseq, int S = 1);
 
diff --git a/supertonic_amd/csrc/kernels_fold.hip b/supertonic_amd/csrc/kernels_fold.hip
--- a/supertonic_amd/csrc/kernels_fold.hip
+++ b/supertonic_amd/csrc/kernels_fold.hip
@@ -268,6 +268,196 @@
     }
 }
 
+constexpr int fold_runs_phase1_rows(int S, int K, int nslot, bool rv) { return rv && fold_phase1_rows(S, K, nslot) == 3 ? 2 : fold_phase1_rows(S, K, nslot); }
+template <typename OutT, bool F16, int K, bool RV, int FOLD_NSLOT, int S>
+__global__ __launch_bounds__(FOLD_NT) void fold_dwconv_ln_runs_kernel(const float* __restrict__ xin, float* __restrict__ xout, int R, int rows, int C,
+                                                                      const uint16_t* __restrict__ part, int64_t pstride,
+                                                                      const float* __restrict__ b2, const float* __restrict__ gamma,
+                                                                      const float* __restrict__ rowvec, int rv_ld, const float* __restrict__ w_t,
+                                                                      const float* __restrict__ bias, int dil, const float* __restrict__ g,
+                                                                      const float* __restrict__ bt, float eps, float inv_c, OutT* __restrict__ y,
+                                                                      const int4* __restrict__ runs, const int* __restrict__ row_off,
+                                                                      const int* __restrict__ row_b, unsigned long long* __restrict__ ts) {
+    extern __shared__ __attribute__((aligned(16))) float fold_sm[];
+    unsigned long long st0 = 0, st1 = 0, st2 = 0;
+    if (ts) st0 = __builtin_readcyclecounter();
+    constexpr int HALF = (K - 1) / 2;
+    constexpr int U = fold_runs_phase1_rows(S, K, FOLD_NSLOT, RV);
+    const int tid = threadIdx.x, C8 = C >> 3, C4 = C >> 2;
+    const int r0 = (int)blockIdx.x * R, W0 = r0 - HALF * dil;
+    const int rpp = FOLD_NT / C8;
+    const int c8 = tid % C8, rq = tid / C8;
+    const int4 ent = runs[blockIdx.x];
+    const int t = r0 + 2 * (tid >> 6) + ((tid & 63) >> 5);
+    const int bt_ = row_b[min(t, rows - 1)];
+    int rb[U];
+    if constexpr (RV) {
+#pragma unroll
+        for (int u = 0; u < U; ++u) rb[u] = row_b[min(max(W0 + rq + u * rpp, 0), rows - 1)];
+    }
+    const int r1 = ent.x;
+    if (r0 >= r1) return;
+    int w0, w1;
+    fold_run_window(r0, r1, ent.y, ent.z, HALF * dil, w0, w1);
+    const int nwu = r1 + HALF * dil - W0;
+    int seq_s = 0, seq_e = 0;
+    bool have_seq = false;
+    float* const zrow = fold_sm + (size_t)(FOLD_TCH + (K - 1) * dil) * C;
+    float* const wsm = zrow + C;
+    constexpr int NPV = (K + 3 + 7) / 8;
+    float4 pv[NPV];
+#pragma unroll
+    for (int i = 0; i < NPV; ++i) {
+        const int q = tid + i * FOLD_NT;
+        const int seg = q / C4, c4 = q - seg * C4;
+        const float* src = seg < K ? w_t + (size_t)seg * C : seg == K ? bias : seg == K + 1 ? g : bt;
+        pv[i] = q < (K + 3) * C4 ? reinterpret_cast<const float4*>(src)[c4] : make_float4(0.f, 0.f, 0.f, 0.f);
+    }
+    if (rq < rpp) {
+        const float4* bp = reinterpret_cast<const float4*>(b2 + c8 * 8);
+        const float4* gp = reinterpret_cast<const float4*>(gamma + c8 * 8);
+        const float4 bb0 = bp[0], bb1 = bp[1], gm0 = gp[0], gm1 = gp[1];
+        for (int q0 = rq; q0 < nwu; q0 += rpp * U) {
+            float4 xa[U][2];
+            float4 tv[U][2];
+            float acc[U][8];
+            int64_t mrow[U];
+#pragma unroll
+            for (int u = 0; u < U; ++u) {
+                mrow[u] = min(max(W0 + q0 + u * rpp, w0), w1 - 1);
+                tv[u][0] = tv[u][1] = make_float4(0.f, 0.f, 0.f, 0.f);
+                if constexpr (RV) { if (q0 != rq) rb[u] = row_b[mrow[u]]; }
+            }
+            auto behind = [&]() {
+                if constexpr (RV) {
+#pragma unroll
+                    for (int u = 0; u < U; ++u) {
+                        const float4* tp = reinterpret_cast<const float4*>(rowvec + (size_t)rb[u] * rv_ld + c8 * 8);
+                        tv[u][0] = tp[0]; tv[u][1] = tp[1];
+                    }
+                }
+                if (!have_seq) { seq_s = row_off[bt_]; seq_e = row_off[bt_ + 1]; have_seq = true; }
+            };
+            if constexpr (U >= 2) {
+                constexpr int CH = S;
+                uint4 w[U][CH];
+#pragma unroll
+                for (int u = 0; u < 2; ++u) {
+                    const float4* xp = reinterpret_cast<const float4*>(xin + mrow[u] * C + c8 * 8);
+                    xa[u][0] = xp[0]; xa[u][1] = xp[1];
+#pragma unroll
+                    for (int sp = 0; sp < CH; ++sp) w[u][sp] = *reinterpret_cast<const uint4*>(part + (size_t)sp * pstride + (size_t)mrow[u] * C + c8 * 8);
+                }
+                if constexpr (U == 3) {
+                    const int m2 = W0 + q0 + 2 * rpp;
+                    if (m2 >= w0 && m2 < w1) {
+                        const float4* xp = reinterpret_cast<const float4*>(xin + mrow[2] * C + c8 * 8);
+                        xa[2][0] = xp[0]; xa[2][1] = xp[1];
+#pragma unroll
+                        for (int sp = 0; sp < CH; ++sp) w[2][sp] = *reinterpret_cast<const uint4*>(part + (size_t)sp * pstride + (size_t)mrow[2] * C + c8 * 8);
+                    } else {
+                        xa[2][0] = xa[2][1] = make_float4(0.f, 0.f, 0.f, 0.f);
+#pragma unroll
+                        for (int sp = 0; sp < CH; ++sp) w[2][sp] = make_uint4(0u, 0u, 0u, 0u);
+                    }
+                }
+                behind();
+#pragma unroll
+                for (int u = 0; u < U; ++u)
+#pragma unroll
+                    for (int sp = 0; sp < CH; ++sp) {
+                        const unsigned wj[4] = {w[u][sp].x, w[u][sp].y, w[u][sp].z, w[u][sp].w};
+#pragma unroll
+                        for (int j = 0; j < 4; ++j) {
+                            const float lo = p16_to_f<F16>(wj[j] & 0xFFFFu), hi = p16_to_f<F16>(wj[j] >> 16);
+                            if (sp == 0) { acc[u][2 * j] = lo; acc[u][2 * j + 1] = hi; }
+                            else { acc[u][2 * j] += lo; acc[u][2 * j + 1] += hi; }
+                        }
+                    }
+            } else {
+                const float4* xp = reinterpret_cast<const float4*>(xin + mrow[0] * C + c8 * 8);
+                xa[0][0] = xp[0]; xa[0][1] = xp[1];
+                fold_chunk<F16, 8, (S <= 12 ? S : 12), true>(part + (size_t)mrow[0] * C + c8 * 8, pstride, 0, acc[0]);
+                behind();
+                if constexpr (S > 12) fold_chunk<F16, 8, 12, false>(part + (size_t)mrow[0] * C + c8 * 8, pstride, 12, acc[0]);
+            }
+#pragma unroll
+            for (int u = 0; u < U; ++u) {
+                const int q = q0 + u * rpp, m = W0 + q;
+                if (m >= w0 && m < w1) {
+                    float4* sp4 = reinterpret_cast<float4*>(fold_sm + (size_t)q * C + c8 * 8);
+                    sp4[0] = fold_four(xa[u][0], acc[u], bb0, gm0, tv[u][0]);
+                    sp4[1] = fold_four(xa[u][1], acc[u] + 4, bb1, gm1, tv[u][1]);
+                }
+            }
+        }
+    }
+    if (!have_seq) { seq_s = row_off[bt_]; seq_e = row_off[bt_ + 1]; }
+#pragma unroll
+    for (int i = 0; i < NPV; ++i) {
+        const int q = tid + i * FOLD_NT;
+        if (q < (K + 3) * C4) reinterpret_cast<float4*>(wsm)[q] = pv[i];
+    }
+    if (tid < C4) reinterpret_cast<float4*>(zrow)[tid] = make_float4(0.f, 0.f, 0.f, 0.f);
+    if (ts) st1 = __builtin_readcyclecounter();
+    __syncthreads();
+    if (ts) st2 = __builtin_readcyclecounter();
+    const int lane = tid & 63, l32 = lane & 31;
+    const float4* ws4 = reinterpret_cast<const float4*>(wsm);
+    const bool live = t < r1;
+    float4 h[FOLD_NSLOT];
+#pragma unroll
+    for (int i = 0; i < FOLD_NSLOT; ++i) {
+        const int c4 = l32 + 32 * i, cq = c4 < C4 ? c4 : 0;
+        float4 a = ws4[K * C4 + cq];
+#pragma unroll
+        for (int j = 0; j < K; ++j) {
+            const int m = live ? fold_run_tap(t, (j - HALF) * dil, seq_s, seq_e) : -1;
+            const float4 xv = *reinterpret_cast<const float4*>((m >= 0 ? fold_sm + (size_t)(m - W0) * C : zrow) + cq * 4);
+            const float4 wv = ws4[j * C4 + cq];
+            a.x = fmaf(wv.x, xv.x, a.x); a.y = fmaf(wv.y, xv.y, a.y);
+            a.z = fmaf(wv.z, xv.z, a.z); a.w = fmaf(wv.w, xv.w, a.w);
+        }
+        h[i] = c4 < C4 ? a : make_float4(0.f, 0.f, 0.f, 0.f);
+    }
+    float s = 0.f;
+#pragma unroll
+    for (int i = 0; i < FOLD_NSLOT; ++i) s += (h[i].x + h[i].y) + (h[i].z + h[i].w);
+    const float mean = half_wave_sum(s) * inv_c;
+    float v = 0.f;
+#pragma unroll
+    for (int i = 0; i < FOLD_NSLOT; ++i)
+        if (l32 + 32 * i < C4) {
+            const float dx = h[i].x - mean, dy = h[i].y - mean, dz = h[i].z - mean, dw = h[i].w - mean;
+            v += (dx * dx + dy * dy) + (dz * dz + dw * dw);
+        }
+    const float rstd = rsqrtf(half_wave_sum(v) * inv_c + eps);
+    if (live) {
+#pragma unroll
+        for (int i = 0; i < FOLD_NSLOT; ++i) {
+            const int c4 = l32 + 32 * i;
+            if (c4 < C4) {
+                const float4 gg = ws4[(K + 1) * C4 + c4], bb = ws4[(K + 2) * C4 + c4];
+                store4(y + (int64_t)t * C + c4 * 4, (h[i].x - mean) * rstd * gg.x + bb.x, (h[i].y - mean) * rstd * gg.y + bb.y,
+                       (h[i].z - mean) * rstd * gg.z + bb.z, (h[i].w - mean) * rstd * gg.w + bb.w);
+            }
+        }
+    }
+    if (rq < rpp)
+        for (int q = rq; q < nwu; q += rpp) {
+            const int m = W0 + q;
+            if (m >= r0 && m < r1) {
+                const float4* sp4 = reinterpret_cast<const float4*>(fold_sm + (size_t)q * C + c8 * 8);
+                float4* op = reinterpret_cast<float4*>(xout + (int64_t)m * C + c8 * 8);
+                op[0] = sp4[0]; op[1] = sp4[1];
+            }
+        }
+    if (ts && tid == 0) {
+        unsigned long long* tp = ts + (size_t)blockIdx.x * 4;
+        tp[0] = st0; tp[1] = st1; tp[2] = st2; tp[3] = __builtin_readcyclecounter();
+    }
+}
+
 int fold_run_frames(const int* lengths, int B, int n_cu) {
     if (!lengths || B <= 0 || n_cu <= 0) return 0;
     int Lmax = 0;
@@ -276,6 +466,40 @@
     for (int tch = FOLD_TCH + 8; tch <= FOLD_TCH_MAX; tch += 8)
         if ((long)B * ((Lmax + tch - 1) / tch) <= n_cu) return tch;
     return 0;
+}
+
+FoldRunsShape fold_runs_shape(int rows, int n_cu) {
+    if (rows < 1 || n_cu < 1) throw std::invalid_argument("fold_runs_shape: rows >= 1 and n_cu >= 1 needed");
+    const FoldRunPlan p = fold_run_plan(rows, n_cu);
+    FoldRunsShape s;
+    s.R = p.R; s.grid = p.grid; s.rounds = p.rounds;
+    return s;
+}
+
+bool fold_runs_wanted(int B, int L, int rows, int n_cu) {
+    static const int mode = [] { const char* e = stn::dev_env("STN_FOLD_RUNS"); return e ? atoi(e) : 1; }();
+    if (mode <= 0 || B < 1 || L < 1 || rows < 1 || n_cu < 1 || (int64_t)B * ((L + FOLD_TCH - 1) / FOLD_TCH) < 64) return false;
+    return mode >= 2 || fold_run_plan(rows, n_cu).rounds == 1;
+}
+
+void fold_runs_build(const int* lengths, int B, int rows, int n_cu, int32_t* out) {
+    const FoldRunPlan p = fold_run_plan(rows, n_cu);
+    int64_t live = 0;
+    for (int i = 0; i < B; ++i) live += lengths[i];
+    if (live > rows) throw std::invalid_argument("fold_runs_build: more frames than rows");
+    int b = 0, s = 0;
+    for (int i = 0; i < p.grid; ++i) {
+        const int r0 = i * p.R, r1 = (int)std::min<int64_t>((int64_t)r0 + p.R, live);
+        FoldRunEntry e{r0, r0, r0, 0};
+        if (r0 < r1) {
+            while (s + lengths[b] <= r0) s += lengths[b++];
+            e.lo = s;
+            while (s + lengths[b] < r1) s += lengths[b++];
+            e.hi = s + lengths[b];
+            e.r1 = r1;
+        }
+        out[4 * i] = e.r1; out[4 * i + 1] = e.lo; out[4 * i + 2] = e.hi; out[4 * i + 3] = e.pad;
+    }
 }
 
 static size_t fold_dwconv_lds(int C, int k, int dil, int tch = FOLD_TCH) { return ((size_t)(tch + (k - 1) * dil) + 1 + (size_t)(k + 3)) * C * 4; }
@@ -324,6 +548,47 @@
                 static_cast<const uint16_t*>(f.part), f.part_stride, f.b2, f.gamma, f.rowvec, f.rv_ld, w_t, bias, dil, g, b, eps, 1.0f / (float)C, y, seqlen, row_off, f.ts, fm.run);
 }
 
+std::string fold_dwconv_ln_runs_form(int act_dtype, int rows, int n_cu, int C, int k, int dil, int S, bool has_rowvec) {
+    const FoldDwconvLnForm f = fold_dwconv_ln_form_forced(act_dtype, 1, 1, C, k, dil, S, has_rowvec, 0, 0);
+    if (S == 24) throw std::invalid_argument("fold_dwconv_ln: the packed-run form takes 4, 8 or 12 splits");
+    const FoldRunsShape sh = fold_runs_shape(rows, n_cu);
+    char m_[112];
+    snprintf(m_, sizeof m_, "fold_dwconv_ln_runs<%s,K%d,%s,ns%d,S%d,U%d> R %d grid %d rounds %d", act_dtype == F16 ? "f16" : "bf16", k, has_rowvec ? "rv" : "norv",
+             f.nslot, S, fold_runs_phase1_rows(S, k, f.nslot, has_rowvec), sh.R, sh.grid, sh.rounds);
+    return m_;
+}
+
+template <typename OutT, int K, bool RV, int NSLOT, int S>
+static void launch_fold_dwconv_ln_runs_one(hipStream_t s, const FoldRunPlan& p, const float* x_in, float* x_out, int C, const FoldArgs& f, const float* w_t,
+                                           const float* bias, int dil, const float* g, const float* b, float eps, OutT* y, const int* row_off) {
+    constexpr bool F16 = std::is_same<OutT, f16_t>::value;
+    static PerDeviceOnce attr_once;
+    if (attr_once.need())
+        stn_check_hip(hipFuncSetAttribute(reinterpret_cast<const void*>(&fold_dwconv_ln_runs_kernel<OutT, F16, K, RV, NSLOT, S>), hipFuncAttributeMaxDynamicSharedMemorySize,
+                                          160 * 1024), "hipFuncSetAttribute(fold_dwconv_ln_runs)");
+    STN_KLAUNCH((fold_dwconv_ln_runs_kernel<OutT, F16, K, RV, NSLOT, S>), dim3((unsigned)p.grid), dim3(FOLD_NT), fold_dwconv_lds(C, K, dil), s, x_in, x_out, p.R, f.runs.rows, C,
+                static_cast<const uint16_t*>(f.part), f.part_stride, f.b2, f.gamma, f.rowvec, f.rv_ld, w_t, bias, dil, g, b, eps, 1.0f / (float)C, y,
+                reinterpret_cast<const int4*>(f.runs.table), row_off, f.runs.row_b, f.ts);
+}
+
+static void launch_fold_dwconv_ln_runs(hipStream_t s, int act_dtype, const float* x_in, float* x_out, int C, const FoldArgs& f, const float* w_t, const float* bias,
+                                       int k, int dil, const float* ln_g, const float* ln_b, float eps, void* y, const int* row_off) {
+    if (!f.runs.row_b || f.runs.rows < 1 || f.runs.n_cu < 1 || (reinterpret_cast<uintptr_t>(f.runs.table) & 15) || !fold_dwconv_ln_supported(C, k, dil))
+        throw std::invalid_argument("launch_fold_dwconv_ln: the packed-run form needs a 16-byte aligned run table, the row map, k in {5,7}, C % 8 == 0, C <= 512");
+    const FoldRunPlan p = fold_run_plan(f.runs.rows, f.runs.n_cu);
+    const int nslot = C <= 384 ? 3 : 4;
+    bool found = false;
+    with_half_type(act_dtype, [&](auto* tag) {
+    with_const<5, 7>(k, [&](auto K) {
+    with_const<0, 1>(f.rowvec != nullptr, [&](auto rv) {
+    with_const<3, 4>(nslot, [&](auto ns) {
+    found = with_const<4, 8, 12>(f.S, [&](auto S) {
+        using T = std::remove_pointer_t<decltype(tag)>;
+        launch_fold_dwconv_ln_runs_one<T, K(), rv() != 0, ns(), S()>(s, p, x_in, x_out, C, f, w_t, bias, dil, ln_g, ln_b, eps, static_cast<T*>(y), row_off);
+    }); }); }); }); });
+    if (!found) throw std::invalid_argument("fold_dwconv_ln: the packed-run form takes 4, 8 or 12 splits");
+}
+
 void launch_fold_dwconv_ln(hipStream_t s, int act_dtype, const float* x_in, float* x_out, int B, int L, int C, const FoldArgs& f, const float* w_t,
                            const float* bias, int k, int dil, const float* ln_g, const float* ln_b, float eps, void* y, const int* seqlen,
                            const int* row_off) {
@@ -333,6 +598,7 @@
         throw std::invalid_argument("launch_fold_dwconv_ln: packed 16-bit rows, separate output, k in {5,7}, C % 8 == 0, C <= 512 needed");
     check_fold_args(f, 0, C, "launch_fold_dwconv_ln");
     static const int force = [] { const char* e = stn::dev_env("STN_FOLD_TCH"); return e ? atoi(e) : 0; }();
+    if (f.runs.table && !force && f.S != 24) return launch_fold_dwconv_ln_runs(s, act_dtype, x_in, x_out, C, f, w_t, bias, k, dil, ln_g, ln_b, eps, y, row_off);
     const FoldDwconvLnForm fm = fold_dwconv_ln_form_forced(act_dtype, B, L, C, k, dil, f.S, f.rowvec != nullptr, f.run_frames, force);
     bool found = false;
     with_half_type(act_dtype, [&](auto* tag) {
diff --git a/supertonic_amd/csrc/kernels_fold.hpp b/supertonic_amd/csrc/kernels_fold.hpp
--- a/supertonic_amd/csrc/kernels_fold.hpp
+++ b/supertonic_amd/csrc/kernels_fold.hpp
@@ -42,6 +42,22 @@
 }
 
 
+struct FoldRunEntry { int r1, lo, hi, pad; };
+struct FoldRunPlan { int R, grid, rounds; };
+__host__ __device__ inline FoldRunPlan fold_run_plan(int rows, int n_cu) {
+    const int rounds = (int)(((int64_t)rows + (int64_t)32 * n_cu - 1) / ((int64_t)32 * n_cu));
+    const int R = (int)(((int64_t)rows + (int64_t)rounds * n_cu - 1) / ((int64_t)rounds * n_cu));
+    return FoldRunPlan{R, (rows + R - 1) / R, rounds};
+}
+__host__ __device__ inline void fold_run_window(int r0, int r1, int lo, int hi, int reach, int& w0, int& w1) {
+    w0 = r0 - reach > lo ? r0 - reach : lo;
+    w1 = r1 + reach < hi ? r1 + reach : hi;
+}
+__host__ __device__ inline int fold_run_tap(int t, int shift, int s, int e) {
+    const int tt = t + shift;
+    return tt >= s && tt < e ? tt : -1;
+}
+
 __device__ __forceinline__ float dpp_add(float v, int ctrl_sel) {
     const int iv = __float_as_int(v);
     int o;
```

Result: no change. 48260, median of 3 (+0.0%).
